# FraPria/proovread

Measured on AMD Instinct MI355X. Metric: corrected long-read Mbases/sec per node, higher is better.
Workload: dtype int32

## Files before the change

include/prgpu.h:

```cpp
#ifndef PRGPU_H
#define PRGPU_H
#include <stdint.h>
#ifdef __cplusplus
extern "C" {
#endif

enum {
    PR_OK = 0,
    PR_ERR_ARG = -1,
    PR_ERR_HIP = -2,
    PR_ERR_SAM = -3,
    PR_ERR_NOSEQ = -4,
    PR_ERR_BIN_RANGE = -5,
    PR_ERR_DIV0 = -6,
    PR_ERR_CIGAR = -7,
    PR_ERR_BEYOND_REF = -8,
    PR_ERR_CAPACITY = -9,
    PR_ERR_UNSUPPORTED = -10,
};

const char *pr_last_error(void);
const char *pr_version(void);

typedef struct pr_ctx pr_ctx;
int pr_ctx_create(int device, pr_ctx **out);
void pr_ctx_destroy(pr_ctx *ctx);
int pr_device_count(int *n);
int pr_ctx_sync(pr_ctx *ctx);
int pr_dev_alloc(pr_ctx *ctx, int64_t bytes, void **dev);
int pr_dev_free(pr_ctx *ctx, void *dev);
int pr_dev_download(pr_ctx *ctx, void *host, const void *dev, int64_t bytes);
int pr_dev_upload(pr_ctx *ctx, void *dev, const void *host, int64_t bytes);
typedef struct {
    char name[16];
    int64_t cur, peak, at_total_peak;
} pr_mem_group;
int pr_mem_stats(int64_t *cur, int64_t *peak, pr_mem_group *groups, int cap, int *n_groups);
void pr_mem_reset_peak(void);

#define PR_COMM_ID_BYTES 128
enum { PR_DT_I64 = 0, PR_DT_F64 = 1, PR_DT_I32 = 2, PR_DT_U8 = 3 };
enum { PR_RED_SUM = 0, PR_RED_MAX = 1, PR_RED_MIN = 2 };
typedef struct pr_comm pr_comm;
int pr_comm_unique_id(uint8_t *id);
int pr_comm_init(pr_ctx *ctx, int world, int rank, const uint8_t *id, pr_comm **out);
void pr_comm_destroy(pr_comm *c);
int pr_comm_rank(const pr_comm *c, int *rank, int *world);
int pr_comm_agree(pr_comm *c, int local_rc);
int pr_comm_allreduce_dev(pr_comm *c, const void *dev_in, void *dev_out, int64_t n, int dtype, int op);
int pr_comm_allreduce_host(pr_comm *c, void *buf, int64_t n, int dtype, int op);
int pr_comm_barrier(pr_comm *c);
int pr_comm_allgatherv_host(pr_comm *c, const uint8_t *send, int64_t nbytes, uint8_t *recv, int64_t recv_cap,
                            int64_t *counts);
int pr_comm_alltoall_counts(pr_comm *c, const int64_t *send_counts, int64_t *recv_counts);
int pr_comm_alltoallv_host(pr_comm *c, const uint8_t *send, const int64_t *send_counts, uint8_t *recv,
                           const int64_t *recv_counts);
int pr_comm_alltoallv_dev(pr_comm *c, const void *send, const int64_t *send_counts, void *recv,
                          const int64_t *recv_counts);
int pr_comm_allgatherv_dev(pr_comm *c, const void *send, const int64_t *counts, void *recv);
typedef struct pr_comm_group pr_comm_group;
int pr_comm_group_create(int world, pr_comm_group **out);
void pr_comm_group_destroy(pr_comm_group *g);
void pr_comm_group_abort(pr_comm_group *g);
int pr_comm_init_local(pr_ctx *ctx, pr_comm_group *g, int rank, pr_comm **out);


typedef struct pr_cns_params {
    double max_coverage;
    double bin_size;
    int32_t trim;
    int32_t indel_taboo_length;
    double indel_taboo;
    int32_t min_aln_length;
    int32_t max_ins_length;
    int32_t fallback_phred;
    int32_t phred_offset;
    int32_t ref_phred_offset;
    int32_t use_ref_qual;
    int32_t qual_weighted;
    int32_t detect_chimera;
    int32_t invert_scores;
} pr_cns_params;

void pr_cns_params_default(pr_cns_params *p);

enum { PR_ALN_HAS_SCORE = 1, PR_ALN_NO_QUAL = 2, PR_ALN_NO_SEQ = 4 };

typedef struct pr_cns_batch {
    int32_t n_lr;
    const int64_t *lr_off;
    const uint8_t *ref_seq;
    const uint8_t *ref_qual;
    const int64_t *ign_off;
    const int32_t *ign;
    const int64_t *aln_off;
    const int32_t *aln_pos;
    const double *aln_score;
    const uint8_t *aln_flags;
    const int64_t *aln_seq_off;
    const int32_t *aln_lseq;
    const int64_t *aln_cig_off;
    const int32_t *aln_ncig;
    const uint8_t *seq_pool;
    const uint8_t *qual_pool;
    const uint32_t *cig_pool;
    int64_t seq_pool_len, cig_pool_len;
} pr_cns_batch;

typedef struct pr_cns_bounds {
    int64_t seq_cap;
    int64_t chim_cap;
} pr_cns_bounds;
int pr_cns_bounds_of(const pr_cns_batch *b, pr_cns_bounds *out);

typedef struct pr_cns_out {
    int64_t *out_off;
    int32_t *status;
    int32_t *seq_len;
    int32_t *trace_len;
    int32_t *ncigar;
    int32_t *nchim;
    uint8_t *seq;
    uint8_t *qual;
    uint8_t *trace;
    uint32_t *cigar;
    int64_t *chim_off;
    int32_t *chim;
    uint8_t *kept;
    int64_t *bin_bases;
} pr_cns_out;

int pr_cns_run(pr_ctx *ctx, const pr_cns_params *p, const pr_cns_batch *b, pr_cns_out *o);

int pr_cns_upload(pr_ctx *ctx, const pr_cns_batch *b);
int pr_cns_launch(pr_ctx *ctx, const pr_cns_params *p);
int pr_cns_download(pr_ctx *ctx, pr_cns_out *o);
int pr_cns_last_timing(pr_ctx *ctx, double *ms_prep, double *ms_pileup);
int pr_cns_phase_ticks(pr_ctx *ctx, uint64_t *ticks, int n);
int pr_cns_resident_stats(pr_ctx *ctx, int64_t *columns, int64_t *alg_bytes);



typedef struct pr_sw_opts {
    int32_t a, b;
    int32_t o_del, e_del;
    int32_t o_ins, e_ins;
    int32_t w;
    int32_t pen_clip5, pen_clip3;
    int32_t zdrop;
    double min_score_per_base;
    int32_t bin_size;
    double bin_length;
    double drop_ratio;
    double mask_level;
    double mask_level_redun;
    int32_t max_chain_gap;
} pr_sw_opts;
void pr_sw_opts_default(pr_sw_opts *o, int finish);

typedef struct pr_sw_batch {
    int32_t n_sr;
    const int64_t *sr_off;
    const uint8_t *sr_seq;
    int32_t n_lr;
    const int64_t *lr_off;
    const uint8_t *lr_seq;
    int64_t n_task;
    const int32_t *t_sr, *t_lr;
    const uint8_t *t_strand;
    const int32_t *t_qbeg, *t_rbeg, *t_slen;
    const int32_t *t_chain;
    int64_t read_id0;
} pr_sw_batch;

typedef struct pr_sw_out {
    int32_t *qb, *qe;
    int32_t *rb, *re;
    int32_t *score;
    int32_t *truesc;
    int32_t *pos;
    int32_t *ncigar;
    uint8_t *pass;
    int32_t *status;
    int64_t *cigar_off;
    uint32_t *cigar;
    int64_t cigar_cap;
    int32_t *task;
    int32_t *flag;
} pr_sw_out;

int pr_sw_run(pr_ctx *ctx, const pr_sw_opts *o, const pr_sw_batch *b, pr_sw_out *out);
int pr_sw_upload(pr_ctx *ctx, const pr_sw_batch *b);
int pr_sw_launch(pr_ctx *ctx, const pr_sw_opts *o);
int pr_sw_download(pr_ctx *ctx, pr_sw_out *out);
int pr_sw_cigar_total(pr_ctx *ctx, int64_t *total, int64_t *n_overflow);
int pr_sw_aln_count(pr_ctx *ctx, int64_t *n_aln);
typedef struct pr_sam_in {
    const int64_t *sr_off;
    const uint8_t *sr_text;
    const uint8_t *sr_qual;
    const char *sr_names;
    const int64_t *sr_name_off;
    const char *lr_names;
    const int64_t *lr_name_off;
    const uint8_t *keep;
    int32_t n_threads;
} pr_sam_in;
int pr_sw_binfilter(pr_ctx *ctx, int32_t bin_size, double bin_length, uint8_t *keep);
int pr_sw_sam(pr_ctx *ctx, const pr_sam_in *in, char **text, int64_t *len, int64_t *n_records);
int pr_sw_bwa_stats(pr_ctx *ctx, int32_t *rounds, int64_t *n_extended, int64_t *n_patch);
int pr_sw_bwa_timing(pr_ctx *ctx, float *walk_ms, float *final_ms, float *early_final_ms);
int pr_sw_last_timing(pr_ctx *ctx, double *ms_extend, double *ms_global);
int pr_sw_last_cells(pr_ctx *ctx, int64_t *cells_extend, int64_t *cells_global);
int pr_sw_dominant_kernel(pr_ctx *ctx, double *ms, int64_t *cells);
int pr_sw_extension_kernels(pr_ctx *ctx, double *ms, int64_t *cells, int32_t *launches);
int pr_sw_phase_cycles(pr_ctx *ctx, int64_t *out4);

typedef struct pr_seed_opts {
    int min_seed_len;
    int min_chain_weight;
    int w;
    double split_factor;
    int split_width;
    int max_mem_intv;
    int max_occ;
    double drop_ratio;
    int max_chain_gap;
    double mask_level;
    int a, o_del, e_del, o_ins, e_ins;
    int b;
} pr_seed_opts;
typedef struct pr_seed_task {
    int32_t sr, lr;
    int32_t strand;
    int32_t qbeg, rbeg, slen;
    int32_t rmax0, rmax1;
    int32_t chain;
    int32_t rank;
} pr_seed_task;
typedef struct pr_seed_tasks {
    int64_t n;
    pr_seed_task *t;
} pr_seed_tasks;
typedef struct pr_seed_index pr_seed_index;
void pr_seed_opts_default(pr_seed_opts *o, int finish);
int pr_seed_index_build(const uint8_t *lr_seq, const int64_t *lr_off, int n_lr, pr_seed_index **out);
void pr_seed_index_free(pr_seed_index *h);
int pr_seed_map(const pr_seed_index *h, const pr_seed_opts *o, const uint8_t *sr_seq, const int64_t *sr_off,
                int n_sr, int n_threads, pr_seed_tasks *out);
void pr_seed_tasks_free(pr_seed_tasks *t);
int pr_seed_index_occ(const pr_seed_index *h, const uint8_t *s, int n, int64_t *count);
int pr_seed_index_digest(const pr_seed_index *h, uint64_t *out6);
int pr_seed_index_koff(const pr_seed_index *h, uint64_t *koff, uint64_t *ksplit);
int pr_seed_gpu_index_koff(pr_ctx *ctx, uint64_t *koff, uint64_t *ksplit);
int pr_seed_smem(const pr_seed_index *h, const uint8_t *q, int len, int x, int64_t min_intv, int32_t *start,
                 int32_t *end, int64_t *occ, int cap, int *n_out);
int pr_seed_gpu_upload(pr_ctx *ctx, const pr_seed_index *h);
int pr_seed_gpu_map(pr_ctx *ctx, const pr_seed_opts *o, const uint8_t *sr_seq, const int64_t *sr_off, int n_sr,
                    pr_seed_tasks *out, int32_t *status);
int pr_seed_gpu_index_build(pr_ctx *ctx, const uint8_t *lr_seq, const int64_t *lr_off, int n_lr);
int pr_seed_gpu_index_digest(pr_ctx *ctx, uint64_t *out6);
int pr_seed_gpu_index_last_ms(pr_ctx *ctx, double *ms);
int pr_seed_gpu_seed_count(pr_ctx *ctx, int64_t *n);
int pr_seed_gpu_pass2_reads(pr_ctx *ctx, int64_t *n);
int pr_seed_gpu_pass_reads(pr_ctx *ctx, int64_t *n4);
int pr_seed_gpu_last_ms(pr_ctx *ctx, double *ms);
int pr_seed_gpu_phase_ticks(pr_ctx *ctx, uint64_t *ticks4);
int pr_seed_gpu_lane_ticks(pr_ctx *ctx, uint64_t *ticks6);
int pr_seed_gpu_occ_ticks(pr_ctx *ctx, uint64_t *ticks3);
int pr_seed_gpu_pass2_ticks(pr_ctx *ctx, uint64_t *t7);
int pr_seed_gpu_pass2_ms(pr_ctx *ctx, double *ms);
int pr_seed_map_device_caps(const pr_seed_index *h, const pr_seed_opts *o, const uint8_t *sr_seq,
                            const int64_t *sr_off, int n_sr, int n_threads, pr_seed_tasks *out, int32_t *status);

typedef struct pr_iter_batch {
    pr_sw_batch sw;
    const int64_t *task_lr_off;
    const uint8_t *lr_qual;
    const uint8_t *ref_seq;
} pr_iter_batch;
int pr_iter_upload(pr_ctx *ctx, const pr_iter_batch *b);
int pr_iter_upload_gpu_seeds(pr_ctx *ctx, const pr_iter_batch *b);
int pr_iter_launch(pr_ctx *ctx, const pr_sw_opts *o, const pr_cns_params *p);
int pr_iter_download(pr_ctx *ctx, pr_cns_out *out);
int pr_fmt_chim_lines(int32_t n_lr, const char *names, const int64_t *name_off, const int32_t *nchim,
                      const int64_t *chim_off, const int32_t *chim, char **text, int64_t *len, int64_t *n_lines);
int pr_iter_download_range(pr_ctx *ctx, int32_t first, int32_t n, pr_cns_out *out);
int pr_iter_bounds(pr_ctx *ctx, int32_t *n_lr, int64_t *n_task, pr_cns_bounds *bd);
int pr_iter_alignment_stats(pr_ctx *ctx, int64_t *n_aln, int64_t *sum_ncig, int64_t *sum_lseq);
int pr_iter_handoff_stats(pr_ctx *ctx, int64_t *big_reads, int64_t *big_alns, int32_t *max_alns);
int pr_iter_handoff_order(pr_ctx *ctx, int32_t lr, int32_t *task_idx, int64_t cap, int64_t *n);
int pr_iter_last_timing(pr_ctx *ctx, double *ms_sw_extend, double *ms_sw_global, double *ms_assemble,
                        double *ms_consensus);
int pr_sw_upload_gpu_seeds(pr_ctx *ctx, const pr_sw_batch *b);
int pr_aln_exchange(pr_ctx *ctx, pr_comm *comm, int64_t sr0, const int64_t *lr_bounds, int64_t *n_recv);
int pr_aln_exchange_local(pr_ctx *const *ctxs, int world, const int64_t *sr0, const int64_t *lr_bounds,
                          int64_t *n_recv);
int pr_aln_exchange_sources(pr_ctx *ctx, int64_t *per_rank, int cap, int *world);
typedef struct pr_own_batch {
    int32_t lr0, n_lr;
    const int64_t *lr_off;
    const uint8_t *ref_seq;
    const uint8_t *lr_qual;
    int32_t n_sr;
    const int64_t *sr_off;
    const uint8_t *sr_seq;
    int32_t from_set;
} pr_own_batch;
enum { PR_OWN_FROM_SET = 1, PR_OWN_RESIDENT_SR = 2 };
int pr_iter_upload_owned(pr_ctx *ctx, const pr_own_batch *b);

enum { PR_LRSET_MAP = 0, PR_LRSET_READS = 1 };
enum { PR_LRSET_COMMIT_MASK = 1, PR_LRSET_COMMIT_DRY = 2 };
int pr_lrset_load(pr_ctx *ctx, int32_t n_lr, const int64_t *off, const uint8_t *seq, const uint8_t *qual);
int pr_lrset_info(pr_ctx *ctx, int32_t *n_lr, int64_t *bases);
int pr_lrset_index(pr_ctx *ctx, int which);
int pr_iter_upload_lrset(pr_ctx *ctx, const pr_sw_batch *b);
int pr_lrset_commit(pr_ctx *ctx, pr_comm *comm, int flags);
int pr_lrset_download(pr_ctx *ctx, int64_t *off, uint8_t *seq, uint8_t *qual, uint8_t *map);
int pr_lrset_snapshot(pr_ctx *ctx);
int pr_lrset_restore(pr_ctx *ctx);
int pr_srset_load(pr_ctx *ctx, int64_t n_sr, const int64_t *off, const uint8_t *seq);
int pr_seed_gpu_map_sampled(pr_ctx *ctx, const pr_seed_opts *o, const int64_t *ranges, int n_ranges, int32_t *status);
int pr_srset_sample(pr_ctx *ctx, const int64_t *ranges, int n_ranges);

int pr_iter_stats(pr_ctx *ctx, int32_t min_phred, int64_t *dev_out);

typedef struct pr_mask_params {
    int32_t phred_min, phred_max;
    int32_t mask_min_len;
    int32_t unmask_min_len;
    int32_t mask_reduce;
    double end_ratio;
    int32_t phred_offset;
} pr_mask_params;
void pr_mask_params_default(pr_mask_params *p);
int pr_mask_params_parse(const char *hcr_mask, int32_t min_sr_length, pr_mask_params *out);
int pr_mask_bound(const pr_mask_params *p, int32_t n, const int64_t *off, int64_t *mcr_cap);
int pr_mask_run(pr_ctx *ctx, const pr_mask_params *p, int32_t n, const int64_t *off, const uint8_t *seq,
                const uint8_t *qual, uint8_t *out_seq, int64_t *mcr_off, int32_t *mcr, int32_t *n_mcr,
                int64_t *stats);
int pr_iter_mask(pr_ctx *ctx, const pr_mask_params *p, int64_t *dev_stats);
int pr_iter_mask_download(pr_ctx *ctx, uint8_t *masked);

int pr_fastq4_scan(const uint8_t *data, int64_t n, int64_t *n_rec, int64_t *n_bases);
int pr_fastq4_fill(const uint8_t *data, int64_t n, const uint8_t *table256, int64_t *starts, int64_t *off,
                   uint8_t *pool);

typedef struct pr_trim_params {
    int32_t size;
    int32_t soft;
    int32_t hard;
    int32_t min_len;
    int32_t phred_offset;
} pr_trim_params;
void pr_trim_params_default(pr_trim_params *p);
int pr_trim_params_parse(const char *trim_win, pr_trim_params *p);
int pr_trim_bound(const pr_trim_params *p, int32_t n, const int64_t *off, int64_t *win_cap);
int pr_trim_windows(const pr_trim_params *p, int32_t n, const int64_t *off, const uint8_t *qual, int64_t *win_off,
                    int32_t *win, int32_t *n_win, int n_threads);

int pr_sam_encode(const char *text, int64_t len, const char *const *ref_names, int32_t n_ref, int n_threads,
                  uint8_t **out, int64_t *out_len, int64_t *n_records);
int pr_bgzf_compress(const uint8_t *data, int64_t len, int level, int n_threads, uint8_t **out, int64_t *out_len);
int pr_bgzf_decompress(const uint8_t *data, int64_t len, int n_threads, uint8_t **out, int64_t *out_len);
int pr_bam_sort_records(const uint8_t *recs, int64_t len, int n_threads, uint8_t **out, int64_t *out_len,
                        int64_t *n_records);
typedef struct pr_bam_alns {
    int64_t n;
    int32_t *rid, *pos1;
    double *score;
    uint8_t *flags;
    int64_t *seq_off;
    int32_t *lseq;
    int64_t *cig_off;
    int32_t *ncig;
    uint8_t *seq, *qual;
    uint32_t *cig;
    int64_t seq_len, cig_len;
} pr_bam_alns;
int pr_bam_decode_alns(const uint8_t *recs, int64_t len, int n_threads, pr_bam_alns *out);
void pr_bam_alns_free(pr_bam_alns *a);
int pr_bam_decode_alns_gpu(pr_ctx *ctx, const uint8_t *recs, int64_t len, pr_bam_alns *out);
int pr_cns_upload_bam(pr_ctx *ctx, const pr_cns_batch *reads, const uint8_t *recs, int64_t len,
                      const int32_t *ref_to_lr, int32_t n_ref, int64_t *n_kept);
int pr_cns_resident_bounds(pr_ctx *ctx, pr_cns_bounds *out);
int pr_cns_resident_aln_count(pr_ctx *ctx, int64_t *n_aln, int64_t *aln_off);
int pr_bam_decode_last_ms(pr_ctx *ctx, double *ms);
int pr_bam_index(const uint8_t *data, int64_t len, int n_threads, uint8_t **out, int64_t *out_len);
void pr_buffer_free(void *p);

typedef struct pr_siam_aligner {
    int32_t a, b;
    int32_t o, e;
    int32_t w, zdrop;
    int32_t word;
} pr_siam_aligner;
typedef struct pr_siam_params {
    int32_t seq_min_len;
    int32_t term_ignore_len;
    int32_t trim;
    int32_t filter_inconclusive;
    double aln_min_idy;
    pr_siam_aligner pass1, pass2;
} pr_siam_params;
typedef struct pr_siam_hsp {
    int32_t read, qas, qae, sas, sae, length, matches, score;
} pr_siam_hsp;
enum { PR_SIAM_KEEP = 0, PR_SIAM_TRIM = 1, PR_SIAM_DROP = 2 };
enum {
    PR_SIAM_SEED_OVERFLOW = 1,
    PR_SIAM_HSP_OVERFLOW = 2,
    PR_SIAM_TOO_LONG = 4,
};
#define PR_SIAM_MAX_SEEDS 1024
#define PR_SIAM_MAX_HSPS 64
#define PR_SIAM_MAX_LEN 131072
typedef struct pr_siam_decision {
    int32_t action, from, to;
} pr_siam_decision;
void pr_siam_params_default(pr_siam_params *p);
int pr_siam_hsps_host(const pr_siam_aligner *al, double min_idy, const uint8_t *seq, const int64_t *off, int32_t n,
                      int n_threads, const pr_siam_hsp **hsps, int64_t *n_hsps, int32_t *status);
int pr_siam_hsps_gpu(pr_ctx *ctx, const pr_siam_aligner *al, double min_idy, const uint8_t *seq, const int64_t *off,
                     int32_t n, const pr_siam_hsp **hsps, int64_t *n_hsps, int32_t *status);
int pr_siam_decide(const pr_siam_params *p, int32_t len, const pr_siam_hsp *h1, int32_t n1, const pr_siam_hsp *h2,
                   int32_t n2, pr_siam_decision *out, int32_t *inconclusive);
int pr_siam_run(pr_ctx *ctx, const pr_siam_params *p, const uint8_t *seq, const int64_t *off, int32_t n,
                int n_threads, pr_siam_decision *out, int32_t *status, int64_t *summary);
int pr_siam_last_ms(pr_ctx *ctx, double *ms);
int pr_siam_seeds_host(const uint8_t *seq, int32_t len, int32_t word, int32_t *out, int32_t cap, int32_t *n);
int pr_siam_extend_host(const pr_siam_aligner *al, const uint8_t *q, int32_t qlen, const uint8_t *t, int32_t tlen,
                        int32_t h0, int32_t *out);
int pr_siam_extend_gpu(pr_ctx *ctx, const pr_siam_aligner *al, const uint8_t *q, const int64_t *q_off,
                       const uint8_t *t, const int64_t *t_off, const int32_t *h0, int32_t n, int32_t *out);

#ifdef __cplusplus
}
#endif
#endif
```

proovread_amd/csrc/seed.cpp:

```cpp
#include <algorithm>
#include <atomic>
#include <cstdlib>
#include <cstring>
#include <string>
#include <thread>
#include <utility>
#include <vector>

#include <sys/mman.h>

#include "../../include/prgpu.h"
#include "seed_core.h"
#include "seed_dev.h"

namespace seedc = prgpu::seedc;

int pr_set_error(int code, const char *msg);

namespace {

constexpr int KI = 12;
constexpr uint32_t NK = 1u << (2 * KI);
constexpr uint8_t SEP = 5;
constexpr int KX = 28;
// ... 326 lines not shown
    };
    const int64_t n_text = 2 * l_pac + 2 * (int64_t)n_lr;
    I.text.resize((size_t)n_text);
    I.cstart.assign(2 * (size_t)n_lr, 0);
    for (int i = 0; i < n_lr; ++i) {
        I.cstart[i] = I.lr_off[i] + i;
        I.cstart[2 * (size_t)n_lr - 1 - i] = l_pac + n_lr + (l_pac - I.lr_off[i + 1]) + (n_lr - 1 - i);
    }
    run_threads([&](int t) {
        uint8_t *X = I.text.data();
        for (int i = (int)((int64_t)n_lr * t / nt); i < (int)((int64_t)n_lr * (t + 1) / nt); ++i) {
            const uint8_t *r = lr_seq + lr_off[i];
            const int64_t len = lr_off[i + 1] - lr_off[i];
            uint8_t *f = X + I.cstart[i];
            uint8_t *b = X + I.cstart[2 * (size_t)n_lr - 1 - i];
            for (int64_t p = 0; p < len; ++p) {
                const uint8_t c = seedc::base_code(r[p]);
                f[p] = c;
                b[len - 1 - p] = c < 4 ? (uint8_t)(3 - c) : 4;
            }
            f[len] = SEP;
            b[len] = SEP;
        }
    });
    const uint8_t *T = I.text.data();
    const int64_t n = (int64_t)I.text.size();
    {
        const int64_t nb = (n >> CB_SHIFT) + 1;
        I.cblk.assign((size_t)nb, 0);
        int c = 0;
        const int nc = (int)I.cstart.size();
        for (int64_t b = 0; b < nb; ++b) {
            while (c + 1 < nc && I.cstart[c + 1] <= (b << CB_SHIFT)) ++c;
            I.cblk[(size_t)b] = c;
        }
    }
    auto for_kmers = [&](int64_t p0, int64_t p1, auto f) {
        uint32_t code = 0;
        int run = 0;
        int64_t p = p0 - (KI - 1) > 0 ? p0 - (KI - 1) : 0;
        for (; p < p1 + KI - 1 && p < n; ++p) {
            if (T[p] > 3) { run = 0; code = 0; continue; }
            code = ((code << 2) | T[p]) & (NK - 1);
            if (++run >= KI && p - KI + 1 >= p0) f(code, (int64_t)(p - KI + 1));
        }
    };
    std::vector<std::vector<uint32_t>> tc((size_t)nt);
    run_threads([&](int t) {
        std::vector<uint32_t> &c = tc[(size_t)t];
        c.assign(NK, 0);
        for_kmers(n * t / nt, n * (t + 1) / nt, [&](uint32_t k, int64_t) { ++c[k]; });
    });
    std::vector<uint32_t> kc(NK);
    I.koff.assign(NK + 1, 0);
    std::vector<uint64_t> part((size_t)nt + 1, 0);
    run_threads([&](int t) {
        const uint32_t k0 = (uint32_t)((uint64_t)NK * t / nt), k1 = (uint32_t)((uint64_t)NK * (t + 1) / nt);
        uint64_t run = 0;
        for (uint32_t k = k0; k < k1; ++k) {
            uint32_t sum = 0;
            for (int u = 0; u < nt; ++u) sum += tc[(size_t)u][k];
            kc[k] = sum;
            run += sum;
            I.koff[k + 1] = run;
        }
        part[(size_t)t + 1] = run;
    });
    for (int t = 0; t < nt; ++t) part[(size_t)t + 1] += part[(size_t)t];
    run_threads([&](int t) {
        const uint32_t k0 = (uint32_t)((uint64_t)NK * t / nt), k1 = (uint32_t)((uint64_t)NK * (t + 1) / nt);
        const uint64_t base = part[(size_t)t];
        for (uint32_t k = k0; k < k1; ++k) I.koff[k + 1] += base;
    });
    I.kpos.resize(I.koff[NK]);
    I.kext.resize(I.koff[NK]);
    constexpr int LB = 12;
    constexpr uint32_t NB = NK >> LB;
    struct Rec {
        uint32_t pos, low;
        uint64_t ext;
    };
    const bool paged = n > (int64_t)seedc::POS_PAGE;
    if (paged) I.ksplit.assign(NK, 0);
    BigVec<Rec> tmp(I.koff[NK]);
    {
        std::vector<std::vector<uint64_t>> cur((size_t)nt, std::vector<uint64_t>(NB, 0));
        run_threads([&](int u) {
            for (uint32_t b = (uint32_t)((uint64_t)NB * u / nt); b < (uint32_t)((uint64_t)NB * (u + 1) / nt); ++b) {
                uint64_t o = I.koff[b << LB];
                for (int t = 0; t < nt; ++t) {
                    cur[(size_t)t][b] = o;
                    uint64_t sz = 0;
                    for (uint32_t k = b << LB; k < ((b + 1) << LB); ++k) sz += tc[(size_t)t][k];
                    o += sz;
                }
            }
        });
        tc.clear();
        tc.shrink_to_fit();
        run_threads([&](int t) {
            const int64_t p0 = n * t / nt, p1 = n * (t + 1) / nt;
            uint64_t *c = cur[(size_t)t].data();
            Rec *R = tmp.data();
            uint32_t code = 0;
            int run = 0;
            int64_t p = p0 - (KI - 1) > 0 ? p0 - (KI - 1) : 0;
            uint64_t w = 0;
            for (int j = KX - 1; j >= 0; --j) w = (w << 2) | (p + 1 + j < n ? (uint64_t)(T[p + 1 + j] & 3) : 0);
            int64_t nb = p + 1;
            while (nb < n && T[nb] <= 3) ++nb;
            for (bool first = true; p < p1 + KI - 1 && p < n; ++p, first = false) {
                if (!first) {
                    const int64_t q = p + KX;
                    w = (w >> 2) | ((q < n ? (uint64_t)(T[q] & 3) : 0) << (2 * (KX - 1)));
                    if (nb < p + 1) {
                        nb = p + 1;
                        while (nb < n && T[nb] <= 3) ++nb;
                    }
                }
                if (T[p] > 3) { run = 0; code = 0; continue; }
                code = ((code << 2) | T[p]) & (NK - 1);
                if (++run >= KI && p - KI + 1 >= p0) {
                    int64_t m = nb - (p + 1);
                    if (m > KX) m = KX;
                    const uint64_t ext = (m ? (w & ((1ull << (2 * m)) - 1)) : 0) | ((uint64_t)m << 56);
                    Rec &r = R[c[code >> LB]++];
                    r.pos = (uint32_t)(p - KI + 1);
                    r.low = (code & ((1u << LB) - 1)) | ((uint32_t)((uint64_t)(p - KI + 1) >> 32) << 31);
                    r.ext = ext;
                }
            }
        });
    }
    {
        std::atomic<uint32_t> next{0};
        run_threads([&](int) {
            std::vector<uint64_t> fill((size_t)1 << LB);
            for (uint32_t b; (b = next.fetch_add(1)) < NB;) {
                const uint32_t k0 = b << LB;
                for (uint32_t j = 0; j < (1u << LB); ++j) fill[j] = I.koff[k0 + j];
                if (paged)
                    for (uint32_t j = 0; j < (1u << LB); ++j) I.ksplit[k0 + j] = I.koff[k0 + j + 1];
                for (uint64_t i = I.koff[k0]; i < I.koff[k0 + (1u << LB)]; ++i) {
                    const Rec &r = tmp[i];
                    const uint32_t lo = r.low & ((1u << LB) - 1);
                    const uint64_t slot = fill[lo]++;
                    if ((r.low >> 31) && I.ksplit[k0 + lo] > slot) I.ksplit[k0 + lo] = slot;
                    I.kpos[slot] = r.pos;
                    I.kext[slot] = r.ext;
                }
            }
        });
    }
    tmp.clear();
    tmp.shrink_to_fit();
    std::vector<std::vector<uint32_t>> tail(KI);
    {
        std::vector<std::vector<int64_t>> stops((size_t)nt);
        run_threads([&](int t) {
            for (int64_t p = n * t / nt; p < n * (t + 1) / nt; ++p)
                if (T[p] > 3 && p > 0 && T[p - 1] <= 3) stops[(size_t)t].push_back(p);
        });
        for (auto &v : stops)
            for (const int64_t p : v) {
                uint32_t code = 0;
                for (int j = 1; j < KI && p - j >= 0 && T[p - j] <= 3; ++j) {
                    code |= (uint32_t)T[p - j] << (2 * (j - 1));
                    tail[j].push_back(code);
                }
            }
    }
    I.cnt[KI - 1] = std::move(kc);
    for (int j = KI - 1; j >= 1; --j) {
        std::vector<uint32_t> &cj = I.cnt[j - 1];
        cj.assign((size_t)1 << (2 * j), 0);
        const std::vector<uint32_t> &cn = I.cnt[j];
        for (size_t x = 0; x < cj.size(); ++x) cj[x] = cn[4 * x] + cn[4 * x + 1] + cn[4 * x + 2] + cn[4 * x + 3];
        for (uint32_t code : tail[j]) ++cj[code];
    }
    *out = h;
    return 0;
}

extern "C" void pr_seed_index_free(pr_seed_index *h) { delete h; }

template <class T>
static uint64_t digest_of(const T *p, size_t n) {
    uint64_t h = 1469598103934665603ull ^ (uint64_t)n;
    for (size_t i = 0; i < n; ++i) {
        h ^= (uint64_t)p[i];
        h *= 1099511628211ull;
        h ^= h >> 29;
    }
    return h;
}

template <class A, class B, class Cc, class Dd, class E, class F, class G, class H>
static void digest6(const A &text, const B &koff, const Cc &kpos, const Dd &kext, const E &cnt, const F &cstart,
                    const G &cblk, const H &lr_off, uint64_t *out6) {
    out6[0] = digest_of(text.data(), text.size());
    out6[1] = digest_of(koff.data(), koff.size());
    out6[2] = digest_of(kpos.data(), kpos.size());
    out6[3] = digest_of(kext.data(), kext.size());
    uint64_t c = 0;
    for (int j = 0; j < KI; ++j) c = c * 31 + digest_of(cnt[j].data(), cnt[j].size());
    out6[4] = c;
    out6[5] = digest_of(cstart.data(), cstart.size()) * 31 + digest_of(cblk.data(), cblk.size()) * 7 +
              digest_of(lr_off.data(), lr_off.size());
}

extern "C" int pr_seed_index_digest(const pr_seed_index *h, uint64_t *out6) {
    if (!h || !out6) return pr_set_error(PR_ERR_ARG, "null arg");
    const Index &I = h->I;
    digest6(I.text, I.koff, I.kpos, I.kext, I.cnt, I.cstart, I.cblk, I.lr_off, out6);
    if (!I.ksplit.empty()) out6[1] ^= digest_of(I.ksplit.data(), I.ksplit.size()) * 31;
    return 0;
}

extern "C" int pr_seed_index_koff(const pr_seed_index *h, uint64_t *koff, uint64_t *ksplit) {
    if (!h || !koff) return pr_set_error(PR_ERR_ARG, "null arg");
    std::memcpy(koff, h->I.koff.data(), h->I.koff.size() * 8);
    if (ksplit && !h->I.ksplit.empty()) std::memcpy(ksplit, h->I.ksplit.data(), h->I.ksplit.size() * 8);
    return 0;
}

namespace prgpu {
void seed_digest_tables(const std::vector<uint8_t> &text, const std::vector<uint64_t> &koff,
                        const std::vector<uint32_t> &kpos, const std::vector<uint64_t> &kext,
                        const std::vector<std::vector<uint32_t>> &cnt, const std::vector<int64_t> &cstart,
                        const std::vector<int32_t> &cblk, const std::vector<int64_t> &lr_off,
                        const std::vector<uint64_t> &ksplit, uint64_t *out6) {
    digest6(text, koff, kpos, kext, cnt, cstart, cblk, lr_off, out6);
    if (!ksplit.empty()) out6[1] ^= digest_of(ksplit.data(), ksplit.size()) * 31;
}
}

extern "C" int pr_seed_index_occ(const pr_seed_index *h, const uint8_t *s, int n, int64_t *count) {
    if (!h || !s || !count || n <= 0) return pr_set_error(PR_ERR_ARG, "bad arg");
    for (int i = 0; i < n; ++i)
        if (s[i] > 3) { *count = 0; return 0; }
    *count = occ(h->I, s, 0, n);
    return 0;
}

extern "C" int pr_seed_smem(const pr_seed_index *h, const uint8_t *q, int len, int x, int64_t min_intv,
                            int32_t *start, int32_t *end, int64_t *occs, int cap, int *n_out) {
    if (!h || !q || !n_out || x < 0 || x >= len) return pr_set_error(PR_ERR_ARG, "bad arg");
    std::vector<Iv> mem;
    const int ret = smem1(IndexOcc{h->I, q}, q, len, x, min_intv, mem);
    if ((int)mem.size() > cap) return pr_set_error(PR_ERR_CAPACITY, "smem output capacity");
    for (size_t i = 0; i < mem.size(); ++i) start[i] = mem[i].start, end[i] = mem[i].end, occs[i] = mem[i].occ;
    *n_out = (int)mem.size();
    return ret;
}

extern "C" int pr_seed_map(const pr_seed_index *h, const pr_seed_opts *o, const uint8_t *sr_seq, const int64_t *sr_off,
                           int n_sr, int n_threads, pr_seed_tasks *out) {
    if (!h || !o || !out || n_sr < 0 || (n_sr && (!sr_seq || !sr_off))) return pr_set_error(PR_ERR_ARG, "null arg");
    if (o->min_seed_len < KI) return pr_set_error(PR_ERR_UNSUPPORTED, "min seed length below the 12-mer index");
    if (o->max_occ <= 0 || o->w < 0) return pr_set_error(PR_ERR_ARG, "bad seeding options");
    out->n = 0;
    out->t = nullptr;
    for (int i = 0; i < n_sr; ++i)
        if (sr_off[i + 1] < sr_off[i] || sr_off[i + 1] - sr_off[i] > (1 << 20))
            return pr_set_error(PR_ERR_ARG, "sr_off not monotone");
    int nt = n_threads > 0 ? n_threads : (int)std::thread::hardware_concurrency();
    nt = nt < 1 ? 1 : (nt > 256 ? 256 : nt);
    std::vector<ReadOut> res(n_sr);
    const seedc::IndexView V = view_of(h->I);
    std::atomic<int> next{0};
    auto work = [&]() {
        std::vector<uint8_t> q;
        for (;;) {
            const int i0 = next.fetch_add(64);
            if (i0 >= n_sr) break;
            for (int i = i0; i < n_sr && i < i0 + 64; ++i) {
                const int len = (int)(sr_off[i + 1] - sr_off[i]);
                q.assign(sr_seq + sr_off[i], sr_seq + sr_off[i + 1]);
                for (auto &c : q) c = c < 4 ? c : 4;
                if (len > 0) map_read(V, *o, q.data(), len, i, res[i]);
            }
        }
    };
    std::vector<std::thread> th;
    for (int t = 1; t < nt; ++t) th.emplace_back(work);
    work();
    for (auto &t : th) t.join();
    int64_t total = 0;
    for (auto &r : res) total += (int64_t)r.tasks.size();
    out->t = (pr_seed_task *)std::malloc(sizeof(pr_seed_task) * (size_t)(total > 0 ? total : 1));
    if (!out->t) return pr_set_error(PR_ERR_ARG, "out of host memory");
    int64_t k = 0;
    for (auto &r : res)
        for (auto &t : r.tasks) out->t[k++] = t;
    out->n = total;
    return 0;
}

extern "C" void pr_seed_tasks_free(pr_seed_tasks *t) {
    if (t && t->t) std::free(t->t);
    if (t) t->t = nullptr, t->n = 0;
}

extern "C" int pr_seed_map_device_caps(const pr_seed_index *h, const pr_seed_opts *o, const uint8_t *sr_seq,
                                       const int64_t *sr_off, int n_sr, int n_threads, pr_seed_tasks *out,
                                       int32_t *status) {
    if (!h || !o || !out || !status || n_sr < 0 || (n_sr && (!sr_seq || !sr_off)))
        return pr_set_error(PR_ERR_ARG, "null arg");
    if (o->min_seed_len < KI) return pr_set_error(PR_ERR_UNSUPPORTED, "min seed length below the 12-mer index");
    out->n = 0;
    out->t = nullptr;
    seedc::IndexView V = view_of(h->I);
    int qmax = 1;
    for (int i = 0; i < n_sr; ++i) qmax = std::max<int>(qmax, (int)(sr_off[i + 1] - sr_off[i]));
    std::vector<uint64_t> text4((size_t)(V.n_text / 16 + 8), 0);
    for (size_t w = 0; w < text4.size(); ++w) {
        uint64_t v = 0;
        for (int k = 0; k < 16; ++k) {
            const int64_t x = (int64_t)w * 16 + k;
            v |= (uint64_t)(x < V.n_text ? V.text[x] : SEP) << (4 * k);
        }
        text4[w] = v;
    }
    V.text4 = text4.data();
    seedc::Caps caps = seedc::device_caps(qmax);
    caps.hi = V.ksplit != nullptr;
    caps.lazy = seedc::lazy_occ(*o) ? 1 : 0;
    const int64_t bytes = seedc::scratch_bytes(caps);
    int nt = n_threads > 0 ? n_threads : (int)std::thread::hardware_concurrency();
    nt = nt < 1 ? 1 : (nt > 64 ? 64 : nt);
    std::vector<ReadOut> res(n_sr);
    std::atomic<int> next{0};
    const char *fe = getenv("PRGPU_SCRATCH_FILL");
    const uint64_t fill = fe ? 0x0101010101010101ull * (uint64_t)(strtoul(fe, nullptr, 0) & 0xFF) : 0;
    auto work = [&]() {
        std::vector<uint64_t> slab((size_t)(bytes / 8 + 1), fill);
        seedc::Scratch S = seedc::carve(reinterpret_cast<uint8_t *>(slab.data()), caps);
        for (int k = 0; k < S.hsize; ++k) S.htab[k].key = -1;
        S.htab_clean = true;
        std::vector<pr_seed_task> buf((size_t)caps.out);
        std::vector<uint64_t> big;
        for (;;) {
            const int i = next.fetch_add(1);
            if (i >= n_sr) break;
            const int len = (int)(sr_off[i + 1] - sr_off[i]);
            int n = 0, err = 0;
            if (len > 0) err = seedc::map_read(V, *o, S, sr_seq + sr_off[i], len, i, buf.data(), caps.out, &n);
            seedc::Caps cg = caps;
            for (int pass = 3; pass <= 6 && err && !(err & (seedc::SC_OVER_LEN | seedc::SC_OVER_OUT)); ++pass) {
                cg = seedc::grow_caps(cg, err, 4);
                big.assign((size_t)(seedc::scratch_bytes(cg) / 8 + 1), fill);
                seedc::Scratch G = seedc::carve(reinterpret_cast<uint8_t *>(big.data()), cg);
                for (int k = 0; k < G.hsize; ++k) G.htab[k].key = -1;
                G.htab_clean = true;
                err = seedc::map_read(V, *o, G, sr_seq + sr_off[i], len, i, buf.data(), caps.out, &n);
            }
            status[i] = err;
            if (!err) res[i].tasks.assign(buf.begin(), buf.begin() + n);
        }
    };
    std::vector<std::thread> th;
    for (int t = 1; t < nt; ++t) th.emplace_back(work);
    work();
    for (auto &t : th) t.join();
    int64_t total = 0;
    for (auto &r : res) total += (int64_t)r.tasks.size();
    out->t = (pr_seed_task *)std::malloc(sizeof(pr_seed_task) * (size_t)(total > 0 ? total : 1));
    if (!out->t) return pr_set_error(PR_ERR_ARG, "out of host memory");
    int64_t k = 0;
    for (auto &r : res)
        for (auto &t : r.tasks) out->t[k++] = t;
    out->n = total;
    return 0;
}
```

proovread_amd/csrc/seed_api.cpp:

```cpp
#include <algorithm>
#include <climits>
#include <cstdio>
#include <cstdlib>
#include <cstring>
#include <vector>

#include "ctx.h"
#include "seed_index_dev.h"
#include "seed_plan.h"

static int seed_text4(pr_ctx *c, seedc::IndexView &v, hipStream_t s) {
    int rc = c->sd[SI_TEXT4].ensure((size_t)ix_pack4_words(v.n_text) * 8);
    if (rc) return rc;
    const int e = ix_pack4_launch(v.text, v.n_text, c->sd[SI_TEXT4].as<uint64_t>(), s);
    if (e) return set_error(PR_ERR_HIP, "text packing: %s", hipGetErrorString((hipError_t)e));
    v.text4 = c->sd[SI_TEXT4].as<uint64_t>();
    v.walk_nw = v.n_text > ((int64_t)64 << 24) ? 1 : 4;
    if (const char *w = getenv("PRGPU_SEED_WALK_NW"))
        v.walk_nw = atoi(w) == 1 ? 1 : 4;
    return 0;
}

static int upload_blk_fr(pr_ctx *c, seedc::IndexView &v, const int64_t *cstart, const int64_t *off, int n_lr,
                         int64_t l_pac, int64_t n_text, hipStream_t s) {
    const int64_t nb = (n_text >> seedc::CB_SHIFT) + 1;
    const int nc = 2 * n_lr;
    const int bs = 1 << seedc::CB_SHIFT;
    auto delta = [&](int ci) -> int64_t {
        if (ci < n_lr) return off[ci] - cstart[ci];
        const int rid = 2 * n_lr - 1 - ci;
        return 2 * l_pac - off[rid + 1] - cstart[ci];
    };
    std::vector<seedc::BlkFr> t((size_t)nb);
    int ci = 0;
    for (int64_t b = 0; b < nb; ++b) {
        const int64_t b0 = b << seedc::CB_SHIFT, b1 = b0 + bs;
        while (ci + 1 < nc && cstart[ci + 1] <= b0) ++ci;
        seedc::BlkFr &e = t[(size_t)b];
        e.c0 = ci;
        e.d0 = nc ? delta(ci) : 0;
        e.d1 = ci + 1 < nc ? delta(ci + 1) : 0;
        e.bnd = ci + 1 < nc && cstart[ci + 1] < b1 ? (int32_t)(cstart[ci + 1] - b0) : bs;
        e.bnd2 = ci + 2 < nc && cstart[ci + 2] < b1 ? (int32_t)(cstart[ci + 2] - b0) : bs;
    }
    int rc = c->sd[SI_BLKFR].ensure(t.size() * sizeof(seedc::BlkFr));
    if (rc) return rc;
    HIPCHK(hipMemcpyAsync(c->sd[SI_BLKFR].p, t.data(), t.size() * sizeof(seedc::BlkFr), hipMemcpyHostToDevice, s));
    HIPCHK(hipStreamSynchronize(s));
    v.blkfr = c->sd[SI_BLKFR].as<seedc::BlkFr>();
    return 0;
}

extern "C" int pr_seed_gpu_upload(pr_ctx *c, const pr_seed_index *h) {
    if (!c || !h) return set_error(PR_ERR_ARG, "null arg");
    HIPCHK(hipSetDevice(c->device));
    hipStream_t s = c->stream;
    const seedc::IndexView hv = seed_index_view(h);
    const SeedIndexSizes z = seed_index_sizes(h);
    DevBuf *D = c->sd;
    int rc;
    if ((rc = upload(D[SI_TEXT], hv.text, (size_t)z.text, s)) || (rc = upload(D[SI_CSTART], hv.cstart, (size_t)z.cstart, s)) ||
        (rc = upload(D[SI_CBLK], hv.cblk, (size_t)z.cblk, s)) || (rc = upload(D[SI_LROFF], hv.lr_off, (size_t)z.lr_off, s)) ||
        (rc = upload(D[SI_KOFF], hv.koff, (size_t)z.koff, s)) || (rc = upload(D[SI_KPOS], hv.kpos, (size_t)z.kpos, s)) ||
        (rc = upload(D[SI_KEXT], hv.kext, (size_t)z.kpos, s)) ||
        (z.ksplit && (rc = upload(D[SI_KSPLIT], hv.ksplit, (size_t)z.ksplit, s))))
        return rc;
    seedc::IndexView v = hv;
    for (int j = 0; j < seedc::KI - 1; ++j) {
        if ((rc = upload(D[SI_CNT0 + j], hv.cnt[j], (size_t)z.cnt[j], s))) return rc;
        v.cnt[j] = D[SI_CNT0 + j].as<uint32_t>();
    }
    v.text = D[SI_TEXT].as<uint8_t>();
    v.cstart = D[SI_CSTART].as<int64_t>();
    v.cblk = D[SI_CBLK].as<int32_t>();
    v.lr_off = D[SI_LROFF].as<int64_t>();
    v.koff = D[SI_KOFF].as<uint64_t>();
    v.kpos = D[SI_KPOS].as<uint32_t>();
    v.kext = D[SI_KEXT].as<uint64_t>();
    v.ksplit = z.ksplit ? D[SI_KSPLIT].as<uint64_t>() : nullptr;
    if ((rc = seed_text4(c, v, s))) return rc;
    if ((rc = upload_blk_fr(c, v, hv.cstart, hv.lr_off, hv.n_lr, hv.l_pac, hv.n_text, s))) return rc;
    HIPCHK(hipStreamSynchronize(s));
    c->seed_view = v;
    c->seed_loaded = true;
    return 0;
}

static void index_host_tables(const int64_t *lr_off, int n_lr, int64_t l_pac, int64_t n_text, std::vector<int64_t> &off,
                              std::vector<int64_t> &cstart, std::vector<int32_t> &cblk) {
    off.assign((size_t)n_lr + 1, 0);
    cstart.assign(2 * (size_t)n_lr, 0);
    for (int i = 0; i <= n_lr; ++i) off[(size_t)i] = lr_off[i] - (n_lr ? lr_off[0] : 0);
    for (int i = 0; i < n_lr; ++i) {
        cstart[(size_t)i] = off[(size_t)i] + i;
        cstart[2 * (size_t)n_lr - 1 - i] = l_pac + n_lr + (l_pac - off[(size_t)i + 1]) + (n_lr - 1 - i);
    }
    const int64_t nb = (n_text >> seedc::CB_SHIFT) + 1;
    cblk.assign((size_t)nb, 0);
    int ci = 0;
    const int nc = 2 * n_lr;
    for (int64_t b = 0; b < nb; ++b) {
        while (ci + 1 < nc && cstart[(size_t)ci + 1] <= (b << seedc::CB_SHIFT)) ++ci;
        cblk[(size_t)b] = ci;
    }
}

static int64_t index_sort_chunk(const DevBuf *D, int64_t n_text) {
    int64_t chunk = (int64_t)1 << 30;
    if (n_text > chunk) {
        size_t fr = 0, tot = 0;
        (void)hipMemGetInfo(&fr, &tot);
        (void)hipGetLastError();
        const int64_t have = (int64_t)(D[SX_KEY0].cap + D[SX_KEY1].cap + D[SX_VAL0].cap + D[SX_VAL1].cap + D[SX_TEMP].cap);
        if ((int64_t)fr + have >= ((int64_t)1 << 31) * 20 + ((int64_t)64 << 30)) chunk = (int64_t)1 << 31;
    }
    if (const char *ch = getenv("PRGPU_INDEX_CHUNK")) {
        const int k = atoi(ch);
        if (k >= 16 && k <= 31) chunk = (int64_t)1 << k;
    }
    return chunk;
}

static int index_buffers(pr_ctx *c, const uint8_t *lr_seq, const int64_t *lr_off, int n_lr, bool lr_dev, int64_t l_pac,
                         int64_t n_text, int64_t chunk, const std::vector<int64_t> &off, const std::vector<int64_t> &cstart,
                         const std::vector<int32_t> &cblk, SeedIndexBuild &B) {
    hipStream_t s = c->stream;
    DevBuf *D = c->sd;
    const size_t nt = (size_t)(n_text > 0 ? n_text : 1);
    const bool chunked = n_text > chunk;
    const size_t ns = (size_t)(chunked ? chunk : (int64_t)nt);
    const size_t temp = seed_index_temp_bytes((int64_t)ns);
    const size_t nk1 = (size_t)seedc::NK + 1;
    int rc;
    if ((rc = upload(D[SX_LRSEQ], lr_dev ? nullptr : (n_lr ? lr_seq + lr_off[0] : lr_seq), (size_t)l_pac, s)) ||
        (rc = upload(D[SI_LROFF], off.data(), off.size(), s)) || (rc = upload(D[SI_CSTART], cstart.data(), cstart.size(), s)) ||
        (rc = upload(D[SI_CBLK], cblk.data(), cblk.size(), s)) || (rc = D[SI_TEXT].ensure(nt)) ||
        (rc = D[SX_KEY0].ensure(ns * 4)) || (rc = D[SX_KEY1].ensure(ns * 4)) || (rc = D[SX_VAL0].ensure(ns * 4)) ||
        (rc = D[SX_KC].ensure(nk1 * 4)) || (rc = D[SI_KOFF].ensure(nk1 * 8)) ||
        (rc = D[SI_KPOS].ensure(nt * 4)) || (rc = D[SI_KEXT].ensure(nt * 8)) || (rc = D[SX_TEMP].ensure(temp)) ||
        (rc = D[SX_CNTPTR].ensure(sizeof(uint32_t *) * (seedc::KI - 1))))
        return rc;
    if (chunked && ((rc = D[SX_VAL1].ensure(ns * 4)) || (rc = D[SX_KCC].ensure(nk1 * 4)) ||
                    (rc = D[SX_KOFFC].ensure(nk1 * 4)) || (rc = D[SX_KCUR].ensure(nk1 * 8))))
        return rc;
    const bool paged = n_text > (int64_t)seedc::POS_PAGE;
    if (paged && (rc = D[SI_KSPLIT].ensure(nk1 * 8))) return rc;
    if (lr_dev && l_pac) HIPCHK(hipMemcpyAsync(D[SX_LRSEQ].p, lr_seq + lr_off[0], (size_t)l_pac, hipMemcpyDeviceToDevice, s));
    uint32_t *cptr[seedc::KI - 1];
    for (int j = 1; j < seedc::KI; ++j) {
        if ((rc = D[SI_CNT0 + j - 1].ensure(((size_t)1 << (2 * j)) * 4))) return rc;
        cptr[j - 1] = B.cnt[j - 1] = D[SI_CNT0 + j - 1].as<uint32_t>();
    }
    HIPCHK(hipMemcpyAsync(D[SX_CNTPTR].p, cptr, sizeof cptr, hipMemcpyHostToDevice, s));
    B.lr_seq = D[SX_LRSEQ].as<uint8_t>();
    B.lr_off = D[SI_LROFF].as<int64_t>();
    B.n_lr = n_lr;
    B.l_pac = l_pac;
    B.cstart = D[SI_CSTART].as<int64_t>();
    B.n_text = n_text;
    B.text = D[SI_TEXT].as<uint8_t>();
    B.chunk = chunk;
    B.key0 = D[SX_KEY0].as<uint32_t>();
    B.key1 = D[SX_KEY1].as<uint32_t>();
    B.val0 = D[SX_VAL0].as<uint32_t>();
    B.val1 = chunked ? D[SX_VAL1].as<uint32_t>() : nullptr;
    B.kc = D[SX_KC].as<uint32_t>();
    B.koff = D[SI_KOFF].as<uint64_t>();
    B.kcc = chunked ? D[SX_KCC].as<uint32_t>() : nullptr;
    B.koffc = chunked ? D[SX_KOFFC].as<uint32_t>() : nullptr;
    B.kcur = chunked ? D[SX_KCUR].as<uint64_t>() : nullptr;
    B.kpos = D[SI_KPOS].as<uint32_t>();
    B.kext = D[SI_KEXT].as<uint64_t>();
    B.ksplit = paged ? D[SI_KSPLIT].as<uint64_t>() : nullptr;
    B.cnt_dev = reinterpret_cast<uint32_t *const *>(D[SX_CNTPTR].p);
    B.temp = D[SX_TEMP].p;
    B.temp_bytes = temp;
    return 0;
}

int index_build(pr_ctx *c, const uint8_t *lr_seq, const int64_t *lr_off, int n_lr, bool lr_dev) {
    if (!c || n_lr < 0 || (n_lr && (!lr_seq || !lr_off))) return set_error(PR_ERR_ARG, "null arg");
    for (int i = 0; i < n_lr; ++i)
        if (lr_off[i + 1] < lr_off[i]) return set_error(PR_ERR_ARG, "lr_off not monotone");
    const int64_t l_pac = n_lr ? lr_off[n_lr] - lr_off[0] : 0;
    if (2 * l_pac + 2 * (int64_t)n_lr > seedc::MAX_TEXT)
        return set_error(PR_ERR_CAPACITY, "long reads beyond the index's 2^33 text positions (l_pac < 4.29 Gb)");
    if ((int64_t)n_lr >= ((int64_t)1 << seedc::FR_RID_BITS))
        return set_error(PR_ERR_CAPACITY, "more than 2^24 long reads in one index");
    HIPCHK(hipSetDevice(c->device));
    hipStream_t s = c->stream;
    DevBuf *D = c->sd;
    const int64_t n_text = 2 * l_pac + 2 * (int64_t)n_lr;
    std::vector<int64_t> off, cstart;
    std::vector<int32_t> cblk;
    index_host_tables(lr_off, n_lr, l_pac, n_text, off, cstart, cblk);
    SeedIndexBuild B{};
    int rc = index_buffers(c, lr_seq, lr_off, n_lr, lr_dev, l_pac, n_text, index_sort_chunk(D, n_text), off, cstart, cblk, B);
    if (rc) return rc;
    HIPCHK(hipEventRecord(c->ev[8], s));
    const int e = seed_index_device_build(B, s);
    if (e) return set_error(PR_ERR_HIP, "seed index build: %s", hipGetErrorString((hipError_t)e));
    HIPCHK(hipEventRecord(c->ev[9], s));
    uint64_t nh = 0;
    HIPCHK(hipMemcpyAsync(&nh, B.koff + seedc::NK, 8, hipMemcpyDeviceToHost, s));
    HIPCHK(hipStreamSynchronize(s));
    float ms = 0.f;
    if (hipEventElapsedTime(&ms, c->ev[8], c->ev[9]) == hipSuccess) c->ms_index = ms;
    if (n_text > (int64_t)seedc::POS_PAGE) {
        for (int id : {(int)SX_KEY0, (int)SX_KEY1, (int)SX_VAL0, (int)SX_VAL1, (int)SX_TEMP}) D[id].release();
    }
    seedc::IndexView v{};
    v.text = B.text;
    v.n_text = n_text;
    v.cstart = B.cstart;
    v.n_contig = 2 * n_lr;
    v.cblk = D[SI_CBLK].as<int32_t>();
    v.lr_off = B.lr_off;
    v.n_lr = n_lr;
    v.l_pac = l_pac;
    v.koff = B.koff;
    v.kpos = B.kpos;
    v.kext = B.kext;
    v.ksplit = B.ksplit;
    for (int j = 0; j < seedc::KI - 1; ++j) v.cnt[j] = B.cnt[j];
    if ((rc = seed_text4(c, v, s))) return rc;
    if ((rc = upload_blk_fr(c, v, cstart.data(), off.data(), n_lr, l_pac, n_text, s))) return rc;
    c->seed_view = v;
    c->seed_loaded = true;
    c->seed_n_text = n_text;
    c->seed_n_hits = nh;
    return 0;
}

extern "C" int pr_seed_gpu_index_build(pr_ctx *c, const uint8_t *lr_seq, const int64_t *lr_off, int n_lr) {
    return index_build(c, lr_seq, lr_off, n_lr, false);
}

extern "C" int pr_seed_gpu_index_digest(pr_ctx *c, uint64_t *out6) {
    if (!c || !out6) return set_error(PR_ERR_ARG, "null arg");
    if (!c->seed_loaded || !c->seed_n_text) return set_error(PR_ERR_ARG, "no device-built seed index");
    HIPCHK(hipSetDevice(c->device));
    const seedc::IndexView &v = c->seed_view;
    const size_t nt = (size_t)c->seed_n_text, nh = (size_t)c->seed_n_hits, nk = (size_t)seedc::NK;
    std::vector<uint8_t> text(nt);
    std::vector<uint64_t> koff(nk + 1);
    std::vector<uint32_t> kpos(nh), kc(nk);
    std::vector<uint64_t> kext(nh);
    std::vector<int64_t> cstart((size_t)v.n_contig), lro((size_t)v.n_lr + 1);
    std::vector<int32_t> cblk((size_t)((c->seed_n_text >> seedc::CB_SHIFT) + 1));
    std::vector<std::vector<uint32_t>> cnt(seedc::KI);
    HIPCHK(hipMemcpy(text.data(), v.text, nt, hipMemcpyDeviceToHost));
    HIPCHK(hipMemcpy(koff.data(), v.koff, (nk + 1) * 8, hipMemcpyDeviceToHost));
    if (nh) HIPCHK(hipMemcpy(kpos.data(), v.kpos, nh * 4, hipMemcpyDeviceToHost));
    if (nh) HIPCHK(hipMemcpy(kext.data(), v.kext, nh * 8, hipMemcpyDeviceToHost));
    HIPCHK(hipMemcpy(kc.data(), c->sd[SX_KC].p, nk * 4, hipMemcpyDeviceToHost));
    if (!cstart.empty()) HIPCHK(hipMemcpy(cstart.data(), v.cstart, cstart.size() * 8, hipMemcpyDeviceToHost));
    HIPCHK(hipMemcpy(lro.data(), v.lr_off, lro.size() * 8, hipMemcpyDeviceToHost));
    HIPCHK(hipMemcpy(cblk.data(), v.cblk, cblk.size() * 4, hipMemcpyDeviceToHost));
    for (int j = 0; j < seedc::KI - 1; ++j) {
        cnt[(size_t)j].resize((size_t)1 << (2 * (j + 1)));
        HIPCHK(hipMemcpy(cnt[(size_t)j].data(), v.cnt[j], cnt[(size_t)j].size() * 4, hipMemcpyDeviceToHost));
    }
    cnt[seedc::KI - 1] = std::move(kc);
    std::vector<uint64_t> ksplit(v.ksplit ? nk : 0);
    if (v.ksplit) HIPCHK(hipMemcpy(ksplit.data(), v.ksplit, nk * 8, hipMemcpyDeviceToHost));
    seed_digest_tables(text, koff, kpos, kext, cnt, cstart, cblk, lro, ksplit, out6);
    return 0;
}

extern "C" int pr_seed_gpu_index_koff(pr_ctx *c, uint64_t *koff, uint64_t *ksplit) {
    if (!c || !koff) return set_error(PR_ERR_ARG, "null arg");
    if (!c->seed_loaded) return set_error(PR_ERR_ARG, "no device seed index");
    HIPCHK(hipSetDevice(c->device));
    HIPCHK(hipStreamSynchronize(c->stream));
    HIPCHK(hipMemcpy(koff, c->seed_view.koff, ((size_t)seedc::NK + 1) * 8, hipMemcpyDeviceToHost));
    if (ksplit && c->seed_view.ksplit)
        HIPCHK(hipMemcpy(ksplit, c->seed_view.ksplit, (size_t)seedc::NK * 8, hipMemcpyDeviceToHost));
    return 0;
}

extern "C" int pr_seed_gpu_index_last_ms(pr_ctx *c, double *ms) {
    if (!c || !ms) return set_error(PR_ERR_ARG, "null arg");
    *ms = c->ms_index;
    return 0;
}

extern "C" int pr_srset_load(pr_ctx *c, int64_t n_sr, const int64_t *off, const uint8_t *seq) {
    if (!c || n_sr < 0 || !off || (off[n_sr] && !seq) || off[0] != 0) return set_error(PR_ERR_ARG, "bad arg");
    HIPCHK(hipSetDevice(c->device));
    int rc = upload(c->ls[LS_SRSEQ], seq, (size_t)off[n_sr], c->stream);
    if (rc) return rc;
    HIPCHK(hipStreamSynchronize(c->stream));
    c->ss_off.assign(off, off + n_sr + 1);
    c->ss_samp_off.clear();
    c->ls[LS_SRSAMP].release();
    return 0;
}

static int gather_ranges(pr_ctx *c, const int64_t *ranges, int n_ranges, int64_t max_reads, DevBuf &dst,
                         std::vector<int64_t> &off) {
    if (c->ss_off.empty()) return set_error(PR_ERR_ARG, "no resident short reads (pr_srset_load)");
    const int64_t N = (int64_t)c->ss_off.size() - 1;
    off.assign(1, 0);
    for (int k = 0; k < n_ranges; ++k) {
        const int64_t r0 = ranges[2 * k], r1 = ranges[2 * k + 1];
        if (r0 < 0 || r1 < r0 || r1 > N) return set_error(PR_ERR_ARG, "record range outside the short reads");
        for (int64_t i = r0; i < r1; ++i) off.push_back(off.back() + c->ss_off[(size_t)i + 1] - c->ss_off[(size_t)i]);
    }
    if ((int64_t)off.size() - 1 > max_reads) return set_error(PR_ERR_CAPACITY, "too many short reads in one sample");
    HIPCHK(hipSetDevice(c->device));
    int rc = dst.ensure((size_t)off.back() + 1);
    if (rc) return rc;
    int64_t at = 0;
    for (int k = 0; k < n_ranges; ++k) {
        const int64_t b0 = c->ss_off[(size_t)ranges[2 * k]], b1 = c->ss_off[(size_t)ranges[2 * k + 1]];
        if (b1 > b0)
            HIPCHK(hipMemcpyAsync(dst.as<uint8_t>() + at, c->ls[LS_SRSEQ].as<uint8_t>() + b0, (size_t)(b1 - b0),
                                  hipMemcpyDeviceToDevice, c->stream));
        at += b1 - b0;
    }
    return 0;
}

extern "C" int pr_srset_sample(pr_ctx *c, const int64_t *ranges, int n_ranges) {
    if (!c || n_ranges < 0 || (n_ranges && !ranges)) return set_error(PR_ERR_ARG, "null arg");
    std::vector<int64_t> off;
    int rc = gather_ranges(c, ranges, n_ranges, INT64_MAX, c->ls[LS_SRSAMP], off);
    if (rc) return rc;
    c->ss_samp_off.swap(off);
    return 0;
}

namespace {

struct SeedMap {
    pr_ctx *c;
    hipStream_t s;
    DevBuf *D;
    int n_sr;
    int qmax;
    SeedDev K;
    seedc::Caps small, caps;
    int64_t waves;
    int64_t lanes2;
    int64_t chunk;
    std::vector<int32_t> nout, st;
    std::vector<int64_t> pre;
    int64_t total = 0, bad = 0;
    int32_t bad_flags = 0;
};

void map_plan(SeedMap &M, const pr_seed_opts *o, const int64_t *sr_off) {
    pr_ctx *c = M.c;
    int qmax = 1;
    for (int i = 0; i < M.n_sr; ++i) qmax = std::max<int>(qmax, (int)(sr_off[i + 1] - sr_off[i]));
    M.qmax = qmax;
    seedc::Caps &caps = M.caps, &small = M.small;
    caps = seedc::device_caps(qmax);
    caps.hi = c->seed_view.ksplit != nullptr;
    caps.nopos = 1;
    small = seedc::device_caps_small(std::min(qmax, caps.lmax));
    small.hi = caps.hi;
    small.nopos = 1;
    small.lazy = seedc::lazy_occ(*o) ? 1 : 0;
    if (const char *sc = getenv("PRGPU_SEED_SMALL"))
        sscanf(sc, "%d,%d,%d,%d,%d", &small.hits, &small.iv, &small.mems, &small.seeds, &small.chains);
    SeedDev &K = M.K;
    K = SeedDev{};
    K.V = c->seed_view;
    K.O = *o;
    K.n_sr = M.n_sr;
    K.caps = small;
    K.stride = seedc::scratch_bytes(small);
    const char *wpc = getenv("PRGPU_SEED_WAVES_PER_CU");
    size_t fr = 0, tot = 0;
    (void)hipMemGetInfo(&fr, &tot);
    (void)hipGetLastError();
    M.waves = seedp::pass1_waves(M.n_sr, c->n_cu, wpc ? atoi(wpc) : 16, getenv("PRGPU_SEED_BALANCE") != nullptr,
                                 seedp::scratch_budget((int64_t)fr, (int64_t)M.D[SB_SCRATCH].cap), K.stride);
    K.n_lanes = M.waves;
    M.lanes2 = (int64_t)c->n_cu * seed_slots_per_cu(c->seed_view.walk_nw);
    const char *ob = getenv("PRGPU_SEED_OUT_MB");
    M.chunk = seedp::out_chunk((ob ? std::max<int64_t>(1, atoll(ob)) : 8192) << 20,
                               (int64_t)caps.out * (int64_t)sizeof(pr_seed_task));
}

int map_buffers(SeedMap &M, const pr_seed_opts *o, const uint8_t *sr_seq, bool in_sb_seq, const int64_t *sr_off) {
    pr_ctx *c = M.c;
    DevBuf *D = M.D;
    SeedDev &K = M.K;
    const int n_sr = M.n_sr;
    hipStream_t s = M.s;
    int rc;
    K.dp = nullptr;
    if (seedc::seed_flt_min_score(*o, M.qmax) >= 0) {
        if ((rc = D[SB_DP].ensure((size_t)M.waves * 2 * 201 * 64 * sizeof(int16_t)))) return rc;
        K.dp = D[SB_DP].as<int16_t>();
    }
    const int64_t scratch = std::max<int64_t>(M.waves * 64 * K.stride, M.lanes2 * seedc::scratch_bytes(M.caps));
    const int64_t nb = n_sr ? sr_off[n_sr] : 0;
    const int64_t slot_bytes = (int64_t)M.caps.out * (int64_t)sizeof(pr_seed_task);
    c->seed_sr_bases = nb;
    if ((!in_sb_seq && (rc = upload(D[SB_SEQ], sr_seq, (size_t)nb, s))) || (rc = upload(D[SB_OFF], sr_off, (size_t)n_sr + 1, s)) ||
        (rc = D[SB_SCRATCH].ensure((size_t)scratch)) ||
        (rc = D[SB_OUT].ensure((size_t)(std::min<int64_t>(M.chunk, n_sr) * slot_bytes + 16))) ||
        (rc = D[SB_NOUT].ensure((size_t)n_sr * 4 + 16)) || (rc = D[SB_STATUS].ensure((size_t)n_sr * 4 + 16)) ||
        (rc = D[SB_NEXT].ensure(256)) || (rc = D[SB_PRE].ensure(((size_t)n_sr + 1) * 8)) ||
        (rc = D[SB_DENSE].ensure(sizeof(pr_seed_task))))
        return rc;
    K.sr_seq = D[SB_SEQ].as<uint8_t>();
    K.sr_off = D[SB_OFF].as<int64_t>();
    K.out = D[SB_OUT].as<pr_seed_task>();
    K.n_out = D[SB_NOUT].as<int32_t>();
    K.status = D[SB_STATUS].as<int32_t>();
    K.next = D[SB_NEXT].as<int32_t>();
    K.prof = reinterpret_cast<unsigned long long *>(D[SB_NEXT].as<uint8_t>() + 64);
    HIPCHK(hipMemsetAsync(K.next, 0, 256, s));
    return 0;
}

int pass1(SeedMap &M, int64_t r0, int64_t r1, std::vector<int32_t> &redo, seedp::Flagged &f) {
    DevBuf *D = M.D;
    SeedDev &K = M.K;
    hipStream_t s = M.s;
    int rc;
    K.caps = M.small;
    K.stride = seedc::scratch_bytes(M.small);
    K.n_lanes = M.waves;
    K.scratch = D[SB_SCRATCH].as<uint8_t>();
    K.rlist = nullptr;
    K.n_list = 0;
    K.out0 = r0;
    K.n_sr = r1;
    int32_t start = (int32_t)r0;
    const char *lpt = getenv("PRGPU_SEED_LPT");
    if (lpt && lpt[0] == '1') {
        int32_t *order = nullptr;
        if ((rc = D[SB_ORDER].ensure(seed_order_bytes(r1 - r0)))) return rc;
        int eo = seed_order_launch(K, r0, r1 - r0, D[SB_ORDER].p, &order, (void *)s);
        if (eo) return set_error(PR_ERR_HIP, "seed order: %s", hipGetErrorString((hipError_t)eo));
        K.rlist = order;
        K.n_list = r1 - r0;
        start = 0;
    }
    HIPCHK(hipMemcpyAsync(K.next, &start, 4, hipMemcpyHostToDevice, s));
    int e = seed_batch_launch(K, (void *)s);
    if (e) return set_error(PR_ERR_HIP, "seed kernel: %s", hipGetErrorString((hipError_t)e));
    if (r0 == 0) HIPCHK(hipEventRecord(M.c->ev[10], s));
    std::vector<int32_t> st1((size_t)(r1 - r0)), no1((size_t)(r1 - r0));
    if ((rc = download(st1.data(), D[SB_STATUS], (size_t)(r1 - r0), s, (size_t)r0)) ||
        (rc = download(no1.data(), D[SB_NOUT], (size_t)(r1 - r0), s, (size_t)r0)))
        return rc;
    HIPCHK(hipStreamSynchronize(s));
    for (int64_t i = r0; i < r1; ++i)
        if (st1[(size_t)(i - r0)]) {
            redo.push_back((int32_t)i);
            f.add(st1[(size_t)(i - r0)], no1[(size_t)(i - r0)]);
        }
    return 0;
}

int launch_pass(SeedMap &M, const char *name, bool by_wave, const seedc::Caps &caps, int64_t lanes,
                const std::vector<int32_t> &reads) {
    SeedDev &K = M.K;
    K.caps = caps;
    K.stride = seedc::scratch_bytes(caps);
    K.n_lanes = lanes;
    K.scratch = M.D[SB_SCRATCH].as<uint8_t>();
    K.rlist = M.D[SB_PRE].as<int32_t>();
    K.n_list = (int64_t)reads.size();
    HIPCHK(hipMemcpyAsync(M.D[SB_PRE].p, reads.data(), reads.size() * 4, hipMemcpyHostToDevice, M.s));
    HIPCHK(hipMemsetAsync(K.next, 0, 4, M.s));
    const int e = by_wave ? seed_launch(K, (void *)M.s) : seed_batch_launch(K, (void *)M.s);
    if (e) return set_error(PR_ERR_HIP, "seed kernel (%s): %s", name, hipGetErrorString((hipError_t)e));
    return 0;
}

int still_flagged(SeedMap &M, int64_t r0, int64_t r1, const std::vector<int32_t> &reads, std::vector<int32_t> &left,
                  int32_t &flags) {
    std::vector<int32_t> st((size_t)(r1 - r0));
    int rc = download(st.data(), M.D[SB_STATUS], (size_t)(r1 - r0), M.s, (size_t)r0);
    if (rc) return rc;
    HIPCHK(hipStreamSynchronize(M.s));
    left.clear();
    flags = 0;
    for (int32_t i : reads)
        if (st[(size_t)(i - r0)]) left.push_back(i), flags |= st[(size_t)(i - r0)];
    return 0;
}

int pass1b(SeedMap &M, int64_t r0, int64_t r1, const seedp::Flagged &f, std::vector<int32_t> &redo, seedc::Caps &p2caps,
           bool &p2_ran) {
    if (!seedp::pass1b_wanted(f)) return 0;
    const seedp::Pass1bCaps p = seedp::pass1b_caps(M.small, M.caps, f);
    DevBuf &scr = M.D[SB_SCRATCH];
    int rc;
    size_t fr = 0, tot = 0;
    (void)hipMemGetInfo(&fr, &tot);
    (void)hipGetLastError();
    if (const int64_t want = seedp::pass1b_scratch_want(M.waves, f.n, p.sb, (int64_t)fr, (int64_t)scr.cap)) {
        HIPCHK(hipStreamSynchronize(M.s));
        if ((rc = scr.ensure((size_t)want))) return rc;
    }
    const char *p1b = getenv("PRGPU_SEED_1B");
    const seedp::Pass1bForce force =
        !p1b ? seedp::P1B_AUTO : !strcmp(p1b, "wave") ? seedp::P1B_FORCE_WAVE : seedp::P1B_FORCE_LANE;
    const seedp::Pass1bRun r =
        seedp::pass1b_run(p, f, M.small.hits, force, (int64_t)scr.cap, M.waves, M.lanes2, M.c->n_cu);
    if (r.mode == seedp::P1B_SKIP) return 0;
    const bool by_wave = r.mode == seedp::P1B_WAVE;
    if ((rc = launch_pass(M, by_wave ? "pass 1b, waves" : "pass 1b", by_wave, by_wave ? p.cw : p.cb, by_wave ? r.ww : r.wb, redo)))
        return rc;
    M.c->seed_pass_reads[by_wave ? 1 : 0] += (int64_t)redo.size();
    if (by_wave) p2caps = p.cw, p2_ran = true;
    std::vector<int32_t> left;
    int32_t fl;
    if ((rc = still_flagged(M, r0, r1, redo, left, fl))) return rc;
    redo.swap(left);
    M.K.rlist = nullptr;
    M.K.n_list = 0;
    return 0;
}

int pass2_and_later(SeedMap &M, int64_t r0, int64_t r1, std::vector<int32_t> &redo, seedc::Caps cg, bool p2_ran) {
    if (redo.empty()) return 0;
    int rc;
    if (!p2_ran) {
        if ((rc = launch_pass(M, "pass 2", true, M.caps, std::min<int64_t>(M.lanes2, (int64_t)redo.size()), redo))) return rc;
        HIPCHK(hipStreamSynchronize(M.s));
        M.c->seed_pass_reads[2] += (int64_t)redo.size();
    }
    for (int pass = 3; pass <= 6; ++pass) {
        std::vector<int32_t> again;
        int32_t fl;
        if ((rc = still_flagged(M, r0, r1, redo, again, fl))) return rc;
        if (again.empty() || (fl & (seedc::SC_OVER_LEN | seedc::SC_OVER_OUT))) break;
        cg = seedc::grow_caps(cg, fl, 4);
        redo.swap(again);
        const int64_t lanes = std::min<int64_t>(M.lanes2, (int64_t)redo.size());
        if ((rc = M.D[SB_SCRATCH].ensure((size_t)(lanes * seedc::scratch_bytes(cg))))) return rc;
        char name[16];
        snprintf(name, sizeof name, "pass %d", pass);
        if ((rc = launch_pass(M, name, true, cg, lanes, redo))) return rc;
        HIPCHK(hipStreamSynchronize(M.s));
        M.c->seed_pass_reads[3] += (int64_t)redo.size();
    }
    return 0;
}

int compact_chunk(SeedMap &M, int64_t r0, int64_t r1) {
    DevBuf *D = M.D;
    hipStream_t s = M.s;
    int rc;
    if ((rc = download(M.nout.data() + r0, D[SB_NOUT], (size_t)(r1 - r0), s, (size_t)r0)) ||
        (rc = download(M.st.data() + r0, D[SB_STATUS], (size_t)(r1 - r0), s, (size_t)r0)))
        return rc;
    HIPCHK(hipStreamSynchronize(s));
    const int64_t t0 = M.total;
    for (int64_t i = r0; i < r1; ++i) {
        if (M.nout[(size_t)i] < 0 || M.nout[(size_t)i] > M.caps.out) return set_error(PR_ERR_HIP, "seed kernel: bad task count");
        M.total += M.nout[(size_t)i];
        M.pre[(size_t)i + 1] = M.total;
        M.bad += M.st[(size_t)i] != 0;
        M.bad_flags |= M.st[(size_t)i];
    }
    if ((rc = upload(D[SB_PRE], M.pre.data() + r0, (size_t)(r1 - r0 + 1), s)) ||
        (rc = D[SB_DENSE].grow_keep(sizeof(pr_seed_task) * (size_t)(M.total > 0 ? M.total : 1),
                                    sizeof(pr_seed_task) * (size_t)t0, s)))
        return rc;
    const int e = seed_compact_launch(D[SB_OUT].as<pr_seed_task>(), D[SB_NOUT].as<int32_t>() + r0, D[SB_PRE].as<int64_t>(),
                                      r1 - r0, M.caps.out, D[SB_DENSE].as<pr_seed_task>(), (void *)s);
    if (e) return set_error(PR_ERR_HIP, "seed compaction: %s", hipGetErrorString((hipError_t)e));
    return 0;
}

int seed_map(pr_ctx *c, const pr_seed_opts *o, const uint8_t *sr_seq, bool in_sb_seq, const int64_t *sr_off, int n_sr,
             pr_seed_tasks *out, int32_t *status) {
    if (!o || n_sr < 0 || (n_sr && ((!sr_seq && !in_sb_seq) || !sr_off))) return set_error(PR_ERR_ARG, "null arg");
    c->seed_pre.clear();
    if (!c->seed_loaded) return set_error(PR_ERR_ARG, "no seed index on the device (pr_seed_gpu_upload)");
    if (o->min_seed_len < seedc::KI) return set_error(PR_ERR_UNSUPPORTED, "min seed length below the 12-mer index");
    if (o->max_occ <= 0 || o->w < 0) return set_error(PR_ERR_ARG, "bad seeding options");
    if (out) out->n = 0, out->t = nullptr;
    if (n_sr && sr_off[0] != 0) return set_error(PR_ERR_ARG, "sr_off must start at 0");
    for (int i = 0; i < n_sr; ++i)
        if (sr_off[i + 1] < sr_off[i]) return set_error(PR_ERR_ARG, "sr_off not monotone");
    HIPCHK(hipSetDevice(c->device));
    SeedMap M;
    M.c = c;
    M.s = c->stream;
    M.D = c->sd;
    M.n_sr = n_sr;
    hipStream_t s = M.s;
    int rc;
    map_plan(M, o, sr_off);
    if ((rc = map_buffers(M, o, sr_seq, in_sb_seq, sr_off))) return rc;
    HIPCHK(hipEventRecord(c->ev[8], s));
    c->seed_pass2 = 0;
    std::fill(c->seed_pass_reads, c->seed_pass_reads + 4, 0);
    M.nout.resize((size_t)n_sr);
    M.st.resize((size_t)n_sr);
    M.pre.assign((size_t)n_sr + 1, 0);
    for (int64_t r0 = 0; r0 < n_sr; r0 += M.chunk) {
        const int64_t r1 = std::min<int64_t>(n_sr, r0 + M.chunk);
        std::vector<int32_t> redo;
        seedp::Flagged f;
        seedc::Caps p2caps = M.caps;
        bool p2_ran = false;
        if ((rc = pass1(M, r0, r1, redo, f)) || (rc = pass1b(M, r0, r1, f, redo, p2caps, p2_ran))) return rc;
        c->seed_pass2 += (int64_t)redo.size();
        if ((rc = pass2_and_later(M, r0, r1, redo, p2caps, p2_ran)) || (rc = compact_chunk(M, r0, r1))) return rc;
    }
    HIPCHK(hipEventRecord(c->ev[9], s));
    HIPCHK(hipStreamSynchronize(s));
    float ms = 0.f;
    if (n_sr && hipEventElapsedTime(&ms, c->ev[8], c->ev[9]) == hipSuccess) c->ms_seed = ms;
    c->ms_seed_pass2 = 0.f;
    if (n_sr && hipEventElapsedTime(&ms, c->ev[10], c->ev[9]) == hipSuccess) c->ms_seed_pass2 = ms;
    if (M.bad) c->seed_pre.clear();
    else c->seed_pre = M.pre;
    if (out) {
        out->t = (pr_seed_task *)std::malloc(sizeof(pr_seed_task) * (size_t)(M.total > 0 ? M.total : 1));
        if (!out->t) return set_error(PR_ERR_ARG, "out of host memory");
        if (M.total && (rc = download(out->t, M.D[SB_DENSE], (size_t)M.total, s))) return rc;
    }
    HIPCHK(hipStreamSynchronize(s));
    if (out) out->n = M.total;
    if (status) std::memcpy(status, M.st.data(), (size_t)n_sr * 4);
    if (M.bad)
        return set_error(PR_ERR_CAPACITY, "%lld reads outgrew the seeding scratch (status flags, or: 0x%x)", (long long)M.bad,
                         M.bad_flags);
    return 0;
}

}

extern "C" int pr_seed_gpu_map(pr_ctx *c, const pr_seed_opts *o, const uint8_t *sr_seq, const int64_t *sr_off, int n_sr,
                               pr_seed_tasks *out, int32_t *status) {
    if (!c) return set_error(PR_ERR_ARG, "null arg");
    return seed_map(c, o, sr_seq, false, sr_off, n_sr, out, status);
}

extern "C" int pr_seed_gpu_map_sampled(pr_ctx *c, const pr_seed_opts *o, const int64_t *ranges, int n_ranges,
                                       int32_t *status) {
    if (!c || !o || n_ranges < 0 || (n_ranges && !ranges)) return set_error(PR_ERR_ARG, "null arg");
    std::vector<int64_t> off;
    int rc = gather_ranges(c, ranges, n_ranges, INT32_MAX, c->sd[SB_SEQ], off);
    if (rc) return rc;
    return seed_map(c, o, nullptr, true, off.data(), (int)off.size() - 1, nullptr, status);
}


extern "C" int pr_seed_gpu_seed_count(pr_ctx *c, int64_t *n) {
    if (!c || !n) return set_error(PR_ERR_ARG, "null arg");
    *n = c->seed_pre.empty() ? 0 : c->seed_pre.back();
    return 0;
}

extern "C" int pr_seed_gpu_pass2_reads(pr_ctx *c, int64_t *n) {
    if (!c || !n) return set_error(PR_ERR_ARG, "null arg");
    *n = c->seed_pass2;
    return 0;
}

extern "C" int pr_seed_gpu_pass_reads(pr_ctx *c, int64_t *n4) {
    if (!c || !n4) return set_error(PR_ERR_ARG, "null arg");
    std::copy(c->seed_pass_reads, c->seed_pass_reads + 4, n4);
    return 0;
}

extern "C" int pr_seed_gpu_last_ms(pr_ctx *c, double *ms) {
    if (!c || !ms) return set_error(PR_ERR_ARG, "null arg");
    *ms = c->ms_seed;
    return 0;
}

extern "C" int pr_seed_gpu_pass2_ms(pr_ctx *c, double *ms) {
    if (!c || !ms) return set_error(PR_ERR_ARG, "null arg");
    *ms = c->ms_seed_pass2;
    return 0;
}

extern "C" int pr_seed_gpu_phase_ticks(pr_ctx *c, uint64_t *ticks4) {
    if (!c || !ticks4) return set_error(PR_ERR_ARG, "null arg");
    if (!c->sd[SB_NEXT].p) return set_error(PR_ERR_ARG, "no pr_seed_gpu_map launch yet");
    HIPCHK(hipSetDevice(c->device));
    HIPCHK(hipMemcpy(ticks4, c->sd[SB_NEXT].as<uint8_t>() + 64, 32, hipMemcpyDeviceToHost));
    return 0;
}

extern "C" int pr_seed_gpu_lane_ticks(pr_ctx *c, uint64_t *ticks6) {
    if (!c || !ticks6) return set_error(PR_ERR_ARG, "null arg");
    if (!c->sd[SB_NEXT].p) return set_error(PR_ERR_ARG, "no pr_seed_gpu_map launch yet");
    HIPCHK(hipSetDevice(c->device));
    HIPCHK(hipMemcpy(ticks6, c->sd[SB_NEXT].as<uint8_t>() + 64 + 4 * 8, 48, hipMemcpyDeviceToHost));
    return 0;
}

extern "C" int pr_seed_gpu_pass2_ticks(pr_ctx *c, uint64_t *t7) {
    if (!c || !t7) return set_error(PR_ERR_ARG, "null arg");
    if (!c->sd[SB_NEXT].p) return set_error(PR_ERR_ARG, "no pr_seed_gpu_map launch yet");
    HIPCHK(hipSetDevice(c->device));
    HIPCHK(hipMemcpy(t7, c->sd[SB_NEXT].as<uint8_t>() + 64 + 13 * 8, 56, hipMemcpyDeviceToHost));
    return 0;
}

extern "C" int pr_seed_gpu_occ_ticks(pr_ctx *c, uint64_t *ticks3) {
    if (!c || !ticks3) return set_error(PR_ERR_ARG, "null arg");
    if (!c->sd[SB_NEXT].p) return set_error(PR_ERR_ARG, "no pr_seed_gpu_map launch yet");
    HIPCHK(hipSetDevice(c->device));
    HIPCHK(hipMemcpy(ticks3, c->sd[SB_NEXT].as<uint8_t>() + 64 + 10 * 8, 24, hipMemcpyDeviceToHost));
    return 0;
}
```

proovread_amd/csrc/seed_core.h:

```cpp
#pragma once
#include <math.h>
#include <stdint.h>

#include "../../include/prgpu.h"

#if defined(__HIPCC__)
#define SC_HD __host__ __device__ inline
#else
#define SC_HD inline
#endif

#if defined(PR_SEED_STATS) && !defined(__HIP_DEVICE_COMPILE__)
extern unsigned long long pr_seed_stat_g[24];
#define SC_STAT(k, v) __atomic_fetch_add(&pr_seed_stat_g[k], (unsigned long long)(v), __ATOMIC_RELAXED)
#else
#define SC_STAT(k, v) ((void)0)
#endif

namespace prgpu {
namespace seedc {

constexpr int KI = 12;
constexpr uint32_t NK = 1u << (2 * KI);
constexpr int KX = 28;
constexpr uint64_t KX_MASK = (1ull << (2 * KX)) - 1;
#ifndef SC_SCANGE
#define SC_SCANGE 1
#endif
constexpr int HB = 20;
constexpr int CB_SHIFT = 12;
constexpr int RK = 11;

constexpr uint64_t POS_PAGE = 1ull << 32;
constexpr int64_t MAX_TEXT = (int64_t)1 << 33;

struct BlkFr {
    int64_t d0, d1;
    int32_t c0, bnd, bnd2, pad;
};

struct IndexView {
    const uint8_t *text;
    int64_t n_text;
    const int64_t *cstart;
    int32_t n_contig;
    const int32_t *cblk;
    const int64_t *lr_off;
    int32_t n_lr;
    int64_t l_pac;
    const uint64_t *koff;
    const uint32_t *kpos;
    const uint64_t *ksplit;
    const uint64_t *kext;
    const uint32_t *cnt[KI - 1];
    const uint64_t *text4;
    const BlkFr *blkfr;
    int32_t walk_nw = 4;
};

struct Iv {
    int32_t start, end;
    int64_t occ;
};
struct Seed {
    int64_t rbeg;
    int16_t qbeg, len;
    int32_t nx;
};
struct RangeRec {
    int32_t head, tail, n, l_idx;
    int64_t tpos;
    int64_t f_rbeg, l_rbeg;
    int32_t f_ql, l_ql;
    int32_t pad[4];
};
struct RangeEnt {
    int32_t key, r;
};
struct Chain {
    int64_t pos;
    int32_t rid, head, tail, n;
    int32_t w, kept, first;
};

enum {
    SC_OVER_LEN = 1, SC_OVER_HITS = 2, SC_OVER_IV = 4, SC_OVER_MEMS = 8, SC_OVER_SEEDS = 16,
    SC_OVER_CHAINS = 32, SC_OVER_OUT = 64
};

struct Scratch {
    int32_t lmax;
    int32_t *hoff;
    uint64_t *qext;
    int32_t *codes;
    uint32_t *ge;
    uint32_t *hpos;
    uint8_t *hhi;
    uint16_t *hml;
    int32_t cap_hits;
    Iv *mems;
    int32_t cap_mems;
    Iv *m1, *curr, *prev;
    int32_t cap_iv;
    Seed *seeds;
    int32_t cap_seeds;
    Chain *cv, *ch;
    int32_t *cnx, *kept;
    RangeEnt *htab;
    RangeRec *rg;
    int32_t cap_chains, hsize;
    uint16_t *rmax;
    uint64_t *hfr;
    int32_t *hend;
    uint8_t *ready;
    uint64_t *q4w;
    int32_t *lz;
    bool htab_clean;
};

SC_HD uint64_t pack_ext(const uint8_t *s, int n) {
    uint64_t v = 0;
    int k = 0;
    for (; k < n && s[k] < 4; ++k) v |= (uint64_t)s[k] << (2 * k);
    return v | ((uint64_t)k << 56);
}

SC_HD int ctz64(uint64_t x) { return __builtin_ctzll(x); }

SC_HD uint8_t base_code(uint8_t c) {
    if (c < 4) return c;
    switch (c | 0x20) {
        case 'a': return 0;
        case 'c': return 1;
        case 'g': return 2;
        case 't': return 3;
        default: return 4;
    }
}

SC_HD uint64_t hit_pos(const IndexView &I, uint32_t code, uint64_t r) {
    uint64_t p = I.kpos[r];
    if (I.ksplit && r >= I.ksplit[code]) p += POS_PAGE;
    return p;
}
SC_HD uint64_t get_hpos(const Scratch &S, int64_t k) {
    return (uint64_t)S.hpos[k] | (S.hhi ? (uint64_t)S.hhi[k] << 32 : 0ull);
}
SC_HD void set_hpos(const Scratch &S, int64_t k, uint64_t p) {
    if (!S.hpos) return;
    S.hpos[k] = (uint32_t)p;
    if (S.hhi) S.hhi[k] = (uint8_t)(p >> 32);
}

SC_HD int contig_of(const IndexView &I, int64_t p) {
    int c = I.cblk[p >> CB_SHIFT];
    while (c + 1 < I.n_contig && I.cstart[c + 1] <= p) ++c;
    return c;
}

SC_HD void text_to_fr(const IndexView &I, uint64_t p, int64_t &fr, int &rid) {
    const int c = contig_of(I, p);
    const int64_t o = (int64_t)p - I.cstart[c];
    if (c < I.n_lr) {
        rid = c;
        fr = I.lr_off[c] + o;
    } else {
        rid = 2 * I.n_lr - 1 - c;
        fr = I.l_pac + (I.l_pac - I.lr_off[rid + 1]) + o;
    }
}

SC_HD uint64_t pack_fr_blk(const IndexView &I, uint64_t p);

constexpr int FR_RID_BITS = 24;
SC_HD uint64_t pack_fr(const IndexView &I, uint64_t p) {
    int64_t fr;
    int rid;
    text_to_fr(I, p, fr, rid);
    return ((uint64_t)fr << FR_RID_BITS) | (uint64_t)rid;
}

SC_HD uint64_t pack_fr_blk(const IndexView &I, uint64_t p) {
    if (I.blkfr) {
        const BlkFr bt = I.blkfr[p >> CB_SHIFT];
        const int o = (int)(p & ((1u << CB_SHIFT) - 1u));
        int c = -1;
        int64_t d = 0;
        if (o < bt.bnd) c = bt.c0, d = bt.d0;
        else if (o < bt.bnd2) c = bt.c0 + 1, d = bt.d1;
        if (c >= 0) {
            const int rid = c < I.n_lr ? c : 2 * I.n_lr - 1 - c;
            return ((uint64_t)((int64_t)p + d) << FR_RID_BITS) | (uint64_t)rid;
        }
    }
    return pack_fr(I, p);
}

SC_HD uint64_t nib16c(const uint64_t *w4, uint64_t x) {
    const uint64_t w = x >> 4;
    const int sh = (int)(x & 15) * 4;
    const uint64_t lo = w4[w];
    return sh ? (lo >> sh) | (w4[w + 1] << (64 - sh)) : lo;
}

constexpr int LC_MAX = 6;
SC_HD constexpr int lc_off(int j) { return ((1 << (2 * j)) - 4) / 3; }
constexpr int LC_N = lc_off(LC_MAX + 1);

template <bool LZ> struct OccB;
SC_HD void materialize(const OccB<true> &occ, int a);

template <bool LZ>
struct OccB {
    const IndexView *I;
    const Scratch *S;
    const uint8_t *q;
    int len;
    const uint32_t *lc = nullptr;

    SC_HD void need(int a) const {
        if constexpr (LZ) {
            if (a < len && !S->ready[a]) materialize(*this, a);
        }
    }
    SC_HD int32_t end_of(int a) const {
        if constexpr (LZ) return S->hend[a];
        else return S->hoff[a + 1];
    }

    SC_HD int64_t jmer(int a, int b) const {
        const int n = b - a;
        uint32_t code = 0;
        const int32_t c12 = a + KI <= len ? S->codes[a] : -1;
        if (c12 >= 0) code = (uint32_t)c12 >> (2 * (KI - n));
        else
            for (int x = a; x < b; ++x) code = (code << 2) | q[x];
        if (lc && n <= LC_MAX) return lc[lc_off(n) + code];
        return I->cnt[n - 1][code];
    }

    SC_HD int64_t operator()(int a, int b) const {
        const int n = b - a;
        SC_STAT(8, 1);
        if (n < KI) return jmer(a, b);
        need(a);
        if (n - KI < HB) return S->ge[(int64_t)a * HB + (n - KI)];
        int64_t c = 0;
        SC_STAT(9, 1);
        const int32_t h1 = end_of(a);
        SC_STAT(10, h1 - S->hoff[a]);
        for (int32_t k = S->hoff[a]; k < h1; ++k) c += S->hml[k] >= n;
        return c;
    }
    SC_HD int64_t scan_ge(int a, int n, int &mn) const {
        int64_t c = 0;
        int m = 0x7fffffff;
        need(a);
        const int32_t h1 = end_of(a);
        SC_STAT(9, 1);
        SC_STAT(10, h1 - S->hoff[a]);
        for (int32_t k = S->hoff[a]; k < h1; ++k) {
            const int v = S->hml[k];
            if (v >= n) {
                ++c;
                m = v < m ? v : m;
            }
        }
        mn = c ? m : 0;
        return c;
    }
};
using Occ = OccB<false>;
using OccLazy = OccB<true>;

SC_HD int short_limit(const uint8_t *q, int len, int a) {
    int e = a;
    while (e < len && e - a < KI - 1 && q[e] < 4) ++e;
    return e;
}
template <class OccT>
SC_HD int rmax_short(const OccT &occ, const uint8_t *q, int len, int a, int64_t k) {
    int e = short_limit(q, len, a);
    while (e > a && occ.jmer(a, e) < k) --e;
    return e;
}

SC_HD void topk_insert(uint16_t (&top)[RK], uint16_t v) {
#pragma unroll
    for (int k = 0; k < RK; ++k) {
        const uint16_t t = top[k];
        const bool gt = v > t;
        top[k] = gt ? v : t;
        v = gt ? t : v;
    }
}
template <class OccT>
SC_HD void fill_rk_top(const OccT &occ, const Scratch &S, const uint8_t *q, int len, int a, const uint16_t (&top)[RK]) {
    uint16_t *r = S.rmax + (int64_t)a * RK;
    int e = -1;
    int64_t ce = 0;
    for (int k = 1; k <= RK; ++k) {
        if (top[k - 1] > 0) {
            r[k - 1] = (uint16_t)(a + top[k - 1]);
            continue;
        }
        if (e < 0) {
            e = short_limit(q, len, a);
            ce = e > a ? occ.jmer(a, e) : 0;
        }
        while (e > a && ce < k) {
            --e;
            ce = e > a ? occ.jmer(a, e) : 0;
        }
        r[k - 1] = (uint16_t)e;
    }
}
template <class OccT>
SC_HD void fill_rk(const OccT &occ, const Scratch &S, const uint8_t *q, int len, int a) {
    uint16_t top[RK];
#pragma unroll
    for (int k = 0; k < RK; ++k) top[k] = 0;
    if (q[a] < 4 && a + KI <= len && S.codes[a] >= 0)
        for (int32_t h = S.hoff[a]; h < S.hoff[a + 1]; ++h) topk_insert(top, S.hml[h]);
    fill_rk_top(occ, S, q, len, a, top);
}

template <class OccT>
SC_HD int rmax_k(const OccT &occ, const Scratch &S, const uint8_t *q, int len, int a, int64_t k) {
    if (k < 1) k = 1;
    occ.need(a);
    if (k <= RK) return S.rmax[(int64_t)a * RK + (k - 1)];
    if (q[a] > 3) return a;
    if (a + KI <= len && S.codes[a] >= 0) {
        const uint32_t *g = S.ge + (int64_t)a * HB;
        if ((int64_t)g[0] >= k) {
            if ((int64_t)g[HB - 1] < k) {
                int lo = 0, hi = HB - 2;
                while (lo < hi) {
                    const int mid = (lo + hi + 1) >> 1;
                    if ((int64_t)g[mid] >= k) lo = mid; else hi = mid - 1;
                }
                return a + KI + lo;
            }
            int lo = KI + HB - 1, hi = len - a;
            while (lo < hi) {
                const int mid = (lo + hi + 1) >> 1;
                int64_t c = 0;
                const int32_t h1 = occ.end_of(a);
                for (int32_t h = S.hoff[a]; h < h1; ++h) c += S.hml[h] >= mid;
                if (c >= k) lo = mid; else hi = mid - 1;
            }
            return a + lo;
        }
    }
    return rmax_short(occ, q, len, a, k);
}

SC_HD int hit_ml(const IndexView &I, const Scratch &S, const uint8_t *q, int len, int a, uint64_t p, uint64_t ex,
                 uint64_t qe) {
    const int le = (int)(ex >> 56), lq = (int)(qe >> 56);
    const uint64_t x = (ex ^ qe) & KX_MASK;
    int m = x ? ctz64(x) >> 1 : KX;
    m = m < le ? m : le;
    m = m < lq ? m : lq;
    int ml = KI + m;
    if (m < KX) return ml;
    if (I.text4 && S.q4w) {
        bool go = a + ml < len;
        while (go) {
            const uint64_t tp = p + (uint64_t)ml;
            const uint64_t *tw4 = I.text4 + (tp >> 4);
            const int sh = (int)(tp & 15) * 4;
            uint64_t w5[5];
#pragma unroll
            for (int j = 0; j < 5; ++j) w5[j] = tw4[j];
#pragma unroll
            for (int j = 0; j < 4; ++j) {
                if (!go) break;
                const int xx = a + ml;
                const uint64_t tw = sh ? (w5[j] >> sh) | (w5[j + 1] << (64 - sh)) : w5[j];
                const uint64_t qw = nib16c(S.q4w, (uint64_t)xx);
                const uint64_t nq = (qw >> 2) & 0x1111111111111111ull;
                const uint64_t bad = (qw ^ tw) | (nq * 0xFull);
                const int lim = len - xx;
                if (bad) {
                    const int f = ctz64(bad) >> 2;
                    ml += f < lim ? f : lim;
                    go = false;
                } else if (lim <= 16) {
                    ml += lim;
                    go = false;
                } else {
                    ml += 16;
                }
            }
        }
    } else {
        while (a + ml < len && q[a + ml] < 4 && I.text[p + ml] == q[a + ml]) ++ml;
    }
    return ml;
}

#if defined(__HIPCC__)
__attribute__((noinline))
#endif
SC_HD void materialize(const OccLazy &occ, int a) {
    const IndexView &I = *occ.I;
    const Scratch &S = *occ.S;
    const uint8_t *q = occ.q;
    const int len = occ.len;
    S.ready[a] = 1;
    const int32_t beg = S.lz[0];
    uint32_t g[HB];
    uint16_t top[RK];
#pragma unroll
    for (int t = 0; t < HB; ++t) g[t] = 0u;
#pragma unroll
    for (int k = 0; k < RK; ++k) top[k] = 0;
    int32_t n = 0;
    const int32_t code = a + KI <= len ? S.codes[a] : -1;
    if (code >= 0) {
        const uint64_t r0 = I.koff[code], r1 = I.koff[code + 1];
        const int64_t need = (int64_t)beg + (int64_t)(r1 - r0);
        if (need > S.cap_hits) {
            S.lz[1] |= SC_OVER_HITS;
            S.lz[2] = (int32_t)(need < (int64_t)1 << 30 ? need : (int64_t)1 << 30);
        } else {
            n = (int32_t)(r1 - r0);
            const uint64_t qe = S.qext[a];
            const bool ranked = q[a] < 4;
            constexpr int MB = 4;
            for (uint64_t r = r0; r < r1; r += MB) {
                uint64_t pp[MB], ex[MB], fr[MB];
#pragma unroll
                for (int u = 0; u < MB; ++u) {
                    const bool ok = r + u < r1;
                    pp[u] = ok ? hit_pos(I, (uint32_t)code, r + u) : 0ull;
                    ex[u] = ok ? I.kext[r + u] : 0ull;
                }
#pragma unroll
                for (int u = 0; u < MB; ++u) fr[u] = r + u < r1 ? pack_fr_blk(I, pp[u]) : 0ull;
#pragma unroll
                for (int u = 0; u < MB; ++u) {
                    if (r + u >= r1) break;
                    const int ml = hit_ml(I, S, q, len, a, pp[u], ex[u], qe);
                    const int32_t k = beg + (int32_t)(r + u - r0);
                    const uint16_t v = (uint16_t)(ml < 65535 ? ml : 65535);
                    S.hml[k] = v;
                    S.hfr[k] = fr[u];
                    const int d = ml - KI;
#pragma unroll
                    for (int t = 0; t < HB; ++t) g[t] += d >= t ? 1u : 0u;
                    if (ranked) topk_insert(top, v);
                }
            }
        }
    }
    S.hoff[a] = beg;
    S.hend[a] = beg + n;
    S.lz[0] = beg + n;
    uint32_t *dst = S.ge + (int64_t)a * HB;
#pragma unroll
    for (int t = 0; t < HB; ++t) dst[t] = g[t];
    fill_rk_top(occ, S, q, len, a, top);
}

SC_HD int build_starts(const IndexView &I, Scratch &S, const uint8_t *q, int len) {
    if (len > S.lmax) return SC_OVER_LEN;
    for (int a = 0; a <= len; ++a) {
        S.codes[a] = -1;
        S.qext[a] = 0;
        S.hoff[a] = 0;
        S.hend[a] = 0;
        S.ready[a] = a == len ? 1 : 0;
    }
    for (int a = 0; a + KI <= len; ++a) {
        const int n = len - a - KI;
        S.qext[a] = pack_ext(q + a + KI, n < KX ? n : KX);
    }
    uint32_t code = 0;
    int run = 0;
    for (int e = 0; e < len; ++e) {
        if (q[e] > 3) {
            run = 0;
            code = 0;
        } else {
            code = ((code << 2) | q[e]) & (NK - 1);
            ++run;
        }
        if (e - KI + 1 >= 0 && run >= KI) S.codes[e - KI + 1] = (int32_t)code;
    }
    if (S.q4w) {
        for (int w = 0; w <= (len >> 4) + 3; ++w) {
            uint64_t v = 0;
            for (int k = 0; k < 16; ++k) {
                const int x = w * 16 + k;
                const uint64_t c = x < len ? (q[x] < 4 ? q[x] : 4u) : 6u;
                v |= c << (4 * k);
            }
            S.q4w[w] = v;
        }
    }
    S.lz[0] = S.lz[1] = S.lz[2] = 0;
    return 0;
}

SC_HD int build_occ(const IndexView &I, Scratch &S, const uint8_t *q, int len) {
    if (len > S.lmax) return SC_OVER_LEN;
    for (int a = 0; a <= len; ++a) {
        S.hoff[a] = 0;
        S.codes[a] = -1;
        S.qext[a] = 0;
    }
    for (int64_t k = 0; k < (int64_t)len * HB; ++k) S.ge[k] = 0;
    for (int a = 0; a + KI <= len; ++a) {
        const int n = len - a - KI;
        S.qext[a] = pack_ext(q + a + KI, n < KX ? n : KX);
    }
    {
        uint32_t code = 0;
        int run = 0;
        for (int e = 0; e < len; ++e) {
            if (q[e] > 3) {
                run = 0;
                code = 0;
            } else {
                code = ((code << 2) | q[e]) & (NK - 1);
                ++run;
            }
            if (e - KI + 1 >= 0 && run >= KI) S.codes[e - KI + 1] = (int32_t)code;
        }
    }
    const uint8_t *T = I.text;
    int32_t nh = 0, prev0 = 0, prev1 = 0;
    for (int a = 0; a + KI <= len; ++a) {
#if !defined(__HIP_DEVICE_COMPILE__)
        constexpr int PF_OFF = 24, PF_POS = 12;
        if (a + PF_OFF < len && S.codes[a + PF_OFF] >= 0) __builtin_prefetch(&I.koff[S.codes[a + PF_OFF]]);
        if (a + PF_POS < len && S.codes[a + PF_POS] >= 0) {
            const uint64_t r0 = I.koff[S.codes[a + PF_POS]];
            __builtin_prefetch(&I.kpos[r0]);
            __builtin_prefetch(&I.kext[r0]);
            __builtin_prefetch(&I.kext[r0] + 8);
        }
#endif
        S.hoff[a] = nh;
        if (S.codes[a] >= 0) {
            const uint32_t code = (uint32_t)S.codes[a];
            const uint64_t r0 = I.koff[code], r1 = I.koff[code + 1];
            if ((int64_t)nh + (int64_t)(r1 - r0) > S.cap_hits) return SC_OVER_HITS;
            uint32_t *g = S.ge + (int64_t)a * HB;
            int32_t k = prev0;
            for (uint64_t r = r0; r < r1; ++r) {
                const uint64_t p = hit_pos(I, code, r);
                while (k < prev1 && get_hpos(S, k) + 1 < p) ++k;
                int ml;
                if (k < prev1 && get_hpos(S, k) + 1 == p && S.hml[k] > KI) {
                    ml = S.hml[k] - 1;
                } else {
                    const uint64_t ex = I.kext[r];
                    const uint64_t qe = S.qext[a];
                    const int le = (int)(ex >> 56), lq = (int)(qe >> 56);
                    const uint64_t x = (ex ^ qe) & KX_MASK;
                    int m = x ? ctz64(x) >> 1 : KX;
                    m = m < le ? m : le;
                    m = m < lq ? m : lq;
                    ml = KI + m;
                    if (m == KX)
                        while (a + ml < len && q[a + ml] < 4 && T[p + ml] == q[a + ml]) ++ml;
                }
                set_hpos(S, nh, p);
                S.hfr[nh] = pack_fr(I, p);
                S.hml[nh] = (uint16_t)(ml < 65535 ? ml : 65535);
                ++nh;
                ++g[ml - KI < HB - 1 ? ml - KI : HB - 1];
            }
            for (int t = HB - 2; t >= 0; --t) g[t] += g[t + 1];
        }
        prev0 = S.hoff[a];
        prev1 = nh;
    }
    for (int a = len - KI + 1 < 0 ? 0 : len - KI + 1; a <= len; ++a) S.hoff[a] = nh;
    const Occ occ{&I, &S, q, len, nullptr};
    for (int a = 0; a < len; ++a) fill_rk(occ, S, q, len, a);
    return 0;
}

SC_HD void iv_reverse(Iv *v, int n) {
    for (int i = 0, j = n - 1; i < j; ++i, --j) {
        const Iv t = v[i];
        v[i] = v[j];
        v[j] = t;
    }
}

template <class OccT>
SC_HD int smem1(const OccT &occ, const Scratch &S, const uint8_t *q, int len, int x, int64_t min_intv, Iv *mem,
                int &nmem, int &err) {
    nmem = 0;
    if (q[x] > 3) return x + 1;
    SC_STAT(16, 1);
    if (min_intv < 1) min_intv = 1;
    Iv *curr = S.curr, *prev = S.prev;
    const int cap = S.cap_iv;
    int nc = 0, np = 0;
    Iv ik{x, x + 1, occ(x, x + 1)};
    int i;
    uint32_t pre[9];
    const bool have = S.codes != nullptr && x + KI <= len && S.codes[x] >= 0;
    if (have) {
        occ.need(x);
        const uint32_t c12 = (uint32_t)S.codes[x];
#pragma unroll
        for (int n = 7; n < KI; ++n) pre[n - 7] = occ.I->cnt[n - 1][c12 >> (2 * (KI - n))];
#pragma unroll
        for (int n = KI; n < 16; ++n) pre[n - 7] = S.ge[(int64_t)x * HB + (n - KI)];
    }
    uint32_t blk[8];
    int blk0 = -1;
    for (i = x + 1; i < len; ++i) {
        if (q[i] < 4) {
            const int n = i + 1 - x;
            int64_t o;
            int skip = 0;
            if (SC_SCANGE && have && n >= KI + HB) {
                int mn;
                o = occ.scan_ge(x, n, mn);
                skip = mn > n ? mn - n : 0;
            } else if (have && n >= 7 && n < 16) {
                uint32_t v = pre[0];
#pragma unroll
                for (int t = 1; t < 9; ++t) v = n - 7 == t ? pre[t] : v;
                o = v;
            } else if (have && n >= 16 && n < KI + HB) {
                const int b0 = n & ~7;
                if (b0 != blk0) {
#pragma unroll
                    for (int t = 0; t < 8; ++t) blk[t] = S.ge[(int64_t)x * HB + (b0 - KI) + t];
                    blk0 = b0;
                }
                uint32_t v = blk[0];
#pragma unroll
                for (int t = 1; t < 8; ++t) v = (n & 7) == t ? blk[t] : v;
                o = v;
            } else {
                o = occ(x, i + 1);
            }
            if (o != ik.occ) {
                if (nc >= cap) { err |= SC_OVER_IV; return len; }
                curr[nc++] = ik;
                if (o < min_intv) break;
            }
            i += skip;
            ik = Iv{x, i + 1, o};
        } else {
            if (nc >= cap) { err |= SC_OVER_IV; return len; }
            curr[nc++] = ik;
            break;
        }
    }
    if (i == len) {
        if (nc >= cap) { err |= SC_OVER_IV; return len; }
        curr[nc++] = ik;
    }
    const int ret = curr[nc - 1].end;
    (void)prev;
    (void)np;
    int a = x, last = x + 1;
    for (int j = nc - 1; j >= 0; --j) {
        const Iv p = curr[j];
        SC_STAT(17, 1);
        while (a > 0 && rmax_k(occ, S, q, len, a - 1, min_intv) >= p.end) --a;
        if (a < last) {
            if (nmem >= cap) { err |= SC_OVER_IV; return len; }
            mem[nmem++] = Iv{a, p.end, a == x ? p.occ : occ(a, p.end)};
            last = a;
        }
    }
    iv_reverse(mem, nmem);
    return ret;
}

template <class OccT>
SC_HD int seed_strategy1(const OccT &occ, const uint8_t *q, int len, int x, int min_len, int64_t max_intv, Iv &m) {
    m = Iv{0, 0, 0};
    if (q[x] > 3) return x + 1;
    for (int i = x + 1; i < len; ++i) {
        if (q[i] > 3) return i + 1;
        if (i - x >= min_len) {
            const int n = i + 1 - x;
            int mn = 0;
            const int64_t o = SC_SCANGE && n >= KI + HB ? occ.scan_ge(x, n, mn) : occ(x, i + 1);
            if (o < max_intv) {
                m = Iv{x, i + 1, o};
                return i + 1;
            }
            if (mn > n) i += mn - n;
        }
    }
    return len;
}

#if defined(__HIP_DEVICE_COMPILE__)
#define SC_TICK(k)                                          \
    do {                                                    \
        if (ticks) {                                        \
            const unsigned long long t_ = __builtin_amdgcn_s_memrealtime();   \
            ticks[k] += t_ - t_last;                        \
            t_last = t_;                                    \
        }                                                   \
    } while (0)
#else
#define SC_TICK(k) do { (void)ticks; } while (0)
#endif

template <class OccT>
SC_HD int collect_intv(const OccT &occ, Scratch &S, const pr_seed_opts &O, const uint8_t *q, int len, int &err,
                       unsigned long long *ticks = nullptr) {
#if defined(__HIP_DEVICE_COMPILE__)
    unsigned long long t_last = ticks ? __builtin_amdgcn_s_memrealtime() : 0ULL;
#endif
    int nm = 0, n1 = 0;
    auto push = [&](const Iv &v) {
        if (nm >= S.cap_mems) {
            err |= SC_OVER_MEMS;
            return;
        }
        S.mems[nm++] = v;
    };
    for (int x = 0; x < len && !err;) {
        if (q[x] < 4) {
            x = smem1(occ, S, q, len, x, 1, S.m1, n1, err);
            for (int k = 0; k < n1; ++k)
                if (S.m1[k].end - S.m1[k].start >= O.min_seed_len) push(S.m1[k]);
        } else {
            ++x;
        }
    }
    SC_TICK(0);
    const int split_len = (int)(O.min_seed_len * O.split_factor + .499);
    const int nfirst = nm;
    for (int k = 0; k < nfirst && !err; ++k) {
        const Iv p = S.mems[k];
        if (p.end - p.start < split_len || p.occ > O.split_width) continue;
        smem1(occ, S, q, len, (p.start + p.end) >> 1, p.occ + 1, S.m1, n1, err);
        for (int j = 0; j < n1; ++j)
            if (S.m1[j].end - S.m1[j].start >= O.min_seed_len) push(S.m1[j]);
    }
    SC_TICK(1);
    if (O.max_mem_intv > 0) {
        for (int x = 0; x < len && !err;) {
            if (q[x] < 4) {
                Iv m;
                x = seed_strategy1(occ, q, len, x, O.min_seed_len, O.max_mem_intv, m);
                if (m.occ > 0) push(m);
            } else {
                ++x;
            }
        }
    }
    if (nm > 1 && S.cap_seeds >= nm && !err && !S.hend) {
        static_assert(sizeof(Seed) == sizeof(Iv), "the seed pool holds the sorted intervals");
        int32_t *cnt = S.codes;
        Iv *tmp = reinterpret_cast<Iv *>(S.seeds);
        for (int x = 0; x <= len; ++x) cnt[x] = 0;
        for (int i = 0; i < nm; ++i) ++cnt[S.mems[i].start + 1];
        for (int x = 1; x <= len; ++x) cnt[x] += cnt[x - 1];
        for (int i = 0; i < nm; ++i) {
            const Iv v = S.mems[i];
            tmp[cnt[v.start]++] = v;
        }
        for (int i = 0; i < nm; ++i) {
            const Iv v = tmp[i];
            int j = i - 1;
            while (j >= 0 && S.mems[j].start == v.start && S.mems[j].end > v.end) {
                S.mems[j + 1] = S.mems[j];
                --j;
            }
            S.mems[j + 1] = v;
        }
    } else {
        for (int i = 1; i < nm; ++i) {
            const Iv v = S.mems[i];
            int j = i - 1;
            while (j >= 0 && (S.mems[j].start > v.start || (S.mems[j].start == v.start && S.mems[j].end > v.end))) {
                S.mems[j + 1] = S.mems[j];
                --j;
            }
            S.mems[j + 1] = v;
        }
    }
    SC_TICK(2);
    return nm;
}

SC_HD int range_slot(const Scratch &S, int32_t key) {
    uint32_t h = ((uint32_t)key * 0x9E3779B1u) & (uint32_t)(S.hsize - 1);
    while (S.htab[h].key != -1 && S.htab[h].key != key) h = (h + 1) & (uint32_t)(S.hsize - 1);
    return (int)h;
}
SC_HD int32_t pack_ql(const Seed &s) { return (int32_t)(uint16_t)s.qbeg | ((int32_t)s.len << 16); }

SC_HD int test_and_merge(const pr_seed_opts &O, int64_t l_pac, Scratch &S, int32_t &ns, Chain &c, const Seed &p,
                         int rid) {
    const Seed &last = S.seeds[c.tail];
    const Seed &first = S.seeds[c.head];
    const int64_t qend = last.qbeg + last.len, rend = last.rbeg + last.len;
    if (rid != c.rid) return 0;
    if (p.qbeg >= first.qbeg && p.qbeg + p.len <= qend && p.rbeg >= first.rbeg && p.rbeg + p.len <= rend)
        return 1;
    if ((last.rbeg < l_pac || first.rbeg < l_pac) && p.rbeg >= l_pac) return 0;
    const int64_t x = p.qbeg - last.qbeg, y = p.rbeg - last.rbeg;
    if (y >= 0 && x - y <= O.w && y - x <= O.w && x - last.len < O.max_chain_gap && y - last.len < O.max_chain_gap) {
        if (ns >= S.cap_seeds) return -1;
        S.seeds[ns] = p;
        S.seeds[ns].nx = -1;
        S.seeds[c.tail].nx = ns;
        c.tail = ns++;
        ++c.n;
        return 1;
    }
    return 0;
}

SC_HD int merge_tail(const pr_seed_opts &O, int64_t l_pac, Scratch &S, int32_t &ns, RangeRec &R, const Seed &p) {
    const int64_t f_rbeg = R.f_rbeg, l_rbeg = R.l_rbeg;
    const int f_q = (int16_t)(R.f_ql & 0xFFFF), l_q = (int16_t)(R.l_ql & 0xFFFF), l_len = R.l_ql >> 16;
    const int64_t qend = l_q + l_len, rend = l_rbeg + l_len;
    if (p.qbeg >= f_q && p.qbeg + p.len <= qend && p.rbeg >= f_rbeg && p.rbeg + p.len <= rend)
        return 1;
    if ((l_rbeg < l_pac || f_rbeg < l_pac) && p.rbeg >= l_pac) return 0;
    const int64_t x = p.qbeg - l_q, y = p.rbeg - l_rbeg;
    if (y >= 0 && x - y <= O.w && y - x <= O.w && x - l_len < O.max_chain_gap && y - l_len < O.max_chain_gap) {
        if (ns >= S.cap_seeds) return -1;
        S.seeds[ns] = p;
        S.seeds[ns].nx = -1;
        S.seeds[R.l_idx].nx = ns;
        R.l_idx = ns++;
        R.l_rbeg = p.rbeg;
        R.l_ql = pack_ql(p);
        ++R.n;
        return 1;
    }
    return 0;
}
SC_HD void flush_tail(Scratch &S, const RangeRec &R) {
    S.cv[R.tail].tail = R.l_idx;
    S.cv[R.tail].n = R.n;
}

SC_HD int chain_weight(const Scratch &S, const Chain &c) {
    int64_t qe = 0, re = 0;
    int wq = 0, wr = 0;
    for (int32_t k = c.head; k >= 0;) {
        const Seed s = S.seeds[k];
        if (s.qbeg >= qe) wq += s.len;
        else if (s.qbeg + s.len > qe) wq += (int)(s.qbeg + s.len - qe);
        qe = qe > s.qbeg + s.len ? qe : s.qbeg + s.len;
        if (s.rbeg >= re) wr += s.len;
        else if (s.rbeg + s.len > re) wr += (int)(s.rbeg + s.len - re);
        re = re > s.rbeg + s.len ? re : s.rbeg + s.len;
        k = s.nx;
    }
    const int w = wr < wq ? wr : wq;
    return w < (1 << 30) ? w : (1 << 30) - 1;
}

SC_HD int cal_max_gap(const pr_seed_opts &O, int qlen) {
    int l_del = (int)((double)(qlen * O.a - O.o_del) / O.e_del + 1.);
    int l_ins = (int)((double)(qlen * O.a - O.o_ins) / O.e_ins + 1.);
    int l = l_del > l_ins ? l_del : l_ins;
    l = l > 1 ? l : 1;
    return l < O.w << 1 ? l : O.w << 1;
}

SC_HD int seed_flt_min_score(const pr_seed_opts &O, int len) {
    double min_l;
    if (O.min_chain_weight) min_l = (double)(1.1f * (float)O.min_chain_weight);
    else min_l = (double)5.5f * log((double)len);
    if (min_l > (double)(0.05f * (float)len)) return -1;
    return (int)(O.a * min_l + .499);
}

template <class T>
SC_HD int seed_sw_score(const IndexView &I, const pr_seed_opts &O, const uint8_t *q, int len, const Seed &s, int rid,
                        T *H, T *E, int stride = 1) {
    if (s.len >= 200) return -1;
    int qb = s.qbeg - 50, qe = s.qbeg + s.len + 50;
    qb = qb > 0 ? qb : 0;
    qe = qe < len ? qe : len;
    int64_t rb = s.rbeg - 50, re = s.rbeg + s.len + 50;
    const int64_t mid = (s.rbeg + s.rbeg + s.len) >> 1;
    rb = rb > 0 ? rb : 0;
    re = re < (I.l_pac << 1) ? re : (I.l_pac << 1);
    if (rb < I.l_pac && I.l_pac < re) {
        if (mid < I.l_pac) re = I.l_pac;
        else rb = I.l_pac;
    }
    if (qe - qb >= 200 || re - rb >= 200) return -1;
    const bool rev = mid >= I.l_pac;
    const int64_t fb = rev ? (I.l_pac << 1) - I.lr_off[rid + 1] : I.lr_off[rid];
    const int64_t fe = rev ? (I.l_pac << 1) - I.lr_off[rid] : I.lr_off[rid + 1];
    rb = rb > fb ? rb : fb;
    re = re < fe ? re : fe;
    const int64_t tc = rev ? I.cstart[2 * I.n_lr - 1 - rid] : I.cstart[rid];
    const uint8_t *t = I.text + tc + (rb - fb);
    const int qn = qe - qb, tn = (int)(re - rb);
    const int oe_del = O.o_del + O.e_del, oe_ins = O.o_ins + O.e_ins;
    for (int j = 0; j < qn; ++j) H[j * stride] = 0, E[j * stride] = 0;
    int best = 0;
    for (int i = 0; i < tn; ++i) {
        const int ti = t[i];
        int hdiag = 0, f = 0;
        for (int j = 0; j < qn; ++j) {
            const int qj = q[qb + j];
            const int sc = (ti > 3 || qj > 3) ? -1 : (ti == qj ? O.a : -O.b);
            int h = hdiag + sc;
            const int e = E[j * stride];
            h = h > e ? h : e;
            h = h > f ? h : f;
            h = h > 0 ? h : 0;
            hdiag = H[j * stride];
            H[j * stride] = (T)h;
            best = best > h ? best : h;
            int en = e - O.e_del, eo = h - oe_del;
            en = en > eo ? en : eo;
            E[j * stride] = (T)(en > 0 ? en : 0);
            int fn = f - O.e_ins, fo = h - oe_ins;
            fn = fn > fo ? fn : fo;
            f = fn > 0 ? fn : 0;
        }
    }
    return best;
}

SC_HD void chain_flt(const pr_seed_opts &O, Scratch &S, int ncv, int *n_chains);
template <bool LZ = false>
SC_HD int chain_seq(const IndexView &I, const pr_seed_opts &O, Scratch &S, int nm, int *n_cv);

template <bool LZ = false>
SC_HD int map_chains(const IndexView &I, const pr_seed_opts &O, Scratch &S, const uint8_t *q, int len, int *n_chains,
                     unsigned long long *ticks = nullptr, const uint32_t *lcnt = nullptr) {
    *n_chains = 0;
    int err = 0;
#if defined(__HIP_DEVICE_COMPILE__)
    unsigned long long t_last = ticks ? __builtin_amdgcn_s_memrealtime() : 0ULL;
#endif
    const OccB<LZ> occ{&I, &S, q, len, lcnt};
    const int nm = collect_intv(occ, S, O, q, len, err, ticks);
    if (LZ) err |= S.lz[1];
    if (err) return err;
    SC_STAT(0, 1);
    SC_STAT(1, nm);
#if defined(__HIP_DEVICE_COMPILE__)
    if (ticks) t_last = __builtin_amdgcn_s_memrealtime();
#endif
    int ncv = 0;
    err = chain_seq<LZ>(I, O, S, nm, &ncv);
    if (LZ) err |= S.lz[1];
    if (err) return err;
    SC_TICK(3);
    SC_STAT(11, ncv);
    SC_STAT(12, (unsigned long long)ncv * ncv);
    chain_flt(O, S, ncv, n_chains);
    SC_TICK(4);
    return 0;
}

template <bool LZ>
SC_HD int chain_seq(const IndexView &I, const pr_seed_opts &O, Scratch &S, int nm, int *n_cv) {
    const bool clean_on_entry = S.htab_clean;
    int32_t ns = 0, ncv = 0, nrg = 0;
    if (!clean_on_entry)
        for (int k = 0; k < S.hsize; ++k) S.htab[k].key = -1;
    auto leave = [&](int rc) {
        if (clean_on_entry)
            for (int r = 0; r < nrg; ++r) S.htab[S.rg[r].pad[0]].key = -1;
        return rc;
    };
    for (int mi = 0; mi < nm; ++mi) {
        const Iv p = S.mems[mi];
        const int slen = p.end - p.start;
        if (LZ && !S.ready[p.start]) return leave(SC_OVER_HITS);
        const int32_t h0 = S.hoff[p.start], h1 = LZ ? S.hend[p.start] : S.hoff[p.start + 1];
        const int64_t np = p.occ;
        const int64_t step = np > O.max_occ ? np / O.max_occ : 1;
        int64_t fidx = 0, take = 0, count = 0;
        constexpr int CB = 8;
        int32_t k = h0;
        while (k < h1 && count < O.max_occ) {
            int32_t sel[CB];
            int nsel = 0;
            while (k < h1 && count < O.max_occ && nsel < CB) {
                uint16_t ml[8];
#pragma unroll
                for (int u = 0; u < 8; ++u) ml[u] = k + u < h1 ? S.hml[k + u] : (uint16_t)0;
                int u = 0;
                for (; u < 8 && k < h1 && count < O.max_occ && nsel < CB; ++u, ++k) {
                    if (ml[u] < slen) continue;
                    const bool use = fidx == take;
                    ++fidx;
                    if (!use) continue;
                    take += step;
                    ++count;
                    sel[nsel++] = k;
                }
            }
            int64_t rb[CB];
            int rd[CB], hsl[CB];
            int32_t key[CB];
#pragma unroll
            for (int u = 0; u < CB; ++u) {
                const uint64_t v = u < nsel ? S.hfr[sel[u]] : 0ull;
                rb[u] = (int64_t)(v >> FR_RID_BITS);
                rd[u] = (int)(v & ((1u << FR_RID_BITS) - 1u));
                key[u] = rd[u] * 2 + (rb[u] >= I.l_pac ? 1 : 0);
            }
#pragma unroll
            for (int u = 0; u < CB; ++u) hsl[u] = u < nsel ? range_slot(S, key[u]) : 0;
            bool opened = false;
            for (int u = 0; u < nsel; ++u) {
                SC_STAT(3, 1);
                Seed s;
                s.rbeg = rb[u];
                s.qbeg = (int16_t)p.start;
                s.len = (int16_t)slen;
                s.nx = -1;
                const int rid = rd[u];
                const int hs = opened ? range_slot(S, key[u]) : hsl[u];
                const RangeEnt e = S.htab[hs];
                const bool found = e.key == key[u];
                int at = -1;
                bool at_tail = false;
                if (found) {
                    RangeRec &R = S.rg[e.r];
                    SC_STAT(4, 1);
                    if (R.tpos <= s.rbeg) {
                        at = R.tail;
                        at_tail = true;
                    } else {
                        for (int x = R.head; x >= 0 && S.cv[x].pos <= s.rbeg; x = S.cnx[x]) {
                            at = x;
                            SC_STAT(4, 1);
                        }
                    }
                    if (at >= 0) {
                        const int r = at_tail ? merge_tail(O, I.l_pac, S, ns, R, s)
                                              : test_and_merge(O, I.l_pac, S, ns, S.cv[at], s, rid);
                        if (r < 0) return leave(SC_OVER_SEEDS);
                        if (r) { SC_STAT(5, 1); continue; }
                    }
                }
                SC_STAT(6, 1);
                if (ncv >= S.cap_chains) return leave(SC_OVER_CHAINS);
                if (ns >= S.cap_seeds) return leave(SC_OVER_SEEDS);
                S.seeds[ns] = s;
                Chain c;
                c.pos = s.rbeg;
                c.rid = rid;
                c.head = c.tail = ns;
                c.n = 1;
                c.w = c.kept = 0;
                c.first = -1;
                S.cv[ncv] = c;
                if (!found) {
                    RangeRec &R = S.rg[nrg];
                    R.head = R.tail = ncv;
                    R.n = 1;
                    R.l_idx = ns;
                    R.tpos = s.rbeg;
                    R.f_rbeg = R.l_rbeg = s.rbeg;
                    R.f_ql = R.l_ql = pack_ql(s);
                    R.pad[0] = hs;
                    S.htab[hs].key = key[u];
                    S.htab[hs].r = nrg++;
                    S.cnx[ncv] = -1;
                    opened = true;
                } else {
                    RangeRec &R = S.rg[e.r];
                    if (at < 0) {
                        S.cnx[ncv] = R.head;
                        R.head = ncv;
                    } else {
                        const int nx = S.cnx[at];
                        S.cnx[ncv] = nx;
                        S.cnx[at] = ncv;
                        if (nx < 0) {
                            flush_tail(S, R);
                            R.tail = ncv;
                            R.n = 1;
                            R.l_idx = ns;
                            R.tpos = s.rbeg;
                            R.f_rbeg = R.l_rbeg = s.rbeg;
                            R.f_ql = R.l_ql = pack_ql(s);
                        }
                    }
                }
                ++ns;
                ++ncv;
            }
        }
    }
    for (int r = 0; r < nrg; ++r) {
        flush_tail(S, S.rg[r]);
        if (clean_on_entry) S.htab[S.rg[r].pad[0]].key = -1;
    }
    *n_cv = ncv;
    return 0;
}

SC_HD void chain_flt(const pr_seed_opts &O, Scratch &S, int ncv, int *n_chains) {
    int nch = 0;
    const bool keep_all = O.drop_ratio <= 0;
    for (int j = 0; j < ncv; ++j) {
        Chain c = S.cv[j];
        c.w = chain_weight(S, c);
        if (keep_all) c.kept = 3;
        if (c.w >= O.min_chain_weight) S.ch[nch++] = c;
    }
    for (int i = 1; i < nch; ++i) {
        const Chain v = S.ch[i];
        int j = i - 1;
        while (j >= 0 && (S.ch[j].w < v.w || (S.ch[j].w == v.w && (S.ch[j].pos > v.pos ||
                                                                   (S.ch[j].pos == v.pos && S.ch[j].head > v.head))))) {
            S.ch[j + 1] = S.ch[j];
            --j;
            SC_STAT(13, 1);
        }
        S.ch[j + 1] = v;
    }
    if (nch > 0 && !keep_all) {
        int nk = 1;
        S.kept[0] = 0;
        S.ch[0].kept = 3;
        for (int i = 1; i < nch; ++i) {
            int large = 0, k;
            const int bi = S.seeds[S.ch[i].head].qbeg;
            const int ei = S.seeds[S.ch[i].tail].qbeg + S.seeds[S.ch[i].tail].len;
            for (k = 0; k < nk; ++k) {
                Chain &cj = S.ch[S.kept[k]];
                const int bj = S.seeds[cj.head].qbeg;
                const int ej = S.seeds[cj.tail].qbeg + S.seeds[cj.tail].len;
                const int bmax = bj > bi ? bj : bi;
                const int emin = ej < ei ? ej : ei;
                if (emin > bmax) {
                    const int li = ei - bi, lj = ej - bj;
                    const int minl = li < lj ? li : lj;
                    if (emin - bmax >= minl * O.mask_level && minl < O.max_chain_gap) {
                        large = 1;
                        if (cj.first < 0) cj.first = i;
                        if (S.ch[i].w < cj.w * O.drop_ratio && cj.w - S.ch[i].w >= O.min_seed_len << 1) break;
                    }
                }
            }
            if (k == nk) {
                S.kept[nk++] = i;
                S.ch[i].kept = large ? 2 : 3;
            }
        }
        for (int k = 0; k < nk; ++k)
            if (S.ch[S.kept[k]].first >= 0) S.ch[S.ch[S.kept[k]].first].kept = 1;
    }
    *n_chains = nch;
}

SC_HD int flt_seed_list(const Scratch &S, int nch, int32_t *list, int cap) {
    int n = 0;
    for (int ci = 0; ci < nch; ++ci) {
        const Chain &c = S.ch[ci];
        if (c.kept == 0) continue;
        for (int32_t k = c.head; k >= 0; k = S.seeds[k].nx) {
            if (n >= cap) return -1;
            list[n++] = k;
        }
    }
    return n;
}

SC_HD int map_output(const IndexView &I, const pr_seed_opts &O, Scratch &S, const uint8_t *q, int len, int sid,
                     int nch, pr_seed_task *out, int cap_out, int *n_out, const int32_t *scores = nullptr,
                     unsigned long long *ticks = nullptr, int16_t *dp16 = nullptr) {
    *n_out = 0;
#if defined(__HIP_DEVICE_COMPILE__)
    unsigned long long t_last = ticks ? __builtin_amdgcn_s_memrealtime() : 0ULL;
#endif
    const int flt = seed_flt_min_score(O, len);
    int32_t *swH = (int32_t *)S.ge, *swE = swH + 201;
    int no = 0, nkept = 0;
    for (int ci = 0; ci < nch; ++ci) {
        const Chain &c = S.ch[ci];
        if (c.kept == 0) continue;
        const bool rev = S.seeds[c.head].rbeg >= I.l_pac;
        const int64_t L = I.lr_off[c.rid + 1] - I.lr_off[c.rid];
        const int64_t cs = rev ? I.l_pac + (I.l_pac - I.lr_off[c.rid + 1]) : I.lr_off[c.rid];
        if (no + c.n > cap_out) return SC_OVER_OUT;
        const int first = no;
        int idx = 0;
        int64_t r0 = INT64_MAX, r1 = INT64_MIN;
        for (int32_t k = c.head; k >= 0; k = S.seeds[k].nx) {
            const Seed &s = S.seeds[k];
            int score = s.len;
            if (flt >= 0) {
                const int x = scores ? scores[k]
                                     : (dp16 ? seed_sw_score(I, O, q, len, s, c.rid, dp16, dp16 + 201 * 64, 64)
                                             : seed_sw_score(I, O, q, len, s, c.rid, swH, swE));
                if (x >= 0 && x < flt) continue;
                score = x < 0 ? s.len * O.a : x;
            }
            const int64_t b = s.rbeg - (s.qbeg + cal_max_gap(O, s.qbeg));
            const int64_t e = s.rbeg + s.len + ((len - s.qbeg - s.len) + cal_max_gap(O, len - s.qbeg - s.len));
            r0 = r0 < b ? r0 : b;
            r1 = r1 > e ? r1 : e;
            pr_seed_task &t = out[no];
            t.sr = sid;
            t.lr = c.rid;
            t.strand = rev ? 1 : 0;
            t.qbeg = s.qbeg;
            t.rbeg = (int32_t)(s.rbeg - cs);
            t.slen = s.len;
            t.chain = nkept;
            t.rmax0 = score;
            t.rank = idx++;
            int j = no - 1;
            while (j >= first && (out[j].rmax0 < t.rmax0 || (out[j].rmax0 == t.rmax0 && out[j].rank < t.rank))) --j;
            const pr_seed_task v = t;
            for (int m = no; m > j + 1; --m) out[m] = out[m - 1];
            out[j + 1] = v;
            ++no;
        }
        if (no == first) continue;
        r0 -= cs;
        r1 -= cs;
        for (int m = first; m < no; ++m) {
            out[m].rank = m - first;
            out[m].rmax0 = (int32_t)(r0 > 0 ? r0 : 0);
            out[m].rmax1 = (int32_t)(r1 < L ? r1 : L);
        }
        ++nkept;
    }
    *n_out = no;
    SC_STAT(14, nch);
    SC_STAT(15, no);
    SC_TICK(5);
    return 0;
}

template <bool LZ = false>
SC_HD int map_after_occ(const IndexView &I, const pr_seed_opts &O, Scratch &S, const uint8_t *q, int len, int sid,
                        pr_seed_task *out, int cap_out, int *n_out, unsigned long long *ticks = nullptr,
                        const uint32_t *lcnt = nullptr, int16_t *dp16 = nullptr) {
    *n_out = 0;
    int nch = 0;
    const int err = map_chains<LZ>(I, O, S, q, len, &nch, ticks, lcnt);
    if (err) return err;
    return map_output(I, O, S, q, len, sid, nch, out, cap_out, n_out, nullptr, ticks, dp16);
}
#undef SC_TICK

SC_HD int map_read(const IndexView &I, const pr_seed_opts &O, Scratch &S, const uint8_t *q, int len, int sid,
                   pr_seed_task *out, int cap_out, int *n_out) {
    *n_out = 0;
    if (S.hend) {
        const int err = build_starts(I, S, q, len);
        return err ? err : map_after_occ<true>(I, O, S, q, len, sid, out, cap_out, n_out);
    }
    const int err = build_occ(I, S, q, len);
    return err ? err : map_after_occ<false>(I, O, S, q, len, sid, out, cap_out, n_out);
}

SC_HD bool lazy_occ(const pr_seed_opts &O) { return O.min_seed_len >= 17; }

}
}

namespace prgpu {
namespace seedc {

struct Caps {
    int32_t lmax, hits, iv, mems, seeds, chains, out;
    int32_t hi;
    int32_t nopos;
    int32_t lazy;
};
SC_HD int device_out_cap(int qmax) { return qmax > 192 ? 2 * ((qmax + 15) & ~15) : 384; }
SC_HD Caps device_caps(int qmax = 0) {
    Caps c{1024, 8192, 256, 1024, 8192, 4096, 384, 0};
    c.out = device_out_cap(qmax);
    if (qmax > 192) {
        const int l = (qmax + 15) & ~15;
        c.hits = c.hits > 48 * l ? c.hits : 48 * l;
        c.iv = c.iv > l / 2 ? c.iv : l / 2;
        c.mems = c.mems > 2 * l ? c.mems : 2 * l;
        c.seeds = c.seeds > 4 * l ? c.seeds : 4 * l;
        c.chains = c.chains > 2 * l ? c.chains : 2 * l;
    }
    return c;
}
SC_HD Caps device_caps_small(int lmax) {
    const int l = lmax < 16 ? 16 : (lmax + 15) & ~15;
    Caps c{l, 4096, 64, 512, 512, 384, device_out_cap(lmax), 0};
    if (l > 160) {
        c.hits = c.hits > 24 * l ? c.hits : 24 * l;
        c.iv = c.iv > l / 4 ? c.iv : l / 4;
        c.mems = c.mems > 2 * l ? c.mems : 2 * l;
        c.seeds = c.seeds > 2 * l ? c.seeds : 2 * l;
        c.chains = c.chains > l ? c.chains : l;
    }
    return c;
}
SC_HD Caps grow_caps(Caps c, int32_t flags, int32_t hits_factor) {
    if (flags & SC_OVER_HITS) c.hits *= hits_factor;
    if (flags & SC_OVER_IV) c.iv *= 2;
    if (flags & SC_OVER_MEMS) c.mems *= 2;
    if (flags & SC_OVER_SEEDS) c.seeds *= 2;
    if (flags & SC_OVER_CHAINS) c.chains *= 2;
    return c;
}

SC_HD int64_t align8(int64_t x) { return (x + 7) & ~(int64_t)7; }
SC_HD int32_t range_table_size(int32_t chains) {
    int32_t h = 64;
    while (h < 2 * chains) h <<= 1;
    return h;
}

SC_HD int64_t scratch_bytes(const Caps &c) {
    int64_t b = 0;
    b += align8(4 * (int64_t)(c.lmax + 1));
    b += align8(8 * (int64_t)(c.lmax + 1));
    b += align8(4 * (int64_t)(c.lmax + 1));
    b += align8(4 * (int64_t)c.lmax * HB);
    if (!c.nopos) b += align8(4 * (int64_t)c.hits);
    b += align8(2 * (int64_t)c.hits);
    b += align8((int64_t)sizeof(Iv) * c.mems);
    b += 3 * align8((int64_t)sizeof(Iv) * c.iv);
    b += align8((int64_t)sizeof(Seed) * c.seeds);
    b += 2 * align8((int64_t)sizeof(Chain) * c.chains);
    b += 2 * align8(4 * (int64_t)c.chains);
    b += align8((int64_t)sizeof(RangeEnt) * range_table_size(c.chains));
    b = (b + 63) & ~(int64_t)63;
    b += align8((int64_t)sizeof(RangeRec) * c.chains);
    b += align8(2 * (int64_t)(c.lmax + 1) * RK);
    b += align8(8 * (int64_t)c.hits);
    if (c.hi && !c.nopos) b += align8((int64_t)c.hits);
    if (c.lazy) {
        b += align8(4 * (int64_t)(c.lmax + 1));
        b += align8((int64_t)(c.lmax + 1));
        b += align8(8 * (int64_t)(c.lmax / 16 + 4));
        b += align8(16);
    }
    return (b + 63) & ~(int64_t)63;
}

SC_HD Scratch carve(uint8_t *p, const Caps &c) {
    Scratch S{};
    auto take = [&p](int64_t bytes) {
        uint8_t *r = p;
        p += align8(bytes);
        return r;
    };
    S.lmax = c.lmax;
    S.hoff = (int32_t *)take(4 * (int64_t)(c.lmax + 1));
    S.qext = (uint64_t *)take(8 * (int64_t)(c.lmax + 1));
    S.codes = (int32_t *)take(4 * (int64_t)(c.lmax + 1));
    S.ge = (uint32_t *)take(4 * (int64_t)c.lmax * HB);
    S.hpos = c.nopos ? nullptr : (uint32_t *)take(4 * (int64_t)c.hits);
    S.hml = (uint16_t *)take(2 * (int64_t)c.hits);
    S.cap_hits = c.hits;
    S.mems = (Iv *)take((int64_t)sizeof(Iv) * c.mems);
    S.cap_mems = c.mems;
    S.m1 = (Iv *)take((int64_t)sizeof(Iv) * c.iv);
    S.curr = (Iv *)take((int64_t)sizeof(Iv) * c.iv);
    S.prev = (Iv *)take((int64_t)sizeof(Iv) * c.iv);
    S.cap_iv = c.iv;
    S.seeds = (Seed *)take((int64_t)sizeof(Seed) * c.seeds);
    S.cap_seeds = c.seeds;
    S.cv = (Chain *)take((int64_t)sizeof(Chain) * c.chains);
    S.ch = (Chain *)take((int64_t)sizeof(Chain) * c.chains);
    S.cnx = (int32_t *)take(4 * (int64_t)c.chains);
    S.kept = (int32_t *)take(4 * (int64_t)c.chains);
    S.hsize = range_table_size(c.chains);
    S.htab = (RangeEnt *)take((int64_t)sizeof(RangeEnt) * S.hsize);
    p = (uint8_t *)(((uintptr_t)p + 63) & ~(uintptr_t)63);
    S.rg = (RangeRec *)take((int64_t)sizeof(RangeRec) * c.chains);
    S.cap_chains = c.chains;
    S.rmax = (uint16_t *)take(2 * (int64_t)(c.lmax + 1) * RK);
    S.hfr = (uint64_t *)take(8 * (int64_t)c.hits);
    S.hhi = c.hi && !c.nopos ? (uint8_t *)take((int64_t)c.hits) : nullptr;
    if (c.lazy) {
        S.hend = (int32_t *)take(4 * (int64_t)(c.lmax + 1));
        S.ready = (uint8_t *)take((int64_t)(c.lmax + 1));
        S.q4w = (uint64_t *)take(8 * (int64_t)(c.lmax / 16 + 4));
        S.lz = (int32_t *)take(16);
    }
    return S;
}

}
}
```

proovread_amd/csrc/seed_dev.h:

```cpp
#pragma once
#include <stdint.h>

#include <vector>

#include "seed_core.h"

namespace prgpu {

struct SeedDev {
    seedc::IndexView V;
    pr_seed_opts O;
    const uint8_t *sr_seq;
    const int64_t *sr_off;
    int64_t n_sr;
    uint8_t *scratch;
    int64_t stride;
    int64_t n_lanes;
    int32_t *next;
    unsigned long long *prof;
    seedc::Caps caps;
    pr_seed_task *out;
    int64_t out0;
    int32_t *n_out;
    int32_t *status;
    int16_t *dp;
    const int32_t *rlist;
    int64_t n_list;
};

int seed_launch(const SeedDev &D, void *stream);
int seed_batch_launch(const SeedDev &D, void *stream);
size_t seed_order_bytes(int64_t n);
int seed_order_launch(const SeedDev &D, int64_t r0, int64_t n, void *buf, int32_t **order, void *stream);
int seed_slots_per_cu(int walk_nw);
int seed_compact_launch(const pr_seed_task *slots, const int32_t *n_out, const int64_t *pre, int64_t n_sr, int cap,
                        pr_seed_task *out, void *stream);

seedc::IndexView seed_index_view(const pr_seed_index *h);
struct SeedIndexSizes {
    int64_t text, cstart, cblk, lr_off, koff, kpos, ksplit, cnt[seedc::KI - 1];
};
SeedIndexSizes seed_index_sizes(const pr_seed_index *h);
void seed_digest_tables(const std::vector<uint8_t> &text, const std::vector<uint64_t> &koff,
                        const std::vector<uint32_t> &kpos, const std::vector<uint64_t> &kext,
                        const std::vector<std::vector<uint32_t>> &cnt, const std::vector<int64_t> &cstart,
                        const std::vector<int32_t> &cblk, const std::vector<int64_t> &lr_off,
                        const std::vector<uint64_t> &ksplit, uint64_t *out6);

}
```

proovread_amd/csrc/seed_kernels.hip:

```cpp
#include <hip/hip_runtime.h>

#include <rocprim/device/device_radix_sort.hpp>

#include "seed_core.h"
#include "seed_dev.h"

namespace prgpu {

#ifndef SEED_WAVES_DEF
#define SEED_WAVES_DEF 4
#endif
#ifndef SEED_LMAX_DEF
#define SEED_LMAX_DEF 1024
#endif
constexpr int SEED_WAVES = SEED_WAVES_DEF;
constexpr int SEED_LMAX = SEED_LMAX_DEF;
#ifndef SEED_MINB
#define SEED_MINB 4
#endif
#ifndef SEED_WAVE_MINB
#define SEED_WAVE_MINB SEED_MINB
#endif
#ifndef OCC_U
#define OCC_U 2
// ... 468 lines not shown
            const int r = atomicAdd(&lds[128], 1);
            if (r >= S.cap_chains) {
                S.htab[h].r = -1;
                continue;
            }
            RangeRec &R = S.rg[r];
            R.head = R.tail = e;
            R.n = 1;
            R.l_idx = e;
            R.tpos = sd.rbeg;
            R.f_rbeg = R.l_rbeg = sd.rbeg;
            R.f_ql = R.l_ql = pack_ql(sd);
            S.htab[h].r = r;
            S.cnx[e] = -1;
        } else {
            RangeRec &R = S.rg[S.htab[h].r];
            if (at < 0) {
                S.cnx[e] = R.head;
                R.head = e;
            } else {
                const int nx = S.cnx[at];
                S.cnx[e] = nx;
                S.cnx[at] = e;
                if (nx < 0) {
                    flush_tail(S, R);
                    R.tail = e;
                    R.n = 1;
                    R.l_idx = e;
                    R.tpos = sd.rbeg;
                    R.f_rbeg = R.l_rbeg = sd.rbeg;
                    R.f_ql = R.l_ql = pack_ql(sd);
                }
            }
        }
    }
    __threadfence_block();
    wave_sync_lds();
    const int nrg = lds[128];
    if (nrg > S.cap_chains) return -2;
    for (int r = lane; r < nrg; r += 64) flush_tail(S, S.rg[r]);
    __threadfence_block();
    wave_sync_lds();
    int ncv = 0;
    for (int e0 = 0; e0 < n; e0 += 64) {
        const int e = e0 + lane;
        Chain c{};
        if (e < n) c = S.cv[e];
        const bool live = e < n && c.n > 0;
        const unsigned long long lm = __ballot(live);
        wave_sync_lds();
        if (live) S.cv[ncv + __popcll(lm & below)] = c;
        ncv += __popcll(lm);
        __threadfence_block();
        wave_sync_lds();
    }
    return ncv > S.cap_chains ? -2 : ncv;
}

__device__ bool chain_flt_wave(const pr_seed_opts &O, seedc::Scratch &S, int ncv, int lane, int *n_chains) {
    using namespace seedc;
    const int64_t ge_bytes = (int64_t)S.lmax * HB * 4;
    if ((int64_t)ncv * 36 > ge_bytes) return false;
    struct Key { int32_t nw, head; int64_t pos; };
    const bool keep_all = O.drop_ratio <= 0;
    Key *key = reinterpret_cast<Key *>(S.ge);
    for (int j = lane; j < ncv; j += 64) {
        Chain &c = S.cv[j];
        const int w = chain_weight(S, c);
        c.w = w;
        key[j] = Key{w >= O.min_chain_weight ? -w : INT32_MAX, c.head, c.pos};
    }
    __threadfence_block();
    wave_sync_lds();
    int nch = 0;
    for (int ib = 0; ib < ncv; ib += 64) {
        const int i = ib + lane;
        const Key ki = i < ncv ? key[i] : Key{INT32_MAX, 0, 0};
        const bool pass = ki.nw != INT32_MAX;
        nch += __popcll(__ballot(pass));
        int rank = 0;
        for (int jb = 0; jb < ncv; jb += 64) {
            const Key kj = jb + lane < ncv ? key[jb + lane] : Key{INT32_MAX, 0, 0};
            const int plo = (int)(uint32_t)kj.pos, phi = (int)(kj.pos >> 32);
#pragma unroll
            for (int t = 0; t < 64; ++t) {
                const int nw = __builtin_amdgcn_readlane(kj.nw, t), hd = __builtin_amdgcn_readlane(kj.head, t);
                const int64_t ps = (int64_t)(((uint64_t)(uint32_t)__builtin_amdgcn_readlane(phi, t) << 32) |
                                             (uint32_t)__builtin_amdgcn_readlane(plo, t));
                rank += (nw < ki.nw || (nw == ki.nw && (ps < ki.pos || (ps == ki.pos && hd < ki.head)))) ? 1 : 0;
            }
        }
        if (pass) {
            Chain c = S.cv[i];
            if (keep_all) c.kept = 3;
            S.ch[rank] = c;
        }
    }
    __threadfence_block();
    wave_sync_lds();
    if (keep_all) {
        *n_chains = nch;
        return true;
    }
    int4 *iv = reinterpret_cast<int4 *>(S.ge);
    int4 *kv = iv + nch;
    int32_t *fm = reinterpret_cast<int32_t *>(kv + nch);
    for (int i = lane; i < nch; i += 64) {
        const Chain &c = S.ch[i];
        const Seed &h = S.seeds[c.head], &t = S.seeds[c.tail];
        iv[i] = make_int4(h.qbeg, t.qbeg + t.len, c.w, 0);
        fm[i] = -1;
    }
    __threadfence_block();
    wave_sync_lds();
    if (nch > 0) {
        int nk = 1;
        if (lane == 0) {
            kv[0] = iv[0];
            S.ch[0].kept = 3;
        }
        __threadfence_block();
        wave_sync_lds();
        for (int i = 1; i < nch; ++i) {
            const int4 ci = iv[i];
            const int bi = ci.x, ei = ci.y;
            bool large = false, drop = false;
            for (int kb = 0; kb < nk && !drop; kb += 64) {
                const int k = kb + lane;
                bool ov = false, br = false;
                if (k < nk) {
                    const int4 cj = kv[k];
                    const int bj = cj.x, ej = cj.y;
                    const int bmax = bj > bi ? bj : bi;
                    const int emin = ej < ei ? ej : ei;
                    if (emin > bmax) {
                        const int li = ei - bi, lj = ej - bj;
                        const int minl = li < lj ? li : lj;
                        if (emin - bmax >= minl * O.mask_level && minl < O.max_chain_gap) {
                            ov = true;
                            br = ci.z < cj.z * O.drop_ratio && cj.z - ci.z >= O.min_seed_len << 1;
                        }
                    }
                }
                const unsigned long long bm = __ballot(br);
                const int last = bm ? __ffsll((long long)bm) - 1 : 63;
                if (ov && lane <= last && fm[k] < 0) fm[k] = i;
                large = large || __ballot(ov && lane <= last) != 0ull;
                drop = bm != 0ull;
            }
            if (!drop) {
                if (lane == 0) {
                    kv[nk] = ci;
                    S.ch[i].kept = large ? 2 : 3;
                }
                ++nk;
                __threadfence_block();
                wave_sync_lds();
            }
        }
        __threadfence_block();
        wave_sync_lds();
        for (int k = lane; k < nk; k += 64)
            if (fm[k] >= 0) S.ch[fm[k]].kept = 1;
    }
    __threadfence_block();
    wave_sync_lds();
    *n_chains = nch;
    return true;
}

template <int NW>
__global__ void __launch_bounds__(64 * SEED_WAVES, SEED_WAVE_MINB) seed_wave_kernel(SeedDev D) {
    __shared__ __attribute__((aligned(16))) int32_t hoff_lds[SEED_WAVES][SEED_LMAX + 4];
    __shared__ uint64_t q4_lds[SEED_WAVES][SEED_LMAX / 16 + 4];
    __shared__ uint32_t lcnt[seedc::LC_N];
    load_lcnt(D.V, lcnt);
    const int lane = threadIdx.x & 63, wv = threadIdx.x >> 6;
    const int64_t slot = (int64_t)blockIdx.x * SEED_WAVES + wv;
    if (slot >= D.n_lanes) return;
    seedc::Scratch S = seedc::carve(D.scratch + slot * D.stride, D.caps);
    int32_t *ho = hoff_lds[wv];
    unsigned long long pt[4] = {0ULL, 0ULL, 0ULL, 0ULL};
    unsigned long long pl[6] = {0ULL, 0ULL, 0ULL, 0ULL, 0ULL, 0ULL};
    for (;;) {
        int j = 0;
        if (lane == 0) j = atomicAdd(D.next, 1);
        j = __shfl(j, 0, 64);
        if (j >= D.n_list) {
            if (D.prof && lane == 0) {
                pt[1] += pl[0] + pl[1] + pl[2];
                pt[2] += pl[3] + pl[4];
                pt[3] += pl[5];
                for (int k = 0; k < 4; ++k) atomicAdd(&D.prof[k], pt[k]);
            }
            break;
        }
        const int i = D.rlist ? D.rlist[j] : j;
        const int64_t o = D.sr_off[i];
        const int len = (int)(D.sr_off[i + 1] - o);
        const uint8_t *q = D.sr_seq + o;
        int err = 0;
        const unsigned long long t0 = D.prof && lane == 0 ? wall_clock64() : 0ULL;
        if (len > S.lmax || len > SEED_LMAX - 1) err = seedc::SC_OVER_LEN;
        if (len > 0 && !err) err = build_occ_wave<NW>(D.V, S, q, len, ho, lane, q4_lds[wv], lcnt);
        int nch = 0, nlist = -1, nm = 0;
        unsigned long long tm = 0ULL;
        if (lane == 0) {
            if (D.prof) {
                tm = wall_clock64();
                pt[0] += tm - t0;
                atomicMax(&D.prof[17], tm - t0);
            }
            if (len > 0 && !err) {
                const seedc::Occ occ{&D.V, &S, q, len, lcnt};
                nm = seedc::collect_intv(occ, S, D.O, q, len, err, D.prof ? pl : nullptr);
            }
            if (D.prof) atomicMax(&D.prof[18], wall_clock64() - tm);
        }
        err = __shfl(err, 0, 64);
        nm = __shfl(nm, 0, 64);
        if (len > 0 && !err) {
            const unsigned long long tc = D.prof && lane == 0 ? wall_clock64() : 0ULL;
            __threadfence_block();
            int ncv = chain_wave(D.V, D.O, S, nm, lane, ho);
            unsigned long long tf = D.prof && lane == 0 ? wall_clock64() : 0ULL;
            if (lane == 0 && D.prof) atomicAdd(&D.prof[14 + (ncv == -1 ? 1 : 0)], tf - tc);
            if (ncv == -2) {
                ncv = 0;
                err = seedc::SC_OVER_CHAINS;
            }
            if (lane == 0 && ncv == -1) {
                ncv = 0;
                err = seedc::chain_seq(D.V, D.O, S, nm, &ncv);
                if (D.prof) {
                    const unsigned long long t_ = wall_clock64();
                    atomicAdd(&D.prof[13], 1ULL);
                    atomicAdd(&D.prof[15], t_ - tf);
                    tf = t_;
                }
            }
            err = __shfl(err, 0, 64);
            ncv = __shfl(ncv, 0, 64);
            __threadfence_block();
            wave_sync_lds();
            bool flt = err != 0 || chain_flt_wave(D.O, S, ncv, lane, &nch);
            if (lane == 0) {
                if (!flt) seedc::chain_flt(D.O, S, ncv, &nch);
                if (D.prof) {
                    const unsigned long long t_ = wall_clock64();
                    pl[3] += t_ - tc;
                    atomicAdd(&D.prof[16], t_ - tf);
                }
                if (!err && seedc::seed_flt_min_score(D.O, len) >= 0 && 3 * S.cap_seeds <= 2 * S.cap_hits &&
                    2 * 201 * 64 * 2 <= 4 * S.lmax * seedc::HB)
                    nlist = seedc::flt_seed_list(S, nch, (int32_t *)S.hfr + S.cap_seeds, S.cap_seeds);
            }
        }
        err = __shfl(err, 0, 64);
        nlist = __shfl(nlist, 0, 64);
        if (nlist > 0) {
            __threadfence_block();
            const int32_t *list = (const int32_t *)S.hfr + S.cap_seeds;
            int32_t *rid = (int32_t *)S.hfr + 2 * S.cap_seeds;
            if (lane == 0) {
                int x = 0;
                for (int ci = 0; ci < nch; ++ci) {
                    const seedc::Chain &c = S.ch[ci];
                    if (c.kept == 0) continue;
                    for (int32_t k = c.head; k >= 0; k = S.seeds[k].nx) rid[x++] = c.rid;
                }
            }
            __threadfence_block();
            int32_t *scores = (int32_t *)S.hfr;
            int16_t *H = (int16_t *)S.ge + lane, *E = H + 201 * 64;
            for (int x = lane; x < nlist; x += 64) {
                const int32_t k = list[x];
                scores[k] = seedc::seed_sw_score(D.V, D.O, q, len, S.seeds[k], rid[x], H, E, 64);
            }
            __threadfence_block();
        }
        if (lane == 0) {
            int n = 0;
            if (len > 0 && !err)
                err = seedc::map_output(D.V, D.O, S, q, len, i, nch, D.out + (int64_t)(i - D.out0) * D.caps.out,
                                        D.caps.out, &n, nlist >= 0 ? (const int32_t *)S.hfr : nullptr,
                                        D.prof ? pl : nullptr);
            D.n_out[i] = err ? 0 : n;
            D.status[i] = err;
            if (D.prof) atomicMax(&D.prof[19], wall_clock64() - t0);
        }
        __threadfence_block();
    }
}

template <bool LZ>
__global__ void __launch_bounds__(64 * SEED_WAVES, SEED_MINB) seed_batch_kernel(SeedDev D) {
    __shared__ __attribute__((aligned(16))) int32_t hoff_lds[SEED_WAVES][SEED_LMAX + 4];
    __shared__ uint64_t q4_lds[SEED_WAVES][SEED_LMAX / 16 + 4];
    __shared__ uint32_t lcnt[seedc::LC_N];
    load_lcnt(D.V, lcnt);
    const int lane = threadIdx.x & 63, wv = threadIdx.x >> 6;
    const int64_t slot = (int64_t)blockIdx.x * SEED_WAVES + wv;
    if (slot >= D.n_lanes) return;
    uint8_t *base = D.scratch + slot * 64 * D.stride;
    int32_t *ho = hoff_lds[wv];
    unsigned long long pt[2] = {0ULL, 0ULL};
    unsigned long long lt[6] = {0ULL, 0ULL, 0ULL, 0ULL, 0ULL, 0ULL};
    unsigned long long ot[3] = {0ULL, 0ULL, 0ULL};
    constexpr bool HTAB_REUSE = LZ;
    if (HTAB_REUSE) {
        struct __attribute__((aligned(8))) Ent2 { seedc::RangeEnt a, b; };
        const seedc::Scratch S0 = seedc::carve(base, D.caps);
        const int64_t off = reinterpret_cast<uint8_t *>(S0.htab) - base;
        const Ent2 free2{{-1, -1}, {-1, -1}};
        for (int rd = 0; rd < 64; ++rd) {
            Ent2 *t = reinterpret_cast<Ent2 *>(base + (int64_t)rd * D.stride + off);
            for (int k = lane; k < S0.hsize / 2; k += 64) t[k] = free2;
        }
        __threadfence_block();
        wave_sync_lds();
    }
    for (;;) {
        int b0 = 0;
        if (lane == 0) b0 = atomicAdd(D.next, 64);
        b0 = __shfl(b0, 0, 64);
        const int64_t nlim = D.rlist ? D.n_list : D.n_sr;
        if (b0 >= nlim) {
            if (D.prof) {
#pragma unroll
                for (int k = 0; k < 6; ++k)
                    for (int o = 32; o > 0; o >>= 1) lt[k] += __shfl_xor(lt[k], o, 64);
            }
            if (D.prof && lane == 0) {
                atomicAdd(&D.prof[0], pt[0]);
                atomicAdd(&D.prof[1], pt[1]);
                for (int k = 0; k < 6; ++k) atomicAdd(&D.prof[4 + k], lt[k]);
                for (int k = 0; k < 3; ++k) atomicAdd(&D.prof[10 + k], ot[k]);
            }
            break;
        }
        const unsigned long long t0 = D.prof ? wall_clock64() : 0ULL;
        int my_err = 0, my_hits = 0;
        const int nb = (int)(nlim - b0 < 64 ? nlim - b0 : 64);
        for (int rd = 0; rd < nb; ++rd) {
            const int i = D.rlist ? D.rlist[b0 + rd] : b0 + rd;
            const int64_t o = D.sr_off[i];
            const int len = (int)(D.sr_off[i + 1] - o);
            seedc::Scratch S = seedc::carve(base + (int64_t)rd * D.stride, D.caps);
            int err = 0, nh = 0;
            if (len > S.lmax || len > SEED_LMAX - 1) err = seedc::SC_OVER_LEN;
            if (len > 0 && !err)
                err = build_occ_wave<4>(D.V, S, D.sr_seq + o, len, ho, lane, q4_lds[wv], lcnt, &nh, D.prof ? ot : nullptr,
                                     LZ);
            if (lane == rd) my_err = err, my_hits = nh;
        }
        const unsigned long long t1 = D.prof ? wall_clock64() : 0ULL;
        if (lane < nb) {
            const int i = D.rlist ? D.rlist[b0 + lane] : b0 + lane;
            const int64_t o = D.sr_off[i];
            const int len = (int)(D.sr_off[i + 1] - o);
            seedc::Scratch S = seedc::carve(base + (int64_t)lane * D.stride, D.caps);
            S.htab_clean = HTAB_REUSE;
            int n = 0, err = my_err;
            if (len > 0 && !err)
                err = seedc::map_after_occ<LZ>(D.V, D.O, S, D.sr_seq + o, len, i, D.out + (int64_t)(i - D.out0) * D.caps.out,
                                           D.caps.out, &n, D.prof ? lt : nullptr, lcnt,
                                           D.dp ? D.dp + slot * (2 * 201 * 64) + lane : nullptr);
            D.n_out[i] = (my_err & seedc::SC_OVER_HITS) ? -my_hits
                         : (LZ && (err & seedc::SC_OVER_HITS)) ? -S.lz[2]
                                                                        : (err ? 0 : n);
            D.status[i] = err;
        }
        if (D.prof && lane == 0) {
            pt[0] += t1 - t0;
            pt[1] += wall_clock64() - t1;
        }
        __threadfence_block();
    }
}

__global__ void __launch_bounds__(256) seed_cost_kernel(seedc::IndexView V, const uint8_t *sr_seq, const int64_t *sr_off,
                                                        int64_t r0, int64_t n, uint32_t *key, int32_t *val) {
    for (int64_t k = (int64_t)blockIdx.x * blockDim.x + threadIdx.x; k < n; k += (int64_t)gridDim.x * blockDim.x) {
        const int64_t i = r0 + k;
        const int64_t o = sr_off[i];
        const int len = (int)(sr_off[i + 1] - o);
        uint32_t code = 0u, cost = 0u;
        int valid = 0;
        for (int p = 0; p < len; ++p) {
            const uint32_t c = sr_seq[o + p];
            if (c > 3u) {
                valid = 0;
                continue;
            }
            code = ((code << 2) | c) & (seedc::NK - 1u);
            if (++valid >= seedc::KI && (p & 1) == 0) {
                const uint64_t m = V.koff[code + 1] - V.koff[code];
                cost += m < 1024u ? (uint32_t)m : 1024u;
            }
        }
        key[k] = 0xFFFFFFFFu - cost;
        val[k] = (int32_t)i;
    }
}
size_t seed_order_bytes(int64_t n) {
    size_t tb = 0;
    (void)rocprim::radix_sort_pairs(nullptr, tb, (uint32_t *)nullptr, (uint32_t *)nullptr, (int32_t *)nullptr,
                                    (int32_t *)nullptr, (size_t)(n > 0 ? n : 1), 0u, 32u, (hipStream_t)0);
    return (size_t)(n > 0 ? n : 1) * 16 + ((tb + 255) & ~(size_t)255) + 256;
}
int seed_order_launch(const SeedDev &D, int64_t r0, int64_t n, void *buf, int32_t **order, void *stream) {
    hipStream_t s = (hipStream_t)stream;
    const size_t n1 = (size_t)(n > 0 ? n : 1);
    uint32_t *k0 = (uint32_t *)buf, *k1 = k0 + n1;
    int32_t *v0 = (int32_t *)(k1 + n1), *v1 = v0 + n1;
    void *temp = (void *)(((uintptr_t)(v1 + n1) + 255) & ~(uintptr_t)255);
    size_t tb = 0;
    (void)rocprim::radix_sort_pairs(nullptr, tb, k0, k1, v0, v1, n1, 0u, 32u, s);
    int64_t grid = (n + 255) / 256;
    grid = grid < 4096 ? (grid > 0 ? grid : 1) : 4096;
    hipLaunchKernelGGL(seed_cost_kernel, dim3((unsigned)grid), dim3(256), 0, s, D.V, D.sr_seq, D.sr_off, r0, n, k0, v0);
    hipError_t e = hipGetLastError();
    if (e != hipSuccess) return (int)e;
    if ((e = rocprim::radix_sort_pairs(temp, tb, k0, k1, v0, v1, (size_t)n, 0u, 32u, s)) != hipSuccess) return (int)e;
    *order = v1;
    return 0;
}

int seed_slots_per_cu(int walk_nw) {
    int nb = 0;
    const hipError_t e = walk_nw == 1 ? hipOccupancyMaxActiveBlocksPerMultiprocessor(&nb, seed_wave_kernel<1>, 64 * SEED_WAVES, 0)
                                      : hipOccupancyMaxActiveBlocksPerMultiprocessor(&nb, seed_wave_kernel<4>, 64 * SEED_WAVES, 0);
    if (e != hipSuccess || nb < 1)
        nb = 2;
    return nb * SEED_WAVES;
}

int seed_launch(const SeedDev &D, void *stream) {
    if (D.n_list <= 0) return 0;
    const int64_t blocks = (D.n_lanes + SEED_WAVES - 1) / SEED_WAVES;
    if (D.V.walk_nw == 1)
        hipLaunchKernelGGL(seed_wave_kernel<1>, dim3((unsigned)blocks), dim3(64 * SEED_WAVES), 0, (hipStream_t)stream, D);
    else
        hipLaunchKernelGGL(seed_wave_kernel<4>, dim3((unsigned)blocks), dim3(64 * SEED_WAVES), 0, (hipStream_t)stream, D);
    return (int)hipGetLastError();
}

int seed_batch_launch(const SeedDev &D, void *stream) {
    if (D.n_sr <= 0) return 0;
    const int64_t blocks = (D.n_lanes + SEED_WAVES - 1) / SEED_WAVES;
    if (D.caps.lazy)
        hipLaunchKernelGGL(seed_batch_kernel<true>, dim3((unsigned)blocks), dim3(64 * SEED_WAVES), 0, (hipStream_t)stream, D);
    else
        hipLaunchKernelGGL(seed_batch_kernel<false>, dim3((unsigned)blocks), dim3(64 * SEED_WAVES), 0, (hipStream_t)stream, D);
    return (int)hipGetLastError();
}

__global__ void seed_compact_kernel(const pr_seed_task *slots, const int32_t *n_out, const int64_t *pre, int64_t n_sr,
                                    int cap, pr_seed_task *out) {
    const int64_t i = ((int64_t)blockIdx.x * blockDim.x + threadIdx.x) >> 6;
    const int lane = threadIdx.x & 63;
    if (i >= n_sr) return;
    const int n = n_out[i];
    constexpr int TW = (int)(sizeof(pr_seed_task) / 4);
    const uint32_t *src = reinterpret_cast<const uint32_t *>(slots + i * cap);
    uint32_t *dst = reinterpret_cast<uint32_t *>(out + pre[i]);
    for (int k = lane; k < n * TW; k += 64) dst[k] = src[k];
}

int seed_compact_launch(const pr_seed_task *slots, const int32_t *n_out, const int64_t *pre, int64_t n_sr, int cap,
                        pr_seed_task *out, void *stream) {
    if (n_sr <= 0) return 0;
    const int64_t blocks = (n_sr + 3) / 4;
    hipLaunchKernelGGL(seed_compact_kernel, dim3((unsigned)blocks), dim3(256), 0, (hipStream_t)stream, slots, n_out, pre,
                       n_sr, cap, out);
    return (int)hipGetLastError();
}

}
```

proovread_amd/csrc/seed_plan.h:

```cpp
#pragma once
#include <stdint.h>

#include <algorithm>

#include "seed_core.h"

namespace prgpu {
namespace seedp {

inline int64_t scratch_budget(int64_t free_bytes, int64_t have) {
    return std::min<int64_t>((int64_t)40 << 30, std::max<int64_t>((int64_t)24 << 30, (free_bytes + have) * 15 / 100));
}
inline bool scratch_growth_fits(int64_t want, int64_t free_bytes, int64_t have) { return want <= (free_bytes + have) / 2; }

inline int64_t pass1_wave_cap(int n_cu, int64_t budget, int64_t stride) {
    return std::max<int64_t>(n_cu, budget / (64 * stride));
}
inline int64_t pass1_waves(int64_t n_sr, int n_cu, int waves_per_cu, bool balance, int64_t budget, int64_t stride) {
    int64_t waves = (int64_t)n_cu * waves_per_cu;
    const int64_t nbatch = (n_sr + 63) / 64;
    if (waves > nbatch) waves = nbatch;
    if (waves < 1) waves = 1;
    if (balance) {
        const int64_t rounds = (nbatch + waves - 1) / waves;
        waves = (nbatch + rounds - 1) / rounds;
    }
    return std::min(waves, pass1_wave_cap(n_cu, budget, stride));
}

inline int64_t out_chunk(int64_t out_budget, int64_t slot_bytes) {
    return std::max<int64_t>(64, out_budget / slot_bytes / 64 * 64);
}

struct Flagged {
    int64_t n = 0;
    int32_t flags = 0;
    int64_t need_max = 0, need_sum = 0, need_n = 0;
    void add(int32_t status, int32_t n_out) {
        ++n;
        flags |= status;
        need_max = std::max<int64_t>(need_max, -(int64_t)n_out);
        if (n_out < 0) need_sum -= n_out, ++need_n;
    }
};

inline bool pass1b_wanted(const Flagged &f) { return f.n > 4096 && !(f.flags & (seedc::SC_OVER_LEN | seedc::SC_OVER_OUT)); }

struct Pass1bCaps {
    seedc::Caps cb;
    seedc::Caps cw;
    int64_t sb, sw;
};
inline Pass1bCaps pass1b_caps(const seedc::Caps &small, const seedc::Caps &caps, const Flagged &f) {
    Pass1bCaps p;
    p.cb = small;
    if (f.flags & seedc::SC_OVER_HITS) {
        p.cb.hits = (int32_t)std::min<int64_t>(
            std::max<int64_t>((int64_t)p.cb.hits + 512, (f.need_max + f.need_max / 8 + 511) & ~(int64_t)511), (int64_t)1 << 20);
        const int64_t g = std::min<int64_t>(16, std::max<int64_t>(1, p.cb.hits / small.hits));
        p.cb.chains = (int32_t)(p.cb.chains * g);
        p.cb.seeds = (int32_t)(p.cb.seeds * g);
    }
    p.cb = seedc::grow_caps(p.cb, f.flags, 1);
    p.cw = caps;
    p.cw.hits = std::max(caps.hits, p.cb.hits);
    p.cw.iv = std::max(caps.iv, p.cb.iv);
    p.cw.mems = std::max(caps.mems, p.cb.mems);
    p.cw.seeds = std::max(caps.seeds, p.cb.seeds);
    p.cw.chains = std::max(caps.chains, p.cb.chains);
    p.sb = seedc::scratch_bytes(p.cb);
    p.sw = seedc::scratch_bytes(p.cw);
    return p;
}
inline int64_t pass1b_scratch_want(int64_t waves, int64_t n_flagged, int64_t sb, int64_t free_bytes, int64_t have) {
    const int64_t want = std::min<int64_t>(waves, (n_flagged + 63) / 64) * 64 * sb;
    return want > have && want <= scratch_budget(free_bytes, have) && scratch_growth_fits(want, free_bytes, have) ? want : 0;
}

enum Pass1bMode { P1B_SKIP, P1B_LANE, P1B_WAVE };
enum Pass1bForce { P1B_AUTO, P1B_FORCE_LANE, P1B_FORCE_WAVE };
struct Pass1bRun {
    bool by_wave;
    int64_t wb;
    int64_t ww;
    Pass1bMode mode;
};
inline Pass1bRun pass1b_run(const Pass1bCaps &p, const Flagged &f, int32_t small_hits, Pass1bForce force, int64_t scratch_cap,
                            int64_t waves, int64_t lanes2, int n_cu) {
    Pass1bRun r;
    r.wb = std::min<int64_t>(std::min<int64_t>(scratch_cap / (64 * p.sb), (f.n + 63) / 64), waves);
    r.by_wave = force != P1B_AUTO ? force == P1B_FORCE_WAVE : f.need_sum > 4 * (int64_t)small_hits * f.need_n;
    r.ww = std::min<int64_t>(std::min<int64_t>(lanes2, f.n), scratch_cap / p.sw);
    r.mode = !pass1b_wanted(f) ? P1B_SKIP : r.by_wave && r.ww >= n_cu ? P1B_WAVE : r.wb >= n_cu ? P1B_LANE : P1B_SKIP;
    return r;
}

}
}
```

proovread_amd/seed.py:

```python
from __future__ import annotations

import ctypes as C

import numpy as np

from . import _abi


class SeedOpts(C.Structure):
    _fields_ = [("min_seed_len", C.c_int), ("min_chain_weight", C.c_int), ("w", C.c_int),
                ("split_factor", C.c_double), ("split_width", C.c_int), ("max_mem_intv", C.c_int),
                ("max_occ", C.c_int), ("drop_ratio", C.c_double), ("max_chain_gap", C.c_int),
                ("mask_level", C.c_double), ("a", C.c_int), ("o_del", C.c_int), ("e_del", C.c_int),
                ("o_ins", C.c_int), ("e_ins", C.c_int), ("b", C.c_int)]


class SeedTask(C.Structure):
    _fields_ = [(k, C.c_int32) for k in ("sr", "lr", "strand", "qbeg", "rbeg", "slen", "rmax0", "rmax1",
                                          "chain", "rank")]


class SeedTasks(C.Structure):
    _fields_ = [("n", C.c_int64), ("t", C.POINTER(SeedTask))]


TASK_DTYPE = np.dtype([(k, np.int32) for k, _ in SeedTask._fields_])
_done = False


def _setup(L):
    global _done
    if _done:
        return
    L.pr_seed_opts_default.argtypes = [C.POINTER(SeedOpts), C.c_int]
    L.pr_seed_opts_default.restype = None
    L.pr_seed_index_build.argtypes = [C.c_void_p, C.c_void_p, C.c_int, C.POINTER(C.c_void_p)]
    L.pr_seed_index_free.argtypes = [C.c_void_p]
    L.pr_seed_index_free.restype = None
    L.pr_seed_map.argtypes = [C.c_void_p, C.POINTER(SeedOpts), C.c_void_p, C.c_void_p, C.c_int, C.c_int,
                              C.POINTER(SeedTasks)]
    L.pr_seed_tasks_free.argtypes = [C.POINTER(SeedTasks)]
    L.pr_seed_tasks_free.restype = None
    L.pr_seed_index_digest.argtypes = [C.c_void_p, C.c_void_p]
    L.pr_seed_index_occ.argtypes = [C.c_void_p, C.c_void_p, C.c_int, C.POINTER(C.c_int64)]
    L.pr_seed_smem.argtypes = [C.c_void_p, C.c_void_p, C.c_int, C.c_int, C.c_int64, C.c_void_p, C.c_void_p,
                               C.c_void_p, C.c_int, C.POINTER(C.c_int)]
    L.pr_seed_map_device_caps.argtypes = [C.c_void_p, C.POINTER(SeedOpts), C.c_void_p, C.c_void_p, C.c_int, C.c_int,
                                          C.POINTER(SeedTasks), C.c_void_p]
    L.pr_seed_gpu_upload.argtypes = [C.c_void_p, C.c_void_p]
    L.pr_seed_gpu_map.argtypes = [C.c_void_p, C.POINTER(SeedOpts), C.c_void_p, C.c_void_p, C.c_int,
                                  C.POINTER(SeedTasks), C.c_void_p]
    L.pr_seed_gpu_last_ms.argtypes = [C.c_void_p, C.POINTER(C.c_double)]
    L.pr_seed_gpu_index_build.argtypes = [C.c_void_p, C.c_void_p, C.c_void_p, C.c_int]
    L.pr_seed_gpu_index_digest.argtypes = [C.c_void_p, C.c_void_p]
    L.pr_seed_gpu_index_last_ms.argtypes = [C.c_void_p, C.POINTER(C.c_double)]
    L.pr_seed_gpu_phase_ticks.argtypes = [C.c_void_p, C.c_void_p]
    L.pr_seed_gpu_pass2_ms.argtypes = [C.c_void_p, C.POINTER(C.c_double)]
    L.pr_seed_gpu_pass2_reads.argtypes = [C.c_void_p, C.POINTER(C.c_int64)]
    L.pr_seed_gpu_seed_count.argtypes = [C.c_void_p, C.POINTER(C.c_int64)]
    _done = True


def default_opts(finish: bool = False) -> SeedOpts:
    L = _abi.lib()
    _setup(L)
    o = SeedOpts()
    L.pr_seed_opts_default(C.byref(o), 1 if finish else 0)
    return o


class SeedIndex:

    def __init__(self, lr_seq: np.ndarray, lr_off: np.ndarray):
        self.L = _abi.lib()
        _setup(self.L)
        self._seq = np.ascontiguousarray(lr_seq, np.uint8)
        self._off = np.ascontiguousarray(lr_off, np.int64)
        h = C.c_void_p()
        _abi.check(self.L.pr_seed_index_build(self._seq.ctypes.data, self._off.ctypes.data, len(self._off) - 1,
                                              C.byref(h)), "pr_seed_index_build")
        self.h = h

    def close(self):
        if self.h:
            self.L.pr_seed_index_free(self.h)
            self.h = None

    def __del__(self):
        try:
            self.close()
        except Exception:
            pass

    def digest(self) -> tuple:
        out = np.zeros(6, np.uint64)
        _abi.check(self.L.pr_seed_index_digest(self.h, out.ctypes.data), "pr_seed_index_digest")
        return tuple(int(x) for x in out)

    def occ(self, s: np.ndarray) -> int:
        s = np.ascontiguousarray(s, np.uint8)
        n = C.c_int64()
        _abi.check(self.L.pr_seed_index_occ(self.h, s.ctypes.data, len(s), C.byref(n)), "pr_seed_index_occ")
        return n.value

    def smem(self, q: np.ndarray, x: int, min_intv: int = 1):
        q = np.ascontiguousarray(q, np.uint8)
        cap = len(q) + 1
        st, en, oc = np.zeros(cap, np.int32), np.zeros(cap, np.int32), np.zeros(cap, np.int64)
        n = C.c_int()
        ret = self.L.pr_seed_smem(self.h, q.ctypes.data, len(q), x, min_intv, st.ctypes.data, en.ctypes.data,
                                  oc.ctypes.data, cap, C.byref(n))
        if ret < 0:
            _abi.check(ret, "pr_seed_smem")
        return [(int(st[i]), int(en[i]), int(oc[i])) for i in range(n.value)], ret

    def map(self, sr_seq: np.ndarray, sr_off: np.ndarray, opts: SeedOpts | None = None, threads: int = 0):
        opts = opts or default_opts()
        sr_seq = np.ascontiguousarray(sr_seq, np.uint8)
        sr_off = np.ascontiguousarray(sr_off, np.int64)
        out = SeedTasks()
        _abi.check(self.L.pr_seed_map(self.h, C.byref(opts), sr_seq.ctypes.data, sr_off.ctypes.data,
                                      len(sr_off) - 1, threads, C.byref(out)), "pr_seed_map")
        return self._take(out)

    def map_device_caps(self, sr_seq: np.ndarray, sr_off: np.ndarray, opts: SeedOpts | None = None,
                        threads: int = 0):
        opts = opts or default_opts()
        sr_seq = np.ascontiguousarray(sr_seq, np.uint8)
        sr_off = np.ascontiguousarray(sr_off, np.int64)
        st = np.zeros(max(1, len(sr_off) - 1), np.int32)
        out = SeedTasks()
        _abi.check(self.L.pr_seed_map_device_caps(self.h, C.byref(opts), sr_seq.ctypes.data, sr_off.ctypes.data,
                                                  len(sr_off) - 1, threads, C.byref(out), st.ctypes.data),
                   "pr_seed_map_device_caps")
        return self._take(out), st[:len(sr_off) - 1]

    def to_gpu(self, ctx: "_abi.Context"):
        _abi.check(self.L.pr_seed_gpu_upload(ctx.h, self.h), "pr_seed_gpu_upload")
        self._ctx = ctx

    def map_gpu(self, sr_seq: np.ndarray, sr_off: np.ndarray, opts: SeedOpts | None = None,
                allow_flagged: bool = False):
        return _map_gpu(self.L, self._ctx, sr_seq, sr_off, opts, allow_flagged)

    def gpu_ms(self) -> float:
        return _last_ms(self.L.pr_seed_gpu_last_ms, self._ctx)

    def phase_ms(self) -> dict:
        return _phase_ms(self.L, self._ctx)

    def seed_count(self) -> int:
        n = C.c_int64()
        _abi.check(self.L.pr_seed_gpu_seed_count(self._ctx.h, C.byref(n)), "pr_seed_gpu_seed_count")
        return n.value

    def _take(self, out: SeedTasks):
        return _take(self.L, out)


def _take(L, out: SeedTasks):
    try:
        n = int(out.n)
        if n == 0:
            return np.zeros(0, TASK_DTYPE)
        buf = C.cast(out.t, C.POINTER(C.c_int32 * (10 * n))).contents
        return np.frombuffer(bytes(buf), dtype=TASK_DTYPE).copy()
    finally:
        L.pr_seed_tasks_free(C.byref(out))


def _last_ms(fn, ctx) -> float:
    v = C.c_double()
    _abi.check(fn(ctx.h, C.byref(v)), fn.__name__)
    return v.value


def _count(L, ctx) -> int:
    n = C.c_int64()
    _abi.check(L.pr_seed_gpu_seed_count(ctx.h, C.byref(n)), "pr_seed_gpu_seed_count")
    return n.value


def _phase_ms(L, ctx) -> dict:
    t = np.zeros(4, np.uint64)
    _abi.check(L.pr_seed_gpu_phase_ticks(ctx.h, t.ctypes.data), "pr_seed_gpu_phase_ticks")
    n2 = C.c_int64()
    _abi.check(L.pr_seed_gpu_pass2_reads(ctx.h, C.byref(n2)), "pr_seed_gpu_pass2_reads")
    out = {k: round(float(v) / 1e5, 1) for k, v in
           zip(("occ_table", "lane_phase_and_pass2_smems", "pass2_chaining", "pass2_filter_out"), t)}
    out["pass2_reads"] = n2.value
    if hasattr(L, "pr_seed_gpu_pass_reads"):
        pr = np.zeros(4, np.int64)
        L.pr_seed_gpu_pass_reads.argtypes = [C.c_void_p, C.c_void_p]
        _abi.check(L.pr_seed_gpu_pass_reads(ctx.h, pr.ctypes.data), "pr_seed_gpu_pass_reads")
        out["pass_reads"] = dict(zip(("pass1b_lane", "pass1b_wave", "pass2", "later"), (int(v) for v in pr)))
    lt = np.zeros(6, np.uint64)
    L.pr_seed_gpu_lane_ticks.argtypes = [C.c_void_p, C.c_void_p]
    _abi.check(L.pr_seed_gpu_lane_ticks(ctx.h, lt.ctypes.data), "pr_seed_gpu_lane_ticks")
    out["pass1_lane_ms_summed"] = {k: round(float(v) / 1e5, 1) for k, v in
                                   zip(("smem_pass", "reseeding", "y_seeds_sort", "chaining", "chain_flt", "output"), lt)}
    if hasattr(L, "pr_seed_gpu_occ_ticks"):
        ot = np.zeros(3, np.uint64)
        L.pr_seed_gpu_occ_ticks.argtypes = [C.c_void_p, C.c_void_p]
        _abi.check(L.pr_seed_gpu_occ_ticks(ctx.h, ot.ctypes.data), "pr_seed_gpu_occ_ticks")
        out["occ_table_parts"] = {k: round(float(v) / 1e5, 1) for k, v in zip(("starts", "hits", "count_table"), ot)}
    if hasattr(L, "pr_seed_gpu_pass2_ticks"):
        t2 = np.zeros(7, np.uint64)
        L.pr_seed_gpu_pass2_ticks.argtypes = [C.c_void_p, C.c_void_p]
        _abi.check(L.pr_seed_gpu_pass2_ticks(ctx.h, t2.ctypes.data), "pr_seed_gpu_pass2_ticks")
        out["pass2_parts"] = {"one_lane_reads": int(t2[0])}
        out["pass2_parts"].update({k: round(float(v) / 1e5, 1) for k, v in
                                   zip(("chain_wave", "chain_one_lane", "chain_flt", "max_read_occ_table",
                                        "max_read_smems", "max_read"), t2[1:])})
    p2 = C.c_double()
    _abi.check(L.pr_seed_gpu_pass2_ms(ctx.h, C.byref(p2)), "pr_seed_gpu_pass2_ms")
    out["pass2_wall_ms"] = round(p2.value, 1)
    return out


def _map_gpu(L, ctx, sr_seq, sr_off, opts, allow_flagged, keep_on_device=False):
    opts = opts or default_opts()
    sr_seq = np.ascontiguousarray(sr_seq, np.uint8)
    sr_off = np.ascontiguousarray(sr_off, np.int64)
    st = np.zeros(max(1, len(sr_off) - 1), np.int32)
    if keep_on_device:
        rc = L.pr_seed_gpu_map(ctx.h, C.byref(opts), sr_seq.ctypes.data, sr_off.ctypes.data, len(sr_off) - 1,
                               None, st.ctypes.data)
        if rc != 0 and not (allow_flagged and rc == -9):
            _abi.check(rc, "pr_seed_gpu_map")
        return None, st[:len(sr_off) - 1]
    out = SeedTasks()
    rc = L.pr_seed_gpu_map(ctx.h, C.byref(opts), sr_seq.ctypes.data, sr_off.ctypes.data, len(sr_off) - 1,
                           C.byref(out), st.ctypes.data)
    if rc != 0 and not (allow_flagged and rc == -9):
        L.pr_seed_tasks_free(C.byref(out))
        _abi.check(rc, "pr_seed_gpu_map")
    return _take(L, out), st[:len(sr_off) - 1]


class DeviceSeedIndex:

    def __init__(self, ctx: "_abi.Context", lr_seq: np.ndarray, lr_off: np.ndarray):
        self.L = _abi.lib()
        _setup(self.L)
        self._ctx = ctx
        seq = np.ascontiguousarray(lr_seq, np.uint8)
        off = np.ascontiguousarray(lr_off, np.int64)
        _abi.check(self.L.pr_seed_gpu_index_build(ctx.h, seq.ctypes.data, off.ctypes.data, len(off) - 1),
                   "pr_seed_gpu_index_build")

    def digest(self) -> tuple:
        out = np.zeros(6, np.uint64)
        _abi.check(self.L.pr_seed_gpu_index_digest(self._ctx.h, out.ctypes.data), "pr_seed_gpu_index_digest")
        return tuple(int(x) for x in out)

    def build_ms(self) -> float:
        return _last_ms(self.L.pr_seed_gpu_index_last_ms, self._ctx)

    def map(self, sr_seq: np.ndarray, sr_off: np.ndarray, opts: SeedOpts | None = None, allow_flagged: bool = False,
            keep_on_device: bool = False):
        return _map_gpu(self.L, self._ctx, sr_seq, sr_off, opts, allow_flagged, keep_on_device)

    def gpu_ms(self) -> float:
        return _last_ms(self.L.pr_seed_gpu_last_ms, self._ctx)

    def phase_ms(self) -> dict:
        return _phase_ms(self.L, self._ctx)

    def seed_count(self) -> int:
        n = C.c_int64()
        _abi.check(self.L.pr_seed_gpu_seed_count(self._ctx.h, C.byref(n)), "pr_seed_gpu_seed_count")
        return n.value
```

Baseline: 221.6.

## Batch short-read gather into one kernel, tune pass-1 scratch, output and 1b batching

```diff
diff --git a/include/prgpu.h b/include/prgpu.h
--- a/include/prgpu.h
+++ b/include/prgpu.h
@@ -262,6 +262,7 @@
 int pr_seed_gpu_index_digest(pr_ctx *ctx, uint64_t *out6);
 int pr_seed_gpu_index_last_ms(pr_ctx *ctx, double *ms);
 int pr_seed_gpu_seed_count(pr_ctx *ctx, int64_t *n);
+int pr_seed_gpu_seeds(pr_ctx *ctx, pr_seed_tasks *out);
 int pr_seed_gpu_pass2_reads(pr_ctx *ctx, int64_t *n);
 int pr_seed_gpu_pass_reads(pr_ctx *ctx, int64_t *n4);
 int pr_seed_gpu_last_ms(pr_ctx *ctx, double *ms);
@@ -272,6 +273,9 @@
 int pr_seed_gpu_pass2_ms(pr_ctx *ctx, double *ms);
 int pr_seed_map_device_caps(const pr_seed_index *h, const pr_seed_opts *o, const uint8_t *sr_seq,
                             const int64_t *sr_off, int n_sr, int n_threads, pr_seed_tasks *out, int32_t *status);
+int pr_seed_map_device_pass1(const pr_seed_index *h, const pr_seed_opts *o, const uint8_t *sr_seq,
+                             const int64_t *sr_off, int n_sr, int budget, pr_seed_tasks *out, int32_t *status,
+                             int32_t *hits);
 
 typedef struct pr_iter_batch {
     pr_sw_batch sw;
diff --git a/proovread_amd/csrc/seed.cpp b/proovread_amd/csrc/seed.cpp
--- a/proovread_amd/csrc/seed.cpp
+++ b/proovread_amd/csrc/seed.cpp
@@ -652,6 +652,19 @@
     if (t) t->t = nullptr, t->n = 0;
 }
 
+static std::vector<uint64_t> pack_text4(const seedc::IndexView &V) {
+    std::vector<uint64_t> text4((size_t)(V.n_text / 16 + 8), 0);
+    for (size_t w = 0; w < text4.size(); ++w) {
+        uint64_t v = 0;
+        for (int k = 0; k < 16; ++k) {
+            const int64_t x = (int64_t)w * 16 + k;
+            v |= (uint64_t)(x < V.n_text ? V.text[x] : SEP) << (4 * k);
+        }
+        text4[w] = v;
+    }
+    return text4;
+}
+
 extern "C" int pr_seed_map_device_caps(const pr_seed_index *h, const pr_seed_opts *o, const uint8_t *sr_seq,
                                        const int64_t *sr_off, int n_sr, int n_threads, pr_seed_tasks *out,
                                        int32_t *status) {
@@ -663,15 +676,7 @@
     seedc::IndexView V = view_of(h->I);
     int qmax = 1;
     for (int i = 0; i < n_sr; ++i) qmax = std::max<int>(qmax, (int)(sr_off[i + 1] - sr_off[i]));
-    std::vector<uint64_t> text4((size_t)(V.n_text / 16 + 8), 0);
-    for (size_t w = 0; w < text4.size(); ++w) {
-        uint64_t v = 0;
-        for (int k = 0; k < 16; ++k) {
-            const int64_t x = (int64_t)w * 16 + k;
-            v |= (uint64_t)(x < V.n_text ? V.text[x] : SEP) << (4 * k);
-        }
-        text4[w] = v;
-    }
+    const std::vector<uint64_t> text4 = pack_text4(V);
     V.text4 = text4.data();
     seedc::Caps caps = seedc::device_caps(qmax);
     caps.hi = V.ksplit != nullptr;
@@ -723,3 +728,40 @@
     out->n = total;
     return 0;
 }
+
+extern "C" int pr_seed_map_device_pass1(const pr_seed_index *h, const pr_seed_opts *o, const uint8_t *sr_seq,
+                                        const int64_t *sr_off, int n_sr, int budget, pr_seed_tasks *out, int32_t *status,
+                                        int32_t *hits) {
+    if (!h || !o || !out || !status || !hits || n_sr < 0 || budget < 0 || (n_sr && (!sr_seq || !sr_off)))
+        return pr_set_error(PR_ERR_ARG, "null arg");
+    if (o->min_seed_len < KI) return pr_set_error(PR_ERR_UNSUPPORTED, "min seed length below the 12-mer index");
+    out->n = 0;
+    out->t = nullptr;
+    seedc::IndexView V = view_of(h->I);
+    int qmax = 1;
+    for (int i = 0; i < n_sr; ++i) qmax = std::max<int>(qmax, (int)(sr_off[i + 1] - sr_off[i]));
+    const std::vector<uint64_t> text4 = pack_text4(V);
+    V.text4 = text4.data();
+    seedc::Caps caps = seedc::device_caps_small(std::min(qmax, seedc::device_caps(qmax).lmax));
+    caps.hi = V.ksplit != nullptr;
+    caps.lazy = seedc::lazy_occ(*o) ? 1 : 0;
+    caps.budget = budget;
+    std::vector<uint64_t> slab((size_t)(seedc::scratch_bytes(caps) / 8 + 1), 0);
+    seedc::Scratch S = seedc::carve(reinterpret_cast<uint8_t *>(slab.data()), caps);
+    for (int k = 0; k < S.hsize; ++k) S.htab[k].key = -1;
+    S.htab_clean = true;
+    std::vector<pr_seed_task> buf((size_t)caps.out), all;
+    for (int i = 0; i < n_sr; ++i) {
+        const int len = (int)(sr_off[i + 1] - sr_off[i]);
+        int n = 0, err = 0;
+        if (len > 0) err = seedc::map_read(V, *o, S, sr_seq + sr_off[i], len, i, buf.data(), caps.out, &n);
+        status[i] = err;
+        hits[i] = !caps.lazy || len <= 0 || (err & seedc::SC_OVER_LEN) ? 0 : (err & seedc::SC_OVER_HITS) ? S.lz[2] : S.lz[0];
+        if (!err) all.insert(all.end(), buf.begin(), buf.begin() + n);
+    }
+    out->t = (pr_seed_task *)std::malloc(sizeof(pr_seed_task) * (all.empty() ? 1 : all.size()));
+    if (!out->t) return pr_set_error(PR_ERR_ARG, "out of host memory");
+    std::copy(all.begin(), all.end(), out->t);
+    out->n = (int64_t)all.size();
+    return 0;
+}
diff --git a/proovread_amd/csrc/seed_api.cpp b/proovread_amd/csrc/seed_api.cpp
--- a/proovread_amd/csrc/seed_api.cpp
+++ b/proovread_amd/csrc/seed_api.cpp
@@ -311,14 +311,19 @@
     HIPCHK(hipSetDevice(c->device));
     int rc = dst.ensure((size_t)off.back() + 1);
     if (rc) return rc;
+    std::vector<int64_t> so, dn, ln;
     int64_t at = 0;
     for (int k = 0; k < n_ranges; ++k) {
         const int64_t b0 = c->ss_off[(size_t)ranges[2 * k]], b1 = c->ss_off[(size_t)ranges[2 * k + 1]];
-        if (b1 > b0)
-            HIPCHK(hipMemcpyAsync(dst.as<uint8_t>() + at, c->ls[LS_SRSEQ].as<uint8_t>() + b0, (size_t)(b1 - b0),
-                                  hipMemcpyDeviceToDevice, c->stream));
+        if (b1 > b0) {
+            if (!so.empty() && so.back() + ln.back() == b0) ln.back() += b1 - b0;
+            else so.push_back(b0), dn.push_back(at), ln.push_back(b1 - b0);
+        }
         at += b1 - b0;
     }
+    const int e = sr_gather_launch(c->ls[LS_SRSEQ].as<uint8_t>(), dst.as<uint8_t>(), so.data(), dn.data(), ln.data(),
+                                   (int64_t)so.size(), (void *)c->stream);
+    if (e) return set_error(PR_ERR_HIP, "short-read gather: %s", hipGetErrorString((hipError_t)e));
     return 0;
 }
 
@@ -344,6 +349,7 @@
     int64_t waves;
     int64_t lanes2;
     int64_t chunk;
+    int32_t budget;
     std::vector<int32_t> nout, st;
     std::vector<int64_t> pre;
     int64_t total = 0, bad = 0;
@@ -365,6 +371,8 @@
     small.lazy = seedc::lazy_occ(*o) ? 1 : 0;
     if (const char *sc = getenv("PRGPU_SEED_SMALL"))
         sscanf(sc, "%d,%d,%d,%d,%d", &small.hits, &small.iv, &small.mems, &small.seeds, &small.chains);
+    M.budget = small.lazy ? seedp::PASS1_LAZY_BUDGET : 0;
+    if (const char *bu = getenv("PRGPU_SEED_BUDGET")) M.budget = small.lazy ? std::max(0, atoi(bu)) : 0;
     SeedDev &K = M.K;
     K = SeedDev{};
     K.V = c->seed_view;
@@ -376,12 +384,15 @@
     size_t fr = 0, tot = 0;
     (void)hipMemGetInfo(&fr, &tot);
     (void)hipGetLastError();
-    M.waves = seedp::pass1_waves(M.n_sr, c->n_cu, wpc ? atoi(wpc) : 16, getenv("PRGPU_SEED_BALANCE") != nullptr,
-                                 seedp::scratch_budget((int64_t)fr, (int64_t)M.D[SB_SCRATCH].cap), K.stride);
+    const int per_cu = wpc ? atoi(wpc) : 16;
+    const int64_t full = caps.hi ? 0 : (int64_t)c->n_cu * per_cu * 64 * K.stride;
+    M.waves = seedp::pass1_waves(M.n_sr, c->n_cu, per_cu, getenv("PRGPU_SEED_BALANCE") != nullptr,
+                                 seedp::pass1_budget((int64_t)fr, (int64_t)M.D[SB_SCRATCH].cap, full), K.stride);
     K.n_lanes = M.waves;
     M.lanes2 = (int64_t)c->n_cu * seed_slots_per_cu(c->seed_view.walk_nw);
     const char *ob = getenv("PRGPU_SEED_OUT_MB");
-    M.chunk = seedp::out_chunk((ob ? std::max<int64_t>(1, atoll(ob)) : 8192) << 20,
+    M.chunk = seedp::out_chunk(ob ? std::max<int64_t>(1, atoll(ob)) << 20
+                                  : seedp::out_budget((int64_t)fr, (int64_t)M.D[SB_OUT].cap),
                                (int64_t)caps.out * (int64_t)sizeof(pr_seed_task));
 }
 
@@ -425,8 +436,10 @@
     hipStream_t s = M.s;
     int rc;
     K.caps = M.small;
+    K.caps.budget = M.budget;
     K.stride = seedc::scratch_bytes(M.small);
     K.n_lanes = M.waves;
+    K.batch = 64;
     K.scratch = D[SB_SCRATCH].as<uint8_t>();
     K.rlist = nullptr;
     K.n_list = 0;
@@ -461,11 +474,12 @@
 }
 
 int launch_pass(SeedMap &M, const char *name, bool by_wave, const seedc::Caps &caps, int64_t lanes,
-                const std::vector<int32_t> &reads) {
+                const std::vector<int32_t> &reads, int batch = 64) {
     SeedDev &K = M.K;
     K.caps = caps;
     K.stride = seedc::scratch_bytes(caps);
     K.n_lanes = lanes;
+    K.batch = batch;
     K.scratch = M.D[SB_SCRATCH].as<uint8_t>();
     K.rlist = M.D[SB_PRE].as<int32_t>();
     K.n_list = (int64_t)reads.size();
@@ -509,7 +523,13 @@
         seedp::pass1b_run(p, f, M.small.hits, force, (int64_t)scr.cap, M.waves, M.lanes2, M.c->n_cu);
     if (r.mode == seedp::P1B_SKIP) return 0;
     const bool by_wave = r.mode == seedp::P1B_WAVE;
-    if ((rc = launch_pass(M, by_wave ? "pass 1b, waves" : "pass 1b", by_wave, by_wave ? p.cw : p.cb, by_wave ? r.ww : r.wb, redo)))
+    seedp::Pass1bBatch b{64, r.wb};
+    if (!by_wave && p.cb.lazy) {
+        const char *bb = getenv("PRGPU_SEED_1B_BATCH");
+        b = seedp::pass1b_batch(r, f.n, M.waves, (int64_t)scr.cap, p.sb, bb ? atoi(bb) : 0);
+    }
+    if ((rc = launch_pass(M, by_wave ? "pass 1b, waves" : "pass 1b", by_wave, by_wave ? p.cw : p.cb, by_wave ? r.ww : b.waves,
+                          redo, b.batch)))
         return rc;
     M.c->seed_pass_reads[by_wave ? 1 : 0] += (int64_t)redo.size();
     if (by_wave) p2caps = p.cw, p2_ran = true;
@@ -657,6 +677,21 @@
     return 0;
 }
 
+extern "C" int pr_seed_gpu_seeds(pr_ctx *c, pr_seed_tasks *out) {
+    if (!c || !out) return set_error(PR_ERR_ARG, "null arg");
+    out->n = 0, out->t = nullptr;
+    if (c->seed_pre.empty()) return set_error(PR_ERR_ARG, "no complete seed set on the device");
+    HIPCHK(hipSetDevice(c->device));
+    const int64_t total = c->seed_pre.back();
+    out->t = (pr_seed_task *)std::malloc(sizeof(pr_seed_task) * (size_t)(total > 0 ? total : 1));
+    if (!out->t) return set_error(PR_ERR_ARG, "out of host memory");
+    int rc;
+    if (total && (rc = download(out->t, c->sd[SB_DENSE], (size_t)total, c->stream))) return rc;
+    HIPCHK(hipStreamSynchronize(c->stream));
+    out->n = total;
+    return 0;
+}
+
 extern "C" int pr_seed_gpu_pass2_reads(pr_ctx *c, int64_t *n) {
     if (!c || !n) return set_error(PR_ERR_ARG, "null arg");
     *n = c->seed_pass2;
diff --git a/proovread_amd/csrc/seed_core.h b/proovread_amd/csrc/seed_core.h
--- a/proovread_amd/csrc/seed_core.h
+++ b/proovread_amd/csrc/seed_core.h
@@ -115,6 +115,7 @@
     uint8_t *ready;
     uint64_t *q4w;
     int32_t *lz;
+    int32_t lim_hits;
     bool htab_clean;
 };
 
@@ -209,6 +210,8 @@
 
 template <bool LZ> struct OccB;
 SC_HD void materialize(const OccB<true> &occ, int a);
+template <class OccT> struct occ_lazy { static constexpr bool value = false; };
+template <> struct occ_lazy<OccB<true>> { static constexpr bool value = true; };
 
 template <bool LZ>
 struct OccB {
@@ -422,9 +425,16 @@
     if (code >= 0) {
         const uint64_t r0 = I.koff[code], r1 = I.koff[code + 1];
         const int64_t need = (int64_t)beg + (int64_t)(r1 - r0);
-        if (need > S.cap_hits) {
+        if (need > S.lim_hits) {
+            if (!(S.lz[1] & SC_OVER_HITS)) {
+                int64_t all = 0;
+                for (int x = 0; x + KI <= len; ++x) {
+                    const int32_t cx = S.codes[x];
+                    if (cx >= 0) all += (int64_t)(I.koff[cx + 1] - I.koff[cx]);
+                }
+                S.lz[2] = (int32_t)(all < (int64_t)1 << 30 ? all : (int64_t)1 << 30);
+            }
             S.lz[1] |= SC_OVER_HITS;
-            S.lz[2] = (int32_t)(need < (int64_t)1 << 30 ? need : (int64_t)1 << 30);
         } else {
             n = (int32_t)(r1 - r0);
             const uint64_t qe = S.qext[a];
@@ -721,6 +731,10 @@
     unsigned long long t_last = ticks ? __builtin_amdgcn_s_memrealtime() : 0ULL;
 #endif
     int nm = 0, n1 = 0;
+    auto over = [&]() -> bool {
+        if constexpr (occ_lazy<OccT>::value) return S.lz[1] != 0;
+        else return false;
+    };
     auto push = [&](const Iv &v) {
         if (nm >= S.cap_mems) {
             err |= SC_OVER_MEMS;
@@ -728,7 +742,7 @@
         }
         S.mems[nm++] = v;
     };
-    for (int x = 0; x < len && !err;) {
+    for (int x = 0; x < len && !err && !over();) {
         if (q[x] < 4) {
             x = smem1(occ, S, q, len, x, 1, S.m1, n1, err);
             for (int k = 0; k < n1; ++k)
@@ -740,7 +754,7 @@
     SC_TICK(0);
     const int split_len = (int)(O.min_seed_len * O.split_factor + .499);
     const int nfirst = nm;
-    for (int k = 0; k < nfirst && !err; ++k) {
+    for (int k = 0; k < nfirst && !err && !over(); ++k) {
         const Iv p = S.mems[k];
         if (p.end - p.start < split_len || p.occ > O.split_width) continue;
         smem1(occ, S, q, len, (p.start + p.end) >> 1, p.occ + 1, S.m1, n1, err);
@@ -749,7 +763,7 @@
     }
     SC_TICK(1);
     if (O.max_mem_intv > 0) {
-        for (int x = 0; x < len && !err;) {
+        for (int x = 0; x < len && !err && !over();) {
             if (q[x] < 4) {
                 Iv m;
                 x = seed_strategy1(occ, q, len, x, O.min_seed_len, O.max_mem_intv, m);
@@ -759,6 +773,7 @@
             }
         }
     }
+    if (over()) return nm;
     if (nm > 1 && S.cap_seeds >= nm && !err && !S.hend) {
         static_assert(sizeof(Seed) == sizeof(Iv), "the seed pool holds the sorted intervals");
         int32_t *cnt = S.codes;
@@ -1281,6 +1296,7 @@
     int32_t hi;
     int32_t nopos;
     int32_t lazy;
+    int32_t budget;
 };
 SC_HD int device_out_cap(int qmax) { return qmax > 192 ? 2 * ((qmax + 15) & ~15) : 384; }
 SC_HD Caps device_caps(int qmax = 0) {
@@ -1367,6 +1383,7 @@
     S.hpos = c.nopos ? nullptr : (uint32_t *)take(4 * (int64_t)c.hits);
     S.hml = (uint16_t *)take(2 * (int64_t)c.hits);
     S.cap_hits = c.hits;
+    S.lim_hits = c.lazy && c.budget > 0 && c.budget < c.hits ? c.budget : c.hits;
     S.mems = (Iv *)take((int64_t)sizeof(Iv) * c.mems);
     S.cap_mems = c.mems;
     S.m1 = (Iv *)take((int64_t)sizeof(Iv) * c.iv);
diff --git a/proovread_amd/csrc/seed_dev.h b/proovread_amd/csrc/seed_dev.h
--- a/proovread_amd/csrc/seed_dev.h
+++ b/proovread_amd/csrc/seed_dev.h
@@ -26,12 +26,16 @@
     int16_t *dp;
     const int32_t *rlist;
     int64_t n_list;
+    int32_t batch;
 };
 
 int seed_launch(const SeedDev &D, void *stream);
 int seed_batch_launch(const SeedDev &D, void *stream);
 size_t seed_order_bytes(int64_t n);
 int seed_order_launch(const SeedDev &D, int64_t r0, int64_t n, void *buf, int32_t **order, void *stream);
+constexpr int GATHER_RANGES = 112;
+int sr_gather_launch(const uint8_t *src, uint8_t *dst, const int64_t *s_off, const int64_t *d_off, const int64_t *len,
+                     int64_t n, void *stream);
 int seed_slots_per_cu(int walk_nw);
 int seed_compact_launch(const pr_seed_task *slots, const int32_t *n_out, const int64_t *pre, int64_t n_sr, int cap,
                         pr_seed_task *out, void *stream);
diff --git a/proovread_amd/csrc/seed_kernels.hip b/proovread_amd/csrc/seed_kernels.hip
--- a/proovread_amd/csrc/seed_kernels.hip
+++ b/proovread_amd/csrc/seed_kernels.hip
@@ -794,7 +794,9 @@
     const int lane = threadIdx.x & 63, wv = threadIdx.x >> 6;
     const int64_t slot = (int64_t)blockIdx.x * SEED_WAVES + wv;
     if (slot >= D.n_lanes) return;
-    uint8_t *base = D.scratch + slot * 64 * D.stride;
+    int batch = 64;
+    if constexpr (LZ) batch = D.batch;
+    uint8_t *base = D.scratch + slot * batch * D.stride;
     int32_t *ho = hoff_lds[wv];
     unsigned long long pt[2] = {0ULL, 0ULL};
     unsigned long long lt[6] = {0ULL, 0ULL, 0ULL, 0ULL, 0ULL, 0ULL};
@@ -805,7 +807,7 @@
         const seedc::Scratch S0 = seedc::carve(base, D.caps);
         const int64_t off = reinterpret_cast<uint8_t *>(S0.htab) - base;
         const Ent2 free2{{-1, -1}, {-1, -1}};
-        for (int rd = 0; rd < 64; ++rd) {
+        for (int rd = 0; rd < batch; ++rd) {
             Ent2 *t = reinterpret_cast<Ent2 *>(base + (int64_t)rd * D.stride + off);
             for (int k = lane; k < S0.hsize / 2; k += 64) t[k] = free2;
         }
@@ -814,7 +816,7 @@
     }
     for (;;) {
         int b0 = 0;
-        if (lane == 0) b0 = atomicAdd(D.next, 64);
+        if (lane == 0) b0 = atomicAdd(D.next, batch);
         b0 = __shfl(b0, 0, 64);
         const int64_t nlim = D.rlist ? D.n_list : D.n_sr;
         if (b0 >= nlim) {
@@ -833,7 +835,7 @@
         }
         const unsigned long long t0 = D.prof ? wall_clock64() : 0ULL;
         int my_err = 0, my_hits = 0;
-        const int nb = (int)(nlim - b0 < 64 ? nlim - b0 : 64);
+        const int nb = (int)(nlim - b0 < batch ? nlim - b0 : batch);
         for (int rd = 0; rd < nb; ++rd) {
             const int i = D.rlist ? D.rlist[b0 + rd] : b0 + rd;
             const int64_t o = D.sr_off[i];
@@ -919,6 +921,49 @@
     return 0;
 }
 
+struct GatherArgs {
+    int64_t s_off[GATHER_RANGES], d_off[GATHER_RANGES], len[GATHER_RANGES];
+};
+constexpr int64_t GATHER_TILE = 64 << 10;
+__global__ void __launch_bounds__(256) sr_gather_kernel(const uint8_t *__restrict__ src, uint8_t *__restrict__ dst, GatherArgs A) {
+    const int64_t n = A.len[blockIdx.y];
+    const uint8_t *s = src + A.s_off[blockIdx.y];
+    uint8_t *d = dst + A.d_off[blockIdx.y];
+    const int64_t head = std::min<int64_t>(n, (int64_t)((16 - (reinterpret_cast<uintptr_t>(d) & 15)) & 15));
+    if (blockIdx.x == 0)
+        for (int64_t k = threadIdx.x; k < head; k += blockDim.x) d[k] = s[k];
+    const int64_t body = (n - head) & ~(int64_t)15;
+    for (int64_t t0 = (int64_t)blockIdx.x * GATHER_TILE; t0 < body; t0 += (int64_t)gridDim.x * GATHER_TILE) {
+        const int64_t t1 = std::min<int64_t>(body, t0 + GATHER_TILE);
+        for (int64_t k = t0 + (int64_t)threadIdx.x * 16; k < t1; k += (int64_t)blockDim.x * 16) {
+            uint4 v;
+            __builtin_memcpy(&v, s + head + k, 16);
+            *reinterpret_cast<uint4 *>(d + head + k) = v;
+        }
+    }
+    if (blockIdx.x == 0)
+        for (int64_t k = head + body + threadIdx.x; k < n; k += blockDim.x) d[k] = s[k];
+}
+int sr_gather_launch(const uint8_t *src, uint8_t *dst, const int64_t *s_off, const int64_t *d_off, const int64_t *len,
+                     int64_t n, void *stream) {
+    for (int64_t k0 = 0; k0 < n; k0 += GATHER_RANGES) {
+        const int m = (int)std::min<int64_t>(GATHER_RANGES, n - k0);
+        GatherArgs A{};
+        int64_t lmax = 0;
+        for (int k = 0; k < m; ++k) {
+            A.s_off[k] = s_off[k0 + k];
+            A.d_off[k] = d_off[k0 + k];
+            A.len[k] = len[k0 + k];
+            lmax = std::max(lmax, A.len[k]);
+        }
+        const int64_t tiles = std::max<int64_t>(1, std::min<int64_t>(256, (lmax + GATHER_TILE - 1) / GATHER_TILE));
+        hipLaunchKernelGGL(sr_gather_kernel, dim3((unsigned)tiles, (unsigned)m), dim3(256), 0, (hipStream_t)stream, src, dst, A);
+        const hipError_t e = hipGetLastError();
+        if (e != hipSuccess) return (int)e;
+    }
+    return 0;
+}
+
 int seed_slots_per_cu(int walk_nw) {
     int nb = 0;
     const hipError_t e = walk_nw == 1 ? hipOccupancyMaxActiveBlocksPerMultiprocessor(&nb, seed_wave_kernel<1>, 64 * SEED_WAVES, 0)
@@ -940,6 +985,7 @@
 
 int seed_batch_launch(const SeedDev &D, void *stream) {
     if (D.n_sr <= 0) return 0;
+    if (D.caps.lazy && (D.batch < 1 || D.batch > 64)) return (int)hipErrorInvalidValue;
     const int64_t blocks = (D.n_lanes + SEED_WAVES - 1) / SEED_WAVES;
     if (D.caps.lazy)
         hipLaunchKernelGGL(seed_batch_kernel<true>, dim3((unsigned)blocks), dim3(64 * SEED_WAVES), 0, (hipStream_t)stream, D);
diff --git a/proovread_amd/csrc/seed_plan.h b/proovread_amd/csrc/seed_plan.h
--- a/proovread_amd/csrc/seed_plan.h
+++ b/proovread_amd/csrc/seed_plan.h
@@ -13,6 +13,10 @@
 }
 inline bool scratch_growth_fits(int64_t want, int64_t free_bytes, int64_t have) { return want <= (free_bytes + have) / 2; }
 
+inline int64_t pass1_budget(int64_t free_bytes, int64_t have, int64_t full) {
+    const int64_t b = scratch_budget(free_bytes, have);
+    return full > b && full <= ((int64_t)40 << 30) && full <= (free_bytes + have) / 4 ? full : b;
+}
 inline int64_t pass1_wave_cap(int n_cu, int64_t budget, int64_t stride) {
     return std::max<int64_t>(n_cu, budget / (64 * stride));
 }
@@ -28,6 +32,11 @@
     return std::min(waves, pass1_wave_cap(n_cu, budget, stride));
 }
 
+constexpr int32_t PASS1_LAZY_BUDGET = 0;
+
+inline int64_t out_budget(int64_t free_bytes, int64_t have) {
+    return std::min<int64_t>((int64_t)16 << 30, std::max<int64_t>((int64_t)8 << 30, (free_bytes + have) / 10));
+}
 inline int64_t out_chunk(int64_t out_budget, int64_t slot_bytes) {
     return std::max<int64_t>(64, out_budget / slot_bytes / 64 * 64);
 }
@@ -95,5 +104,20 @@
     return r;
 }
 
+struct Pass1bBatch {
+    int32_t batch;
+    int64_t waves;
+};
+inline Pass1bBatch pass1b_batch(const Pass1bRun &r, int64_t n_flagged, int64_t waves, int64_t scratch_cap, int64_t sb,
+                                int force) {
+    Pass1bBatch b;
+    waves = std::max<int64_t>(waves, 1);
+    const int64_t per = force > 0 ? force : (n_flagged + waves - 1) / waves;
+    b.batch = (int32_t)std::min<int64_t>(64, std::max<int64_t>(1, per));
+    b.waves = std::min<int64_t>(std::min<int64_t>((n_flagged + b.batch - 1) / b.batch, waves), scratch_cap / (b.batch * sb));
+    if (b.waves < 1) b.batch = 64, b.waves = r.wb;
+    return b;
+}
+
 }
 }
diff --git a/proovread_amd/seed.py b/proovread_amd/seed.py
--- a/proovread_amd/seed.py
+++ b/proovread_amd/seed.py
@@ -134,6 +134,20 @@
                                                   len(sr_off) - 1, threads, C.byref(out), st.ctypes.data),
                    "pr_seed_map_device_caps")
         return self._take(out), st[:len(sr_off) - 1]
+
+    def map_device_pass1(self, sr_seq: np.ndarray, sr_off: np.ndarray, opts: SeedOpts | None = None, budget: int = 0):
+        opts = opts or default_opts()
+        sr_seq = np.ascontiguousarray(sr_seq, np.uint8)
+        sr_off = np.ascontiguousarray(sr_off, np.int64)
+        n = len(sr_off) - 1
+        st, hits = np.zeros(max(1, n), np.int32), np.zeros(max(1, n), np.int32)
+        out = SeedTasks()
+        self.L.pr_seed_map_device_pass1.argtypes = [C.c_void_p, C.POINTER(SeedOpts), C.c_void_p, C.c_void_p, C.c_int,
+                                                    C.c_int, C.POINTER(SeedTasks), C.c_void_p, C.c_void_p]
+        _abi.check(self.L.pr_seed_map_device_pass1(self.h, C.byref(opts), sr_seq.ctypes.data, sr_off.ctypes.data, n,
+                                                   budget, C.byref(out), st.ctypes.data, hits.ctypes.data),
+                   "pr_seed_map_device_pass1")
+        return self._take(out), st[:n], hits[:n]
 
     def to_gpu(self, ctx: "_abi.Context"):
         _abi.check(self.L.pr_seed_gpu_upload(ctx.h, self.h), "pr_seed_gpu_upload")
```

Result: faster. 232.5, median of 6 (+4.9%).
